# borglab/gtsfm

Measured on NVIDIA H100. Metric: image_pairs_per_sec, higher is better.
Workload: dtype f32

## Files before the change

gtsfm_b200/_lib.py:

```python
from __future__ import annotations

import ctypes as C
from pathlib import Path
from typing import Optional

import numpy as np

LIB_PATH = Path(__file__).resolve().parent / "libgtsfm_b200.so"

_lib: Optional[C.CDLL] = None


class B200Error(RuntimeError):
    pass


class LightGlueParams(C.Structure):
    _fields_ = [("depth_confidence", C.c_double), ("width_confidence", C.c_double), ("filter_threshold", C.c_double),
                ("prune_min_kpts", C.c_int), ("fp16_attention", C.c_int)]


class LightGluePair(C.Structure):
    _fields_ = [("kp0", C.c_void_p), ("desc0", C.c_void_p), ("n0", C.c_int), ("kp1", C.c_void_p), ("desc1", C.c_void_p), ("n1", C.c_int),
                ("out_matches", C.c_void_p), ("out_scores", C.c_void_p), ("out_k", C.c_int), ("out_stop_layer", C.c_int)]


class MnnPair(C.Structure):
    _fields_ = [("desc0", C.c_void_p), ("n0", C.c_int), ("desc1", C.c_void_p), ("n1", C.c_int), ("out_matches", C.c_void_p),
                ("out_dist", C.c_void_p), ("out_k", C.c_int)]


MNN_ERR_RATIO = -4


class SiftKeypoint(C.Structure):
    _fields_ = [("x", C.c_float), ("y", C.c_float), ("size", C.c_float), ("angle", C.c_float), ("response", C.c_float),
                ("octave", C.c_int32)]


SIFT_KEYPOINT_DTYPE = np.dtype([("x", np.float32), ("y", np.float32), ("size", np.float32), ("angle", np.float32),
                                ("response", np.float32), ("octave", np.int32)])


class SiftImage(C.Structure):
    _fields_ = [("image", C.c_void_p), ("mask", C.c_void_p), ("max_keypoints", C.c_int), ("out_keypoints", C.c_void_p),
                ("out_desc", C.c_void_p), ("out_n", C.c_int), ("out_total", C.c_int)]


class D2NetImage(C.Structure):
    _fields_ = [("image", C.c_void_p), ("max_keypoints", C.c_int), ("out_xy", C.c_void_p), ("out_scores", C.c_void_p),
                ("out_desc", C.c_void_p), ("out_n", C.c_int), ("out_total", C.c_int)]


SIFT_CAPACITY = -5


class RansacParams(C.Structure):
    _fields_ = [("threshold", C.c_double), ("confidence", C.c_double), ("max_iters", C.c_int), ("seed", C.c_uint64)]


_vp, _i, _f, _sz = C.c_void_p, C.c_int, C.c_float, C.c_size_t
_ip = C.POINTER(C.c_int)

SIGNATURES = {
    "b2_version": (_i, []),
    "b2_create": (_i, [_i, C.POINTER(_vp)]),
    "b2_destroy": (None, [_vp]),
    "b2_last_error": (C.c_char_p, [_vp]),
    "b2_launch_count": (C.c_uint64, [_vp]),
    "b2_h2d_bytes": (C.c_uint64, [_vp]),
    "b2_set_option": (C.c_int, [_vp, C.c_char_p, C.c_int64]),
    "b2_profile_start": (_i, [_vp, C.c_char_p]),
    "b2_profile_stop": (_i, [_vp, C.POINTER(C.c_double), C.POINTER(C.c_uint64), C.POINTER(C.c_double)]),
    "b2_debug_fetch": (C.c_int64, [_vp, C.c_char_p, _vp, C.c_int64]),
    "b2_debug_gemm_host": (_i, [_vp, _i, _vp, _vp, _vp, _vp, _i, _i, _i]),
    "b2_debug_attention_host": (_i, [_vp, _i, _ip, _ip, _i, _f, _i, _vp, _vp, _vp, _vp]),
    "b2_superpoint_set_weights": (_i, [_vp, _vp, _sz]),
    "b2_superpoint_detect_dev": (_i, [_vp, _vp, _i, _i, _i, _sz, _f, _i, _i, _vp, _vp, _i, _ip, C.POINTER(C.c_uint64), _vp]),
    "b2_superpoint_describe_dev": (_i, [_vp, C.c_uint64, _vp, _i, _vp, _vp]),
    "b2_superpoint_extract_dev": (_i, [_vp, _vp, _i, _i, _i, _sz, _f, _i, _i, _i, _vp, _vp, _vp, _ip, _vp]),
    "b2_superpoint_extract_async_dev": (_i, [_vp, _vp, _i, _i, _i, _sz, _f, _i, _i, _i, _vp, _vp, _vp, _vp, _vp]),
    "b2_superpoint_finish_dev": (_i, [_vp, _vp]),
    "b2_topk_indices_dev": (_i, [_vp, _vp, _i, _i, _vp, _ip, _vp]),
    "b2_superpoint_detect_host": (_i, [_vp, _vp, _i, _i, _i, _f, _i, _i, _vp, _vp, _i, _ip, C.POINTER(C.c_uint64)]),
    "b2_superpoint_describe_host": (_i, [_vp, C.c_uint64, _vp, _i, _vp]),
    "b2_image_resize_dev": (_i, [_vp, _vp, _i, _i, _i, _sz, _vp, _i, _i, _vp]),
    "b2_lightglue_set_weights": (_i, [_vp, _vp, _sz]),
    "b2_lightglue_match_dev": (_i, [_vp, _vp, _vp, _i, _vp, _vp, _i, C.POINTER(LightGlueParams), _vp, _vp, _ip, _ip, _vp]),
    "b2_lightglue_match_host": (_i, [_vp, _vp, _vp, _i, _vp, _vp, _i, C.POINTER(LightGlueParams), _vp, _vp, _ip, _ip]),
    "b2_lightglue_match_batched_dev": (_i, [_vp, C.POINTER(LightGluePair), _i, C.POINTER(LightGlueParams), _vp]),
    "b2_superglue_set_weights": (_i, [_vp, _vp, _sz]),
    "b2_superglue_match_dev": (_i, [_vp, _vp, _vp, _vp, _i, _i, _i, _vp, _vp, _vp, _i, _i, _i, _i, _f, _vp, _vp, _ip, _vp]),
    "b2_superglue_match_host": (_i, [_vp, _vp, _vp, _vp, _i, _i, _i, _vp, _vp, _vp, _i, _i, _i, _i, _f, _vp, _vp, _ip]),
    "b2_netvlad_blob_floats": (_sz, []),
    "b2_netvlad_set_weights": (_i, [_vp, _vp, _sz]),
    "b2_netvlad_describe_dev": (_i, [_vp, _vp, _i, _i, _i, _vp, _vp]),
    "b2_netvlad_describe_host": (_i, [_vp, _vp, _i, _i, _i, _vp]),
    "b2_megaloc_blob_floats": (_sz, []),
    "b2_megaloc_set_weights": (_i, [_vp, _vp, _sz]),
    "b2_megaloc_describe_dev": (_i, [_vp, _vp, _i, _i, _i, _vp, _vp]),
    "b2_megaloc_describe_host": (_i, [_vp, _vp, _i, _i, _i, _vp]),
    "b2_megaloc_describe_u8_dev": (_i, [_vp, _vp, _i, _i, _i, _sz, _vp, _vp]),
    "b2_megaloc_resize_u8_dev": (_i, [_vp, _vp, _i, _i, _i, _sz, _vp, _vp]),
    "b2_similarity_pairs_host": (_i, [_vp, _vp, _i, _i, _i, _f, _vp, _vp]),
    "b2_ransac_essential_host": (_i, [_vp, _vp, _vp, _i, C.POINTER(RansacParams), _vp, _vp, _ip, _vp, _vp]),
    "b2_ransac_fundamental_host": (_i, [_vp, _vp, _vp, _i, C.POINTER(RansacParams), _vp, _vp, _ip]),
    "b2_ransac_essential_dev": (_i, [_vp, _vp, _vp, _vp, _i, _vp, _vp, C.POINTER(RansacParams), _vp, _vp, _ip, _vp, _vp, _vp]),
    "b2_recover_pose_host": (_i, [_vp, _vp, _vp, _vp, _i, _vp, _vp, _ip]),
    "b2_mnn_match_batched_dev": (_i, [_vp, C.POINTER(MnnPair), _i, _i, _i, C.c_double, _vp]),
    "b2_mnn_match_host": (_i, [_vp, _vp, _i, _vp, _i, _i, _i, C.c_double, _vp, _vp, _ip]),
    "b2_sift_detect_batched_dev": (_i, [_vp, C.POINTER(SiftImage), _i, _i, _i, _i, _sz, _vp]),
    "b2_sift_detect_host": (_i, [_vp, _vp, _i, _i, _i, _vp, _vp, _vp, _i, _ip]),
    "b2_d2net_blob_floats": (_sz, []),
    "b2_d2net_norm_table": (_i, [_vp]),
    "b2_d2net_set_weights": (_i, [_vp, _vp, _sz]),
    "b2_d2net_detect_batched_dev": (_i, [_vp, C.POINTER(D2NetImage), _i, _i, _i, _i, _sz, _vp]),
    "b2_d2net_detect_host": (_i, [_vp, _vp, _i, _i, _i, _i, _vp, _vp, _vp, _ip, _ip]),
    "b2_debug_conv_ps_host": (_i, [_vp, _i, _vp, _i, _i, _i, _i, _vp, _vp, _i, _vp]),
    "b2_debug_d2net_avgpool_host": (_i, [_vp, _vp, _i, _i, _vp]),
    "b2_debug_d2net_rank_host": (_i, [_vp, _vp, _vp, _i, _i, _vp]),
}


def load() -> C.CDLL:
    global _lib
    if _lib is not None:
        return _lib
    if not LIB_PATH.exists():
        raise B200Error(f"{LIB_PATH} is missing: run `python -m gtsfm_b200.build` (there is no CPU fallback)")
    lib = C.CDLL(str(LIB_PATH))
    for name, (res, args) in SIGNATURES.items():
        fn = getattr(lib, name)
        fn.restype = res
        fn.argtypes = args
    _lib = lib
    return lib


def ptr(a) -> C.c_void_p:
    if a is None:
        return C.c_void_p(0)
    if isinstance(a, np.ndarray):
        assert a.flags["C_CONTIGUOUS"], "array must be C-contiguous"
        return C.c_void_p(a.ctypes.data)
    if hasattr(a, "data_ptr"):
        assert a.is_contiguous(), "tensor must be contiguous"
        return C.c_void_p(a.data_ptr())
    return C.c_void_p(int(a))


class Context:

    def __init__(self, device: int = 0):
        self._lib = load()
        h = C.c_void_p()
        rc = self._lib.b2_create(int(device), C.byref(h))
        if rc != 0 or not h:
            raise B200Error(
                f"b2_create(device={device}) failed with {rc}: an sm_90 (H100) GPU is required; there is no CPU fallback")
        self.handle = h
        self.device = device

    def check(self, rc: int, what: str) -> None:
        if rc < 0:
            raise B200Error(f"{what} failed ({rc}): {self._lib.b2_last_error(self.handle).decode()}")

    @property
    def lib(self) -> C.CDLL:
        return self._lib

    def launch_count(self) -> int:
        return int(self._lib.b2_launch_count(self.handle))

    def set_option(self, name: str, value: int) -> None:
        self.check(self._lib.b2_set_option(self.handle, name.encode(), int(value)), f"set_option({name})")

    def h2d_bytes(self) -> int:
        return int(self._lib.b2_h2d_bytes(self.handle))

    def profile_start(self, kernel_prefix: str) -> None:
        self.check(self._lib.b2_profile_start(self.handle, kernel_prefix.encode()), "profile_start")

    def profile_stop(self):
        ms, n, w = C.c_double(0), C.c_uint64(0), C.c_double(0)
        self.check(self._lib.b2_profile_stop(self.handle, C.byref(ms), C.byref(n), C.byref(w)), "profile_stop")
        return ms.value, int(n.value), w.value

    def debug_fetch(self, name: str, max_floats: int) -> np.ndarray:
        out = np.empty(max_floats, np.float32)
        n = self._lib.b2_debug_fetch(self.handle, name.encode(), ptr(out), max_floats)
        self.check(int(n), f"debug_fetch({name})")
        return out[:n]

    def close(self) -> None:
        if getattr(self, "handle", None):
            self._lib.b2_destroy(self.handle)
            self.handle = None

    def __del__(self):
        try:
            self.close()
        except Exception:
            pass
```

gtsfm_b200/csrc/attn_ps.cuh:

```cuda
#pragma once
#include "tma.cuh"

constexpr int AW_Q = 128, AW_KV = 64, AW_D = 64;
constexpr int AW_KV_BYTES = AW_KV * AW_D * 2;
constexpr int AS_NS = 4;
constexpr int AS_HALF = 2 * AW_KV_BYTES;
constexpr int AS_STAGE = 2 * AS_HALF;
constexpr int AS_TILE_BYTES = AS_NS * AS_STAGE;
constexpr int AS_Q_PLANE = AW_Q * AW_D * 2;
constexpr int AS_Q_BYTES = 2 * 2 * AS_Q_PLANE;
constexpr size_t AS_SMEM = AS_TILE_BYTES + AS_Q_BYTES + 1024 + 512;
constexpr int AS_THREADS = 256 + 128;
constexpr float AS_RESCALE = 8.0f;
constexpr int AP_MAXP = 16;

struct AttnPsMaps {
  CUtensorMap kh[AP_MAXP], kl[AP_MAXP], vh[AP_MAXP], vl[AP_MAXP];
};

struct AttnPsProblem {
  const __half *Qh, *Ql;
  __half *Oh, *Ol;
  int Nq, Nk;
  int ldo;
  int qt, tiles;
  int w_end;
  int item0;
};
struct AttnPsArgs {
  AttnPsProblem p[AP_MAXP];
  int nprob;
  float* Opart;
  float* ml;
  int* arrivals;
  int W;
  int quota;
  int max_splits;
  float scale;
  int* err_flag;
};

struct AttnPsSeg {
  int z, item, h, q0, tile0, T, split, nsplits, itemg;
};
__device__ __forceinline__ AttnPsSeg attn_ps_decode(const AttnPsArgs& a, int w, int w_end) {
  AttnPsSeg s;
  s.z = 0;
  while (s.z + 1 < a.nprob && w >= a.p[s.z].w_end) ++s.z;
  const AttnPsProblem& p = a.p[s.z];
  const int base = s.z ? a.p[s.z - 1].w_end : 0;
  const int wl = w - base;
  s.item = wl / p.tiles;
  s.tile0 = wl - s.item * p.tiles;
  s.T = min(p.tiles - s.tile0, w_end - w);
  s.h = s.item / p.qt;
  s.q0 = (s.item - s.h * p.qt) * (2 * AW_Q);
  const int wi0 = base + s.item * p.tiles, wi1 = wi0 + p.tiles;
  const int c_first = wi0 / a.quota;
  s.split = w / a.quota - c_first;
  s.nsplits = (wi1 - 1) / a.quota - c_first + 1;
  s.itemg = p.item0 + s.item;
  return s;
}

template <bool SINGLE>
static __global__ void __launch_bounds__(AS_THREADS, 1) k_flash_ps(const __grid_constant__ AttnPsMaps maps, const __grid_constant__ AttnPsArgs args) {
  extern __shared__ unsigned char ap_raw[];
  const uint32_t raw = tc::smem_u32(ap_raw);
  const uint32_t smem0 = (raw + 1023u) & ~1023u;
  unsigned char* sm = ap_raw + (smem0 - raw);
  uint64_t* bars = reinterpret_cast<uint64_t*>(sm + AS_TILE_BYTES + AS_Q_BYTES);
  uint64_t* kv_full = bars;
  uint64_t* kv_empty = kv_full + AS_NS;
  volatile int* last_flag = reinterpret_cast<volatile int*>(kv_empty + AS_NS);

  const int t = threadIdx.x, warp = t >> 5, lane = t & 31;
  const int w_begin = blockIdx.x * args.quota;
  const int w_end = min(args.W, w_begin + args.quota);

  if (t == 0) {
    for (int i = 0; i < AS_NS; ++i) tc::mbar_init(&kv_full[i], 1), tc::mbar_init(&kv_empty[i], 8);
    tc::fence_mbar_init();
  }
  __syncthreads();
  bool ok = true;

  if (warp >= 8) {
    asm volatile("setmaxnreg.dec.sync.aligned.u32 24;\n" ::: "memory");
    if (warp == 8 && lane == 0) {
      int ge = 0;
      for (int w = w_begin; w < w_end;) {
        const AttnPsSeg sg = attn_ps_decode(args, w, w_end);
        const int Nk = args.p[sg.z].Nk;
        for (int e = 0; e < sg.T + 2; ++e) {
          const int g = ge + e, s = g % AS_NS;
          if (g >= AS_NS) ok = tc::mbar_wait(&kv_empty[s], ((g / AS_NS) - 1) & 1) && ok;
          const bool hk = e < sg.T, hv = e >= 2;
          constexpr int PART = SINGLE ? AW_KV_BYTES : AS_HALF;
          tc::mbar_expect_tx(&kv_full[s], (hk ? PART : 0) + (hv ? PART : 0));
          const uint32_t dst = smem0 + s * AS_STAGE;
          if (hk) {
            const int row = sg.h * Nk + (sg.tile0 + e) * AW_KV;
            tc::tma_load_2d(dst, &maps.kh[sg.z], &kv_full[s], 0, row);
            if (!SINGLE) tc::tma_load_2d(dst + AW_KV_BYTES, &maps.kl[sg.z], &kv_full[s], 0, row);
          }
          if (hv) {
            const int row = sg.h * Nk + (sg.tile0 + e - 2) * AW_KV;
            tc::tma_load_2d(dst + AS_HALF, &maps.vh[sg.z], &kv_full[s], 0, row);
            if (!SINGLE) tc::tma_load_2d(dst + AS_HALF + AW_KV_BYTES, &maps.vl[sg.z], &kv_full[s], 0, row);
          }
        }
        ge += sg.T + 2;
        w += sg.T;
      }
    }
  } else {
    asm volatile("setmaxnreg.inc.sync.aligned.u32 240;\n" ::: "memory");
    const int q = warp >> 2;
    const int r = t & 127;
    const int rq = (warp & 3) * 16 + (lane >> 2);
    const int c2 = (lane & 3) * 2;
    const uint32_t sQ = smem0 + AS_TILE_BYTES + q * 2 * AS_Q_PLANE;
    const float c2s = args.scale * 1.4426950408889634f;
    auto wg_bar = [&]() { asm volatile("bar.sync %0, 128;" ::"r"(1 + q) : "memory"); };
    auto release = [&](int g) { if (lane == 0) tc::mbar_arrive(&kv_empty[g % AS_NS]); };

    int ge = 0;
    for (int w = w_begin; w < w_end;) {
      const AttnPsSeg sg = attn_ps_decode(args, w, w_end);
      const AttnPsProblem& pr = args.p[sg.z];
      const int T = sg.T, Nk = pr.Nk;
      {
        const int qrow = sg.q0 + q * AW_Q + r;
        wg_bar();
#pragma unroll
        for (int pl = 0; pl < (SINGLE ? 1 : 2); ++pl) {
          const __half* src = (pl ? pr.Ql : pr.Qh) + ((size_t)sg.h * pr.Nq + qrow) * 64;
          unsigned char* dst = sm + AS_TILE_BYTES + q * 2 * AS_Q_PLANE + pl * AS_Q_PLANE + r * 128;
#pragma unroll
          for (int c = 0; c < 8; ++c) {
            uint4 v = make_uint4(0u, 0u, 0u, 0u);
            if (qrow < pr.Nq) v = __ldg(reinterpret_cast<const uint4*>(src) + c);
            *reinterpret_cast<uint4*>(dst + ((c ^ (r & 7)) << 4)) = v;
          }
        }
        tc::fence_proxy_async();
        wg_bar();
      }
      uint32_t qf[2][16];
#pragma unroll
      for (int sl = 0; sl < 2; ++sl)
#pragma unroll
        for (int h = 0; h < 2; ++h) {
          const int qrow = sg.q0 + q * AW_Q + sl * 64 + rq + 8 * h;
          const uint32_t* src = reinterpret_cast<const uint32_t*>(pr.Qh + ((size_t)sg.h * pr.Nq + qrow) * 64 + c2);
#pragma unroll
          for (int j = 0; j < 8; ++j) qf[sl][4 * (j >> 1) + 2 * (j & 1) + h] = qrow < pr.Nq ? __ldg(src + 4 * j) : 0u;
        }
      float o[2][32];
      float m_ref[2][2], l_i[2][2];
#pragma unroll
      for (int sl = 0; sl < 2; ++sl)
#pragma unroll
        for (int h = 0; h < 2; ++h) m_ref[sl][h] = -INFINITY, l_i[sl][h] = 0.f;
      float s[2][32];
      uint32_t ph[2][16], pl[2][16];
      auto qk = [&](int i, int sl) {
        const uint32_t sK = smem0 + ((ge + i) % AS_NS) * AS_STAGE;
        const uint64_t dKh = tc::wg_desc_sw128(sK), dKl = tc::wg_desc_sw128(sK + AW_KV_BYTES);
        const uint64_t dQl = tc::wg_desc_sw128(sQ + AS_Q_PLANE + sl * (64 * 128));
        tc::wg_fence();
#pragma unroll
        for (int ks = 0; ks < 4; ++ks) {
          const uint64_t adv = (uint64_t)(ks * 2);
          tc::wg_rs_n64(s[sl], qf[sl] + 4 * ks, dKh + adv, ks ? 1u : 0u);
          if (!SINGLE) {
            tc::wg_rs_n64(s[sl], qf[sl] + 4 * ks, dKl + adv, 1u);
            tc::wg_ss_n64(s[sl], dQl + adv, dKh + adv, 1u);
          }
        }
        tc::wg_commit();
      };
      auto softmax = [&](int i, int sl) {
        float* a = s[sl];
        const int k0 = (sg.tile0 + i) * AW_KV;
        if (k0 + AW_KV > Nk) {
#pragma unroll
          for (int jj = 0; jj < 32; ++jj)
            if (k0 + 8 * (jj >> 2) + c2 + (jj & 1) >= Nk) a[jj] = -INFINITY;
        }
#pragma unroll
        for (int h = 0; h < 2; ++h) {
          float mx = a[2 * h];
#pragma unroll
          for (int j = 0; j < 8; ++j) mx = fmaxf(mx, fmaxf(a[4 * j + 2 * h], a[4 * j + 2 * h + 1]));
          mx = fmaxf(mx, __shfl_xor_sync(0xffffffffu, mx, 1));
          mx = fmaxf(mx, __shfl_xor_sync(0xffffffffu, mx, 2));
          const float m_new = fmaxf(m_ref[sl][h], mx * c2s);
          if (m_new - m_ref[sl][h] > AS_RESCALE) {
            const float corr = tc::ex2(m_ref[sl][h] - m_new);
            l_i[sl][h] *= corr;
            if (i > 0) {
#pragma unroll
              for (int j = 0; j < 8; ++j) o[sl][4 * j + 2 * h] *= corr, o[sl][4 * j + 2 * h + 1] *= corr;
            }
            m_ref[sl][h] = m_new;
          }
          float rs = 0.f;
#pragma unroll
          for (int j = 0; j < 8; ++j) {
            const float p0 = tc::ex2(fmaf(a[4 * j + 2 * h], c2s, -m_ref[sl][h]));
            const float p1 = tc::ex2(fmaf(a[4 * j + 2 * h + 1], c2s, -m_ref[sl][h]));
            rs += p0 + p1;
            const __half2 hh = __floats2half2_rn(p0, p1);
            const int ri = 4 * (j >> 1) + 2 * (j & 1) + h;
            ph[sl][ri] = *reinterpret_cast<const uint32_t*>(&hh);
            if (!SINGLE) {
              const float2 hf = __half22float2(hh);
              const __half2 ll = __floats2half2_rn(p0 - hf.x, p1 - hf.y);
              pl[sl][ri] = *reinterpret_cast<const uint32_t*>(&ll);
            }
          }
          l_i[sl][h] += rs;
        }
      };
      auto pv = [&](int i, int sl) {
        const uint32_t sV = smem0 + ((ge + i + 2) % AS_NS) * AS_STAGE + AS_HALF;
        const uint64_t dVh = tc::wg_desc_sw128(sV), dVl = tc::wg_desc_sw128(sV + AW_KV_BYTES);
        tc::wg_fence();
#pragma unroll
        for (int ks = 0; ks < 4; ++ks) {
          const uint64_t advV = (uint64_t)(ks * 128);
          tc::wg_rs_n64_bt(o[sl], ph[sl] + 4 * ks, dVh + advV, (i | ks) ? 1u : 0u);
          if (!SINGLE) {
            tc::wg_rs_n64_bt(o[sl], ph[sl] + 4 * ks, dVl + advV, 1u);
            tc::wg_rs_n64_bt(o[sl], pl[sl] + 4 * ks, dVh + advV, 1u);
          }
        }
        tc::wg_commit();
      };

      for (int j = 0; j < 2; ++j) ok = tc::mbar_wait(&kv_full[(ge + j) % AS_NS], ((ge + j) / AS_NS) & 1) && ok;
      if (T == 1) release(ge + 1);
      for (int i = 0; i < T; ++i) {
        qk(i, 0);
        qk(i, 1);
        tc::wg_wait<1>();
        tc::fence_regs(s[0]);
        softmax(i, 0);
        const int gv = ge + i + 2;
        ok = tc::mbar_wait(&kv_full[gv % AS_NS], (gv / AS_NS) & 1) && ok;
        pv(i, 0);
        tc::wg_wait<1>();
        tc::fence_regs(s[1]);
        release(ge + i);
        softmax(i, 1);
        pv(i, 1);
        tc::wg_wait<0>();
        tc::fence_regs(o[0]), tc::fence_regs(o[1]);
        if (i + 2 >= T) release(gv);
      }
      ge += T + 2;
      w += T;
#pragma unroll
      for (int sl = 0; sl < 2; ++sl)
#pragma unroll
        for (int h = 0; h < 2; ++h) {
          l_i[sl][h] += __shfl_xor_sync(0xffffffffu, l_i[sl][h], 1);
          l_i[sl][h] += __shfl_xor_sync(0xffffffffu, l_i[sl][h], 2);
        }
      auto write_row = [&](const float* v, float inv, int qrow) {
        uint32_t* dh = reinterpret_cast<uint32_t*>(pr.Oh + (size_t)qrow * pr.ldo + sg.h * 64 + c2);
        uint32_t* dl = reinterpret_cast<uint32_t*>(pr.Ol + (size_t)qrow * pr.ldo + sg.h * 64 + c2);
#pragma unroll
        for (int j = 0; j < 8; ++j) {
          uint32_t hi, lo;
          if (SINGLE) {
            const __half2 hh = __floats2half2_rn(tc::clamp_h(v[4 * j] * inv), tc::clamp_h(v[4 * j + 1] * inv));
            hi = *reinterpret_cast<const uint32_t*>(&hh), lo = 0u;
          } else {
            tc::split2(v[4 * j] * inv, v[4 * j + 1] * inv, hi, lo);
          }
          dh[4 * j] = hi;
          dl[4 * j] = lo;
        }
      };
      if (sg.nsplits == 1) {
#pragma unroll
        for (int sl = 0; sl < 2; ++sl)
#pragma unroll
          for (int h = 0; h < 2; ++h) {
            const int qrow = sg.q0 + q * AW_Q + sl * 64 + rq + 8 * h;
            if (qrow >= pr.Nq) continue;
            float v[32];
#pragma unroll
            for (int j = 0; j < 8; ++j) v[4 * j] = o[sl][4 * j + 2 * h], v[4 * j + 1] = o[sl][4 * j + 2 * h + 1];
            write_row(v, 1.0f / l_i[sl][h], qrow);
          }
      } else {
        const size_t slot0 = (size_t)sg.itemg * args.max_splits;
#pragma unroll
        for (int sl = 0; sl < 2; ++sl)
#pragma unroll
          for (int h = 0; h < 2; ++h) {
            const int rl = q * AW_Q + sl * 64 + rq + 8 * h;
            if (sg.q0 + rl >= pr.Nq) continue;
            const size_t rowi = (slot0 + sg.split) * 256 + rl;
            float* dst = args.Opart + rowi * 64 + c2;
#pragma unroll
            for (int j = 0; j < 8; ++j) *reinterpret_cast<float2*>(dst + 8 * j) = make_float2(o[sl][4 * j + 2 * h], o[sl][4 * j + 2 * h + 1]);
            if (c2 == 0) *reinterpret_cast<float2*>(args.ml + rowi * 2) = make_float2(m_ref[sl][h], l_i[sl][h]);
          }
        __threadfence();
        wg_bar();
        if (r == 0) {
          int* cnt = args.arrivals + sg.itemg * 2 + q;
          const int old = atomicAdd(cnt, 1);
          const int last = old == sg.nsplits - 1;
          if (last) atomicExch(cnt, 0);
          last_flag[q] = last;
        }
        wg_bar();
        if (last_flag[q]) {
          __threadfence();
#pragma unroll 1
          for (int sl = 0; sl < 2; ++sl)
#pragma unroll 1
            for (int h = 0; h < 2; ++h) {
              const int rl = q * AW_Q + sl * 64 + rq + 8 * h;
              const int qrow = sg.q0 + rl;
              if (qrow >= pr.Nq) continue;
              float m = -INFINITY;
              for (int sp = 0; sp < sg.nsplits; ++sp) m = fmaxf(m, __ldcg(args.ml + ((slot0 + sp) * 256 + rl) * 2));
              float l = 0.f, v[32];
#pragma unroll
              for (int j = 0; j < 32; ++j) v[j] = 0.f;
              for (int sp = 0; sp < sg.nsplits; ++sp) {
                const size_t ri = (slot0 + sp) * 256 + rl;
                const float2 mlv = __ldcg(reinterpret_cast<const float2*>(args.ml + ri * 2));
                const float wgt = tc::ex2(mlv.x - m);
                l = fmaf(mlv.y, wgt, l);
                const float* src = args.Opart + ri * 64 + c2;
#pragma unroll
                for (int j = 0; j < 8; ++j) {
                  const float2 x = __ldcg(reinterpret_cast<const float2*>(src + 8 * j));
                  v[4 * j] = fmaf(x.x, wgt, v[4 * j]), v[4 * j + 1] = fmaf(x.y, wgt, v[4 * j + 1]);
                }
              }
              write_row(v, 1.0f / l, qrow);
            }
        }
      }
    }
  }
  if (!ok && args.err_flag) *args.err_flag = 1;
}
```

gtsfm_b200/csrc/common.cuh:

```cuda
#pragma once
#include <cuda_runtime.h>
#include <stdint.h>
#include <stdio.h>
#include <stdlib.h>
#include <string.h>

#include <map>
#include <mutex>
#include <string>
#include <vector>

#include "../../include/gtsfm_b200.h"

#define B2_OK 0
#define B2_ERR_CUDA -1
#define B2_ERR_ARG -2
#define B2_ERR_STATE -3
#define B2_ERR_MNN_RATIO -4
#define B2_SIFT_CAPACITY -5

struct DevBuf {
  void* p = nullptr;
  size_t cap = 0;
  DevBuf() = default;
  DevBuf(const DevBuf&) = delete;
  DevBuf& operator=(const DevBuf&) = delete;
  ~DevBuf() { release(); }
  cudaError_t ensure(size_t bytes) {
    if (bytes <= cap) return cudaSuccess;
    if (p) cudaFree(p);
    p = nullptr;
    cap = 0;
    size_t want = bytes + bytes / 8 + 256;
    cudaError_t e = cudaMalloc(&p, want);
    if (e == cudaSuccess) cap = want;
    return e;
  }
  template <typename T>
  T* as() const { return reinterpret_cast<T*>(p); }
  void release() {
    if (p) cudaFree(p);
    p = nullptr;
    cap = 0;
  }
};

struct HostBuf {
  void* p = nullptr;
  size_t cap = 0;
  HostBuf() = default;
  HostBuf(const HostBuf&) = delete;
  HostBuf& operator=(const HostBuf&) = delete;
  ~HostBuf() { release(); }
  cudaError_t ensure(size_t bytes) {
    if (bytes <= cap) return cudaSuccess;
    if (p) cudaFreeHost(p);
    p = nullptr;
    cap = 0;
    size_t want = bytes + bytes / 8 + 256;
    cudaError_t e = cudaMallocHost(&p, want);
    if (e == cudaSuccess) cap = want;
    return e;
  }
  template <typename T>
  T* as() const { return reinterpret_cast<T*>(p); }
  void release() {
    if (p) cudaFreeHost(p);
    p = nullptr;
    cap = 0;
  }
};

struct DebugView {
  const float* p;
  int64_t n;
};

struct ProfState {
  bool on = false;
  std::string name;
  std::vector<cudaEvent_t> ev;
  size_t used = 0;
  double work = 0.0;
  bool match(const char* kernel) const { return on && strncmp(kernel, name.c_str(), name.size()) == 0; }
};

struct SuperPointState;
struct LightGlueState;
struct SuperGlueState;
struct RansacState;
struct RetrievalState;
struct NetVladState;
struct MnnState;
struct SiftState;
struct MegaLocState;
struct D2NetState;

struct FeatCacheEntry {
  const void* host = nullptr;
  size_t bytes = 0;
  uint64_t sig = 0;
  uint64_t stamp = 0;
  DevBuf buf;
};
constexpr int B2_FEAT_CACHE_SLOTS = 96;

struct b2_context {
  int device = 0;
  int sm_count = 132;
  int reserve_sms = 0;
  int lg_batch = 0;
  int sp_graph = -1;
  int force_simt = -1;
  std::string err;
  std::mutex mu;
  uint64_t launches = 0;
  ProfState prof;
  cudaStream_t stream = nullptr;
  std::map<std::string, DebugView> debug;
  SuperPointState* sp = nullptr;
  LightGlueState* lg = nullptr;
  SuperGlueState* sg = nullptr;
  RansacState* rs = nullptr;
  RetrievalState* rt = nullptr;
  NetVladState* nv = nullptr;
  MnnState* mn = nullptr;
  SiftState* sf = nullptr;
  MegaLocState* ml = nullptr;
  D2NetState* d2 = nullptr;
  DevBuf stage_d[8];
  HostBuf stage_h[4];
  FeatCacheEntry fcache[B2_FEAT_CACHE_SLOTS];
  DevBuf resize_taps;
  uint64_t fstamp = 0;
  int fcache_on = -1;
  uint64_t h2d_bytes = 0;
};

inline bool b2_force_simt(const b2_context* ctx) {
  if (ctx->force_simt >= 0) return ctx->force_simt != 0;
  const char* e = getenv("B2_FORCE_SIMT");
  return e && e[0] == '1';
}

inline int b2_fail(b2_context* ctx, int code, const std::string& msg) {
  if (ctx) ctx->err = msg;
  return code;
}

#define B2_CUDA(ctx, expr)                                                                        \
  do {                                                                                            \
    cudaError_t _e = (expr);                                                                      \
    if (_e != cudaSuccess) {                                                                      \
      return b2_fail(ctx, B2_ERR_CUDA, std::string(#expr) + ": " + cudaGetErrorString(_e) +       \
                                           " (" + __FILE__ + ":" + std::to_string(__LINE__) + ")"); \
    }                                                                                             \
  } while (0)

inline void b2_prof_mark(b2_context* ctx, cudaStream_t st) {
  ProfState& p = ctx->prof;
  if (p.used == p.ev.size()) {
    cudaEvent_t e;
    cudaEventCreate(&e);
    p.ev.push_back(e);
  }
  cudaEventRecord(p.ev[p.used++], st);
}
inline void b2_prof_work(b2_context* ctx, const char* kernel, double work) {
  if (ctx->prof.match(kernel)) ctx->prof.work += work;
}

#define B2_LAUNCH(ctx, kernel, grid, block, smem, stream, ...)  \
  do {                                                          \
    const bool _prof = (ctx)->prof.match(#kernel);              \
    if (_prof) b2_prof_mark((ctx), (stream));                   \
    kernel<<<(grid), (block), (smem), (stream)>>>(__VA_ARGS__); \
    if (_prof) b2_prof_mark((ctx), (stream));                   \
    (ctx)->launches++;                                          \
  } while (0)

#define B2_CHECK_LAUNCH(ctx) B2_CUDA(ctx, cudaGetLastError())

static inline int cdiv(int a, int b) { return (a + b - 1) / b; }

void sp_destroy(b2_context* ctx);
void lg_destroy(b2_context* ctx);
void sg_destroy(b2_context* ctx);
void rs_destroy(b2_context* ctx);
void rt_destroy(b2_context* ctx);
void nv_destroy(b2_context* ctx);
void mn_destroy(b2_context* ctx);
void sf_destroy(b2_context* ctx);
void ml_destroy(b2_context* ctx);
void d2_destroy(b2_context* ctx);

__device__ __forceinline__ float warp_sum(float v) {
#pragma unroll
  for (int o = 16; o > 0; o >>= 1) v += __shfl_xor_sync(0xffffffffu, v, o);
  return v;
}
__device__ __forceinline__ float warp_max(float v) {
#pragma unroll
  for (int o = 16; o > 0; o >>= 1) v = fmaxf(v, __shfl_xor_sync(0xffffffffu, v, o));
  return v;
}
```

gtsfm_b200/csrc/debug.cu:

```cuda
#include <stdlib.h>

#include <vector>

#include "common.cuh"
#include "linear.cuh"

static __global__ void k_split_unscaled_f32(const float* __restrict__ x, size_t n, __half* __restrict__ hi, __half* __restrict__ lo) {
  const size_t i = (size_t)blockIdx.x * blockDim.x + threadIdx.x;
  if (i < n) tc::split_h_unscaled(x[i], hi[i], lo[i]);
}

extern "C" int b2_debug_gemm_host(b2_context* ctx, int mode, const float* A, const float* B, const float* bias, float* C,
                                  int M, int N, int K) {
  if (!ctx || !A || !B || !C || M <= 0 || N <= 0 || K <= 0 || (K % 64)) return B2_ERR_ARG;
  std::lock_guard<std::mutex> lk(ctx->mu);
  cudaSetDevice(ctx->device);
  cudaStream_t st = ctx->stream;
  DevBuf dA, dB, dC, dBias, dErr;
  B2_CUDA(ctx, dA.ensure((size_t)M * K * 4));
  B2_CUDA(ctx, dB.ensure((size_t)N * K * 4));
  B2_CUDA(ctx, dC.ensure((size_t)M * N * 4));
  B2_CUDA(ctx, dBias.ensure((size_t)N * 4));
  B2_CUDA(ctx, dErr.ensure(16));
  B2_CUDA(ctx, cudaMemcpyAsync(dA.p, A, (size_t)M * K * 4, cudaMemcpyHostToDevice, st));
  B2_CUDA(ctx, cudaMemcpyAsync(dB.p, B, (size_t)N * K * 4, cudaMemcpyHostToDevice, st));
  if (bias) B2_CUDA(ctx, cudaMemcpyAsync(dBias.p, bias, (size_t)N * 4, cudaMemcpyHostToDevice, st));
  B2_CUDA(ctx, cudaMemsetAsync(dErr.p, 0, 16, st));
  if (mode == 0) {
    const int rc = launch_gemm(ctx, st, gemm_linear(dA.as<float>(), K, K, dB.as<float>(), bias ? dBias.as<float>() : nullptr, dC.as<float>(), N, M, N));
    if (rc != B2_OK) return rc;
  } else {
    DevBuf dAh, dAl, dBh, dBl;
    B2_CUDA(ctx, dAh.ensure((size_t)M * K * 2));
    B2_CUDA(ctx, dAl.ensure((size_t)M * K * 2));
    B2_CUDA(ctx, dBh.ensure((size_t)N * K * 2));
    B2_CUDA(ctx, dBl.ensure((size_t)N * K * 2));
    B2_LAUNCH(ctx, k_split_f32, (unsigned)(((size_t)M * K + 255) / 256), 256, 0, st, dA.as<float>(), (size_t)M * K, dAh.as<__half>(), dAl.as<__half>());
    B2_LAUNCH(ctx, k_split_f32, (unsigned)(((size_t)N * K + 255) / 256), 256, 0, st, dB.as<float>(), (size_t)N * K, dBh.as<__half>(), dBl.as<__half>());
    B2_CUDA(ctx, cudaFuncSetAttribute(k_gemm_ws, cudaFuncAttributeMaxDynamicSharedMemorySize, (int)GW_SMEM));
    TcWeights tw{nullptr, nullptr, nullptr, dErr.as<int>(), true};
    tw.sm_count = ctx->sm_count;
    LinArgs a;
    a.a1p = {dAh.as<__half>(), dAl.as<__half>()}, a.lda1 = K, a.K1 = K, a.bp = {dBh.as<__half>(), dBl.as<__half>()}, a.ldb = K;
    a.bias = bias ? dBias.as<float>() : nullptr, a.cf = dC.as<float>(), a.ldc = N, a.tc_want_f32 = true, a.M = M, a.N = N;
    const int rc = run_linear(ctx, st, tw, &a, 1);
    if (rc != B2_OK) return rc;
    B2_CUDA(ctx, cudaStreamSynchronize(st));
  }
  int err = 0;
  B2_CUDA(ctx, cudaMemcpyAsync(C, dC.p, (size_t)M * N * 4, cudaMemcpyDeviceToHost, st));
  B2_CUDA(ctx, cudaMemcpyAsync(&err, dErr.p, 4, cudaMemcpyDeviceToHost, st));
  B2_CUDA(ctx, cudaStreamSynchronize(st));
  if (err) return b2_fail(ctx, B2_ERR_STATE, "wgmma pipeline timed out on an mbarrier (kernel bug)");
  return B2_OK;
}

extern "C" int b2_debug_attention_host(b2_context* ctx, int np, const int* nq, const int* nk, int heads, float scale, int single,
                                       const float* q, const float* k, const float* v, float* o) {
  if (!ctx || !nq || !nk || !q || !k || !v || !o || np <= 0 || np > AP_MAXP || heads <= 0) return B2_ERR_ARG;
  size_t eq = 0, ek = 0;
  for (int z = 0; z < np; ++z) {
    if (nq[z] <= 0 || nk[z] <= 0) return B2_ERR_ARG;
    eq += (size_t)nq[z] * heads * 64, ek += (size_t)nk[z] * heads * 64;
  }
  std::lock_guard<std::mutex> lk(ctx->mu);
  cudaSetDevice(ctx->device);
  cudaStream_t st = ctx->stream;
  const size_t n = eq + 2 * ek;
  DevBuf dIn, dPl, dO, dErr, part, ml, cnt;
  B2_CUDA(ctx, dIn.ensure(n * 4));
  B2_CUDA(ctx, dPl.ensure(n * 2 * 2));
  B2_CUDA(ctx, dO.ensure(eq * 2 * 2));
  B2_CUDA(ctx, dErr.ensure(16));
  float* in = dIn.as<float>();
  B2_CUDA(ctx, cudaMemcpyAsync(in, q, eq * 4, cudaMemcpyHostToDevice, st));
  B2_CUDA(ctx, cudaMemcpyAsync(in + eq, k, ek * 4, cudaMemcpyHostToDevice, st));
  B2_CUDA(ctx, cudaMemcpyAsync(in + eq + ek, v, ek * 4, cudaMemcpyHostToDevice, st));
  B2_CUDA(ctx, cudaMemsetAsync(dErr.p, 0, 16, st));
  __half *hi = dPl.as<__half>(), *lo = hi + n, *oh = dO.as<__half>(), *ol = oh + eq;
  B2_LAUNCH(ctx, k_split_unscaled_f32, (unsigned)((n + 255) / 256), 256, 0, st, in, n, hi, lo);
  B2_CUDA(ctx, cudaFuncSetAttribute(k_flash_ps<false>, cudaFuncAttributeMaxDynamicSharedMemorySize, (int)AS_SMEM));
  B2_CUDA(ctx, cudaFuncSetAttribute(k_flash_ps<true>, cudaFuncAttributeMaxDynamicSharedMemorySize, (int)AS_SMEM));
  FlashPlanes fp[AP_MAXP];
  size_t qo = 0, ko = eq;
  for (int z = 0; z < np; ++z) {
    const size_t vo = ko + ek;
    fp[z] = {{hi + qo, lo + qo}, {hi + ko, lo + ko}, {hi + vo, lo + vo}, {oh + qo, ol + qo}, nq[z], nk[z], heads, 64 * heads};
    qo += (size_t)nq[z] * heads * 64, ko += (size_t)nk[z] * heads * 64;
  }
  TcWeights tw{nullptr, nullptr, nullptr, dErr.as<int>(), true};
  tw.attn_part = &part, tw.attn_ml = &ml, tw.attn_cnt = &cnt, tw.sm_count = ctx->sm_count;
  const int rc = run_flash_planes(ctx, st, tw, fp, np, scale, single != 0);
  if (rc != B2_OK) return rc;
  std::vector<__half> ho(2 * eq);
  int err = 0;
  B2_CUDA(ctx, cudaMemcpyAsync(ho.data(), oh, eq * 2 * 2, cudaMemcpyDeviceToHost, st));
  B2_CUDA(ctx, cudaMemcpyAsync(&err, dErr.p, 4, cudaMemcpyDeviceToHost, st));
  B2_CUDA(ctx, cudaStreamSynchronize(st));
  for (size_t i = 0; i < eq; ++i) o[i] = __half2float(ho[i]) + __half2float(ho[eq + i]) * tc::LO_INV;
  if (err) return b2_fail(ctx, B2_ERR_STATE, "wgmma attention timed out on an mbarrier (kernel bug)");
  return B2_OK;
}
```

gtsfm_b200/csrc/gemm_ws.cuh:

```cuda
#pragma once
#include "tma.cuh"

constexpr int GW_MAXP = 16;
constexpr int GW_M = 128, GW_N = 128, GW_K = 64;
constexpr int GW_A_BYTES = GW_M * GW_K * 2;
constexpr int GW_B_BYTES = GW_N * GW_K * 2;
constexpr int GW_STAGE_BYTES = 2 * GW_A_BYTES + 2 * GW_B_BYTES;
constexpr int GW_STAGES = 2;
constexpr int GW_PITCH = GW_N + 8;
constexpr int GW_STG_BYTES = GW_M * GW_PITCH * 4;
constexpr int GW_RB = 8;
constexpr int GW_EW = 4;
constexpr int GW_THREADS = 512;
constexpr size_t GW_SMEM = GW_STAGES * GW_STAGE_BYTES + GW_STG_BYTES + 1024  + 256 ;

struct GemmProblem {
  const float* resid;
  float* C;
  __half *Ch, *Cl;
  int M, N, ldc;
  int vec4;
  int tiles_n;
  int tile_end;
};
struct GemmWsMaps {
  CUtensorMap a1h[GW_MAXP], a1l[GW_MAXP];
  CUtensorMap a2h[GW_MAXP], a2l[GW_MAXP];
  CUtensorMap bh[GW_MAXP], bl[GW_MAXP];
};
struct GemmWsArgs {
  GemmProblem p[GW_MAXP];
  int nprob, tiles;
  int K1, K2;
  int b_per_problem;
  const float* bias;
  int ldr;
  float scale;
  int ldch;
  int head_major;
  int relu;
  int gelu;
  int lo_unscaled;
  int* err_flag;
};

static __global__ void __launch_bounds__(GW_THREADS, 1) k_gemm_ws(const __grid_constant__ GemmWsMaps maps, const __grid_constant__ GemmWsArgs g) {
  extern __shared__ unsigned char gw_raw[];
  const uint32_t raw = tc::smem_u32(gw_raw);
  const uint32_t smem0 = (raw + 1023u) & ~1023u;
  unsigned char* sm = gw_raw + (smem0 - raw);
  float* stg = reinterpret_cast<float*>(sm + GW_STAGES * GW_STAGE_BYTES);
  uint64_t* full = reinterpret_cast<uint64_t*>(sm + GW_STAGES * GW_STAGE_BYTES + GW_STG_BYTES);
  uint64_t* empty = full + GW_STAGES;
  uint64_t* sfull = empty + GW_STAGES;
  uint64_t* sempty = sfull + 1;

  const int t = threadIdx.x, warp = t >> 5, lane = t & 31;
  const int nk = (g.K1 + g.K2) / GW_K;

  if (t == 0) {
    for (int s = 0; s < GW_STAGES; ++s) tc::mbar_init(&full[s], 1), tc::mbar_init(&empty[s], 8);
    tc::mbar_init(sfull, 256);
    tc::mbar_init(sempty, 32 * GW_EW);
    tc::fence_mbar_init();
    tc::tma_prefetch_desc(&maps.bh[0]);
    tc::tma_prefetch_desc(&maps.bl[0]);
  }
  __syncthreads();
  bool ok = true;

  auto decode = [&](int tile, int& z, int& m0, int& n0) {
    z = 0;
    while (z + 1 < g.nprob && tile >= g.p[z].tile_end) ++z;
    const int local = tile - (z ? g.p[z - 1].tile_end : 0);
    const int mt = local / g.p[z].tiles_n;
    n0 = (local - mt * g.p[z].tiles_n) * GW_N;
    m0 = mt * GW_M;
  };

  if (warp >= 12) {
    asm volatile("setmaxnreg.dec.sync.aligned.u32 40;\n" ::: "memory");
    if (warp == 12 && lane == 0) {
      int gk = 0;
      for (int tile = blockIdx.x; tile < g.tiles; tile += gridDim.x) {
        int z, m0, n0;
        decode(tile, z, m0, n0);
        const int zb = g.b_per_problem ? z : 0;
        for (int kc = 0; kc < nk; ++kc, ++gk) {
          const int s = gk % GW_STAGES;
          if (gk >= GW_STAGES) ok = tc::mbar_wait(&empty[s], ((gk / GW_STAGES) - 1) & 1) && ok;
          const int k0 = kc * GW_K;
          const bool seg2 = k0 >= g.K1;
          const CUtensorMap* ah = seg2 ? &maps.a2h[z] : &maps.a1h[z];
          const CUtensorMap* al = seg2 ? &maps.a2l[z] : &maps.a1l[z];
          const int ka = seg2 ? k0 - g.K1 : k0;
          const uint32_t sA = smem0 + s * GW_STAGE_BYTES, sB = sA + 2 * GW_A_BYTES;
          tc::mbar_expect_tx(&full[s], GW_STAGE_BYTES);
          tc::tma_load_2d(sA, ah, &full[s], ka, m0);
          tc::tma_load_2d(sA + GW_A_BYTES, al, &full[s], ka, m0);
          tc::tma_load_2d(sB, &maps.bh[zb], &full[s], k0, n0);
          tc::tma_load_2d(sB + GW_B_BYTES, &maps.bl[zb], &full[s], k0, n0);
        }
      }
    }
  } else if (warp < 8) {
    asm volatile("setmaxnreg.inc.sync.aligned.u32 184;\n" ::: "memory");
    const int wg = warp >> 2;
    const int r0 = wg * 64 + (warp & 3) * 16 + (lane >> 2);
    const int c2 = (lane & 3) * 2;
    int gk = 0, it = 0;
    for (int tile = blockIdx.x; tile < g.tiles; tile += gridDim.x, ++it) {
      float acc0[64], acc1[64];
      for (int kc = 0; kc < nk; ++kc, ++gk) {
        const int s = gk % GW_STAGES;
        ok = tc::mbar_wait(&full[s], (gk / GW_STAGES) & 1) && ok;
        const uint32_t aH = smem0 + s * GW_STAGE_BYTES + wg * (64 * 128), aL = aH + GW_A_BYTES;
        const uint32_t bH = smem0 + s * GW_STAGE_BYTES + 2 * GW_A_BYTES, bL = bH + GW_B_BYTES;
        const uint64_t dAh = tc::wg_desc_sw128(aH), dAl = tc::wg_desc_sw128(aL), dBh = tc::wg_desc_sw128(bH), dBl = tc::wg_desc_sw128(bL);
        tc::wg_fence();
#pragma unroll
        for (int ks = 0; ks < GW_K / 16; ++ks) {
          const uint64_t adv = (uint64_t)(ks * 2);
          const uint32_t first = (kc == 0 && ks == 0) ? 0u : 1u;
          tc::wg_ss_n128(acc0, dAh + adv, dBh + adv, first);
          tc::wg_ss_n128(acc1, dAh + adv, dBl + adv, first);
          tc::wg_ss_n128(acc1, dAl + adv, dBh + adv, 1u);
        }
        tc::wg_commit();
        if (kc > 0) {
          tc::wg_wait<1>();
          if (lane == 0) tc::mbar_arrive(&empty[(gk - 1) % GW_STAGES]);
        }
      }
      tc::wg_wait<0>();
      if (lane == 0) tc::mbar_arrive(&empty[(gk - 1) % GW_STAGES]);

      if (it > 0) ok = tc::mbar_wait(sempty, (it - 1) & 1) && ok;
#pragma unroll
      for (int j = 0; j < 16; ++j)
#pragma unroll
        for (int h = 0; h < 2; ++h) {
          const int i = 4 * j + 2 * h;
          *reinterpret_cast<float2*>(stg + (r0 + 8 * h) * GW_PITCH + 8 * j + c2) =
              make_float2(fmaf(acc1[i], tc::LO_INV, acc0[i]), fmaf(acc1[i + 1], tc::LO_INV, acc0[i + 1]));
        }
      tc::mbar_arrive(sfull);
    }
  } else {
    asm volatile("setmaxnreg.dec.sync.aligned.u32 104;\n" ::: "memory");
    const int ew = warp - 8;
    const int c = 4 * lane;
    const float scale = g.scale;
    const int relu = g.relu, gelu = g.gelu, hm = g.head_major, lo_unscaled = g.lo_unscaled, ldr = g.ldr, ldch = g.ldch;
    int it = 0;
    for (int tile = blockIdx.x; tile < g.tiles; tile += gridDim.x, ++it) {
      int z, m0, n0;
      decode(tile, z, m0, n0);
      const GemmProblem& pb = g.p[z];
      const float* resid = pb.resid;
      float* C = pb.C;
      __half *Ch = pb.Ch, *Cl = pb.Cl;
      const int M = pb.M, ldc = pb.ldc;
      const int n = n0 + c;
      const int ncols = min(4, pb.N - n);
      const bool vec = pb.vec4 && ncols == 4;
      const int rows = min(GW_M, M - m0);
      float b4[4] = {0.f, 0.f, 0.f, 0.f};
      if (g.bias)
#pragma unroll
        for (int e = 0; e < 4; ++e)
          if (e < ncols) b4[e] = __ldg(g.bias + n + e);
      const size_t hm_col = (size_t)(n >> 6) * M * 64 + (n & 63);
      const bool vres = resid && vec;
      float4 rr[GW_RB];
      auto load_resid = [&](int rb) {
#pragma unroll
        for (int i = 0; i < GW_RB; ++i)
          if (rb + GW_EW * i < rows) rr[i] = *reinterpret_cast<const float4*>(resid + (size_t)(m0 + rb + GW_EW * i) * ldr + n);
      };
      if (vres) load_resid(ew);
      ok = tc::mbar_wait(sfull, it & 1) && ok;
      if (ncols > 0) {
        for (int rb = ew; rb < rows; rb += GW_EW * GW_RB) {
          if (vres && rb != ew) load_resid(rb);
#pragma unroll
          for (int i = 0; i < GW_RB; ++i) {
            const int r = rb + GW_EW * i;
            if (r >= rows) break;
            const int row = m0 + r;
            const float4 a = *reinterpret_cast<const float4*>(stg + r * GW_PITCH + c);
            float v[4] = {a.x, a.y, a.z, a.w};
#pragma unroll
            for (int e = 0; e < 4; ++e) {
              v[e] = (v[e] + b4[e]) * scale;
              if (relu) v[e] = fmaxf(v[e], 0.f);
              if (gelu) v[e] = 0.5f * v[e] * (1.0f + erff(v[e] * 0.70710678118654752440f));
            }
            const size_t off_c = hm ? hm_col + (size_t)row * 64 : (size_t)row * ldc + n;
            const size_t off_s = hm ? hm_col + (size_t)row * 64 : (size_t)row * ldch + n;
            if (vec) {
              if (resid) v[0] += rr[i].x, v[1] += rr[i].y, v[2] += rr[i].z, v[3] += rr[i].w;
              if (C) *reinterpret_cast<float4*>(C + off_c) = make_float4(v[0], v[1], v[2], v[3]);
              if (Ch) {
                uint32_t h01, l01, h23, l23;
                if (lo_unscaled) {
                  tc::split2_unscaled_clamped(v[0], v[1], h01, l01);
                  tc::split2_unscaled_clamped(v[2], v[3], h23, l23);
                } else {
                  tc::split2(v[0], v[1], h01, l01);
                  tc::split2(v[2], v[3], h23, l23);
                }
                *reinterpret_cast<uint2*>(Ch + off_s) = make_uint2(h01, h23);
                *reinterpret_cast<uint2*>(Cl + off_s) = make_uint2(l01, l23);
              }
            } else {
#pragma unroll
              for (int e = 0; e < 4; ++e) {
                if (e >= ncols) break;
                if (resid) v[e] += resid[(size_t)row * ldr + n + e];
                if (C) C[off_c + e] = v[e];
                if (Ch) {
                  __half hh, ll;
                  if (lo_unscaled) tc::split_h_unscaled(v[e], hh, ll);
                  else tc::split_h(v[e], hh, ll);
                  Ch[off_s + e] = hh;
                  Cl[off_s + e] = ll;
                }
              }
            }
          }
        }
      }
      tc::mbar_arrive(sempty);
    }
  }
  if (!ok && g.err_flag) *g.err_flag = 1;
}
```

gtsfm_b200/csrc/lightglue.cu:

```cuda
#include <stdlib.h>

#include "common.cuh"
#include "linear.cuh"
#include "assign_ps.cuh"

namespace {
constexpr int LG_LAYERS = 9;
constexpr size_t LG_NFLOATS = 11851601;
constexpr int D = 256;

struct SelfW {
  float *wqkv, *bqkv, *wout, *bout, *w0, *b0, *lng, *lnb, *w3, *b3;
};
struct CrossW {
  float *wqk, *bqk, *wv, *bv, *wout, *bout, *w0, *b0, *lng, *lnb, *w3, *b3;
};
struct AssignW {
  float *wm, *bm, *wf, *bf;
};
struct ConfW {
  float *w, *b;
};
}

constexpr int LG_MAX_PAIRS = 8;
constexpr int LG_MAX_SIDES = 2 * LG_MAX_PAIRS;
static_assert(LG_MAX_SIDES <= GW_MAXP && LG_MAX_SIDES <= AP_MAXP, "batch does not fit one launch");

struct LgSide {
  DevBuf x[2], xs[2], qkv, q, k, v, ctx, msg, h, hs, cs[2], sn[2], ind[2], conf, mat, src, md, rmax, rlog, ls, lsg, amax, aidx;
  int cur = 0;
  int n = 0;
  int cap = 0;
};

struct LgPair {
  bool active = false;
  int n0 = 0, n1 = 0;
  int stop = 0;
  long long* out_matches = nullptr;
  float* out_scores = nullptr;
};

struct LightGlueState {
  bool loaded = false;
  int persist_ctas = 132;
  DevBuf wblob, wblob_h, wblob_l, errflag;
  bool use_tc = true;
  float* wr = nullptr;
  SelfW sw[LG_LAYERS];
  CrossW cw[LG_LAYERS];
  AssignW aw[LG_LAYERS];
  ConfW tw[LG_LAYERS - 1];
  float thr[LG_LAYERS];
  LgSide side[LG_MAX_SIDES];
  LgPair pair[LG_MAX_PAIRS];
  DevBuf sim[LG_MAX_PAIRS], counters, attn_part, attn_ml, attn_cnt, as_part, as_bar;
  HostBuf hread;
};

template <typename J>
struct JobList {
  J j[LG_MAX_SIDES];
};

void lg_destroy(b2_context* ctx) {
  delete ctx->lg;
  ctx->lg = nullptr;
}


struct PosJob {
  const float* kp;
  int n;
  float *cs, *sn;
  int* ind;
};
__global__ void __launch_bounds__(1024) k_lg_posenc(const __grid_constant__ JobList<PosJob> jobs, const float* __restrict__ wr ) {
  const PosJob& jb = jobs.j[blockIdx.y];
  const float* __restrict__ kp = jb.kp;
  const int n = jb.n;
  float* __restrict__ cs = jb.cs;
  float* __restrict__ sn = jb.sn;
  int* __restrict__ ind = jb.ind;
  if (n <= 0 || blockIdx.x * 1024 >= n * 32) return;
  __shared__ float red[4][32];
  __shared__ float bb[4];
  float mnx = INFINITY, mny = INFINITY, mxx = -INFINITY, mxy = -INFINITY;
  for (int i = threadIdx.x; i < n; i += blockDim.x) {
    float x = kp[2 * i], y = kp[2 * i + 1];
    mnx = fminf(mnx, x), mny = fminf(mny, y), mxx = fmaxf(mxx, x), mxy = fmaxf(mxy, y);
  }
  mnx = -warp_max(-mnx), mny = -warp_max(-mny), mxx = warp_max(mxx), mxy = warp_max(mxy);
  int lane = threadIdx.x & 31, warp = threadIdx.x >> 5;
  if (lane == 0) red[0][warp] = mnx, red[1][warp] = mny, red[2][warp] = mxx, red[3][warp] = mxy;
  __syncthreads();
  if (warp == 0) {
    float a = -warp_max(-red[0][lane]), b = -warp_max(-red[1][lane]), c = warp_max(red[2][lane]), d = warp_max(red[3][lane]);
    if (lane == 0) bb[0] = a, bb[1] = b, bb[2] = c, bb[3] = d;
  }
  __syncthreads();
  const float sx = 1.0f + bb[2] - bb[0], sy = 1.0f + bb[3] - bb[1];
  const float shx = sx / 2.0f, shy = sy / 2.0f, sc = fmaxf(sx, sy) / 2.0f;
  const int gtid = blockIdx.x * blockDim.x + threadIdx.x, gsz = gridDim.x * blockDim.x;
  for (int i = gtid; i < n * 32; i += gsz) {
    int p = i >> 5, f = i & 31;
    float x = (kp[2 * p] - shx) / sc, y = (kp[2 * p + 1] - shy) / sc;
    float pr = x * wr[2 * f] + y * wr[2 * f + 1];
    cs[i] = cosf(pr);
    sn[i] = sinf(pr);
  }
  for (int i = gtid; i < n; i += gsz) ind[i] = i;
}

struct LoadJob {
  const float* desc;
  int n;
  float* x;
  __half *hi, *lo;
};
__global__ void __launch_bounds__(256) k_lg_load_desc(const __grid_constant__ JobList<LoadJob> jobs) {
  const LoadJob& jb = jobs.j[blockIdx.y];
  const size_t i = ((size_t)blockIdx.x * blockDim.x + threadIdx.x) * 4;
  if (i >= (size_t)jb.n * 256) return;
  const float4 v = *reinterpret_cast<const float4*>(jb.desc + i);
  *reinterpret_cast<float4*>(jb.x + i) = v;
  if (jb.hi) {
    uint32_t h01, l01, h23, l23;
    tc::split2(v.x, v.y, h01, l01);
    tc::split2(v.z, v.w, h23, l23);
    *reinterpret_cast<uint2*>(jb.hi + i) = make_uint2(h01, h23);
    *reinterpret_cast<uint2*>(jb.lo + i) = make_uint2(l01, l23);
  }
}

struct RotJob {
  const float *qkv, *cs, *sn;
  int n;
  size_t plane;
  void *qo, *ko, *vo;
};
template <bool SPLIT>
__global__ void __launch_bounds__(256) k_lg_split_rotary(const __grid_constant__ JobList<RotJob> jobs, int qk_unscaled) {
  const RotJob& jb = jobs.j[blockIdx.y];
  const float* __restrict__ qkv = jb.qkv;
  const float* __restrict__ cs = jb.cs;
  const float* __restrict__ sn = jb.sn;
  const int n = jb.n;
  const size_t plane = jb.plane;
  void* __restrict__ qo = jb.qo;
  void* __restrict__ ko = jb.ko;
  void* __restrict__ vo = jb.vo;
  int i = blockIdx.x * blockDim.x + threadIdx.x;
  if (i >= n * 128) return;
  int p = i & 31, h = (i >> 5) & 3, r = i >> 7;
  const float* src = qkv + (size_t)r * 768 + (h * 64 + 2 * p) * 3;
  float q0 = src[0], k0 = src[1], v0 = src[2], q1 = src[3], k1 = src[4], v1 = src[5];
  float c = cs[r * 32 + p], s = sn[r * 32 + p];
  size_t o = ((size_t)h * n + r) * 64 + 2 * p;
  const float qa = __fadd_rn(__fmul_rn(q0, c), __fmul_rn(-q1, s)), qb = __fadd_rn(__fmul_rn(q1, c), __fmul_rn(q0, s));
  const float ka = __fadd_rn(__fmul_rn(k0, c), __fmul_rn(-k1, s)), kb = __fadd_rn(__fmul_rn(k1, c), __fmul_rn(k0, s));
  if (SPLIT) {
    __half* outs[3] = {static_cast<__half*>(qo), static_cast<__half*>(ko), static_cast<__half*>(vo)};
    const float va[3] = {qa, ka, v0}, vb[3] = {qb, kb, v1};
#pragma unroll
    for (int j = 0; j < 3; ++j) {
      __half ha, la, hb, lb;
      if ((qk_unscaled >> (j < 2 ? 0 : 1)) & 1) {
        tc::split_h_unscaled(va[j], ha, la);
        tc::split_h_unscaled(vb[j], hb, lb);
      } else {
        tc::split_h(va[j], ha, la);
        tc::split_h(vb[j], hb, lb);
      }
      *reinterpret_cast<__half2*>(outs[j] + o) = __halves2half2(ha, hb);
      *reinterpret_cast<__half2*>(outs[j] + plane + o) = __halves2half2(la, lb);
    }
  } else {
    float *q = static_cast<float*>(qo), *k = static_cast<float*>(ko), *v = static_cast<float*>(vo);
    q[o] = qa, q[o + 1] = qb, k[o] = ka, k[o + 1] = kb, v[o] = v0, v[o + 1] = v1;
  }
}

struct LnJob {
  float* h;
  int n;
  __half *hi, *lo;
};
__global__ void __launch_bounds__(256) k_lg_ln_gelu(const __grid_constant__ JobList<LnJob> jobs, const float* __restrict__ g, const float* __restrict__ b) {
  const LnJob& jb = jobs.j[blockIdx.y];
  float* __restrict__ h = jb.h;
  __half* __restrict__ hi = jb.hi;
  __half* __restrict__ lo = jb.lo;
  const int n = jb.n;
  int r = blockIdx.x * 8 + (threadIdx.x >> 5), lane = threadIdx.x & 31;
  if (r >= n) return;
  float4* row = reinterpret_cast<float4*>(h + (size_t)r * 512);
  float4 v[4];
  float s = 0.f;
#pragma unroll
  for (int i = 0; i < 4; ++i) {
    v[i] = row[lane + 32 * i];
    s += v[i].x + v[i].y + v[i].z + v[i].w;
  }
  float mean = warp_sum(s) / 512.0f;
  float q = 0.f;
#pragma unroll
  for (int i = 0; i < 4; ++i) {
    float a = v[i].x - mean, bq = v[i].y - mean, c = v[i].z - mean, d = v[i].w - mean;
    q += a * a + bq * bq + c * c + d * d;
  }
  float rstd = 1.0f / sqrtf(warp_sum(q) / 512.0f + 1e-5f);
#pragma unroll
  for (int i = 0; i < 4; ++i) {
    int c0 = (lane + 32 * i) * 4;
    float4 gg = *reinterpret_cast<const float4*>(g + c0), bb = *reinterpret_cast<const float4*>(b + c0);
    float e[4] = {(v[i].x - mean) * rstd * gg.x + bb.x, (v[i].y - mean) * rstd * gg.y + bb.y,
                  (v[i].z - mean) * rstd * gg.z + bb.z, (v[i].w - mean) * rstd * gg.w + bb.w};
#pragma unroll
    for (int j = 0; j < 4; ++j) e[j] = 0.5f * e[j] * (1.0f + erff(e[j] * 0.70710678118654752440f));
    if (hi) {
      uint32_t h01, l01, h23, l23;
      tc::split2(e[0], e[1], h01, l01);
      tc::split2(e[2], e[3], h23, l23);
      *reinterpret_cast<uint2*>(hi + (size_t)r * 512 + c0) = make_uint2(h01, h23);
      *reinterpret_cast<uint2*>(lo + (size_t)r * 512 + c0) = make_uint2(l01, l23);
    } else {
      row[lane + 32 * i] = make_float4(e[0], e[1], e[2], e[3]);
    }
  }
}

struct HeadJob {
  const float* x;
  int n;
  const float *w2, *b2;
  float *o1, *o2, *zraw;
};
__global__ void __launch_bounds__(256) k_lg_rowheads(const __grid_constant__ JobList<HeadJob> jobs, const float* __restrict__ w1,
                                                      const float* __restrict__ b1) {
  const HeadJob& jb = jobs.j[blockIdx.y];
  const float* __restrict__ x = jb.x;
  const float* __restrict__ w2 = jb.w2;
  const float* __restrict__ b2 = jb.b2;
  float* __restrict__ o1 = jb.o1;
  float* __restrict__ o2 = jb.o2;
  float* __restrict__ zraw = jb.zraw;
  const int n = jb.n;
  int r = blockIdx.x * 8 + (threadIdx.x >> 5), lane = threadIdx.x & 31;
  if (r >= n) return;
  const float4* row = reinterpret_cast<const float4*>(x + (size_t)r * 256);
  float4 a = row[lane], b = row[lane + 32];
  float s1 = 0.f, s2 = 0.f;
  if (w1) {
    float4 wa = reinterpret_cast<const float4*>(w1)[lane], wb = reinterpret_cast<const float4*>(w1)[lane + 32];
    s1 = a.x * wa.x + a.y * wa.y + a.z * wa.z + a.w * wa.w + b.x * wb.x + b.y * wb.y + b.z * wb.z + b.w * wb.w;
  }
  if (w2) {
    float4 wa = reinterpret_cast<const float4*>(w2)[lane], wb = reinterpret_cast<const float4*>(w2)[lane + 32];
    s2 = a.x * wa.x + a.y * wa.y + a.z * wa.z + a.w * wa.w + b.x * wb.x + b.y * wb.y + b.z * wb.z + b.w * wb.w;
  }
  s1 = warp_sum(s1);
  s2 = warp_sum(s2);
  if (lane == 0) {
    if (w1) o1[r] = 1.0f / (1.0f + expf(-(s1 + b1[0])));
    if (w2) {
      float z = s2 + b2[0];
      if (o2) o2[r] = 1.0f / (1.0f + expf(-z));
      if (zraw) zraw[r] = z;
    }
  }
}

struct PruneJob {
  const float *conf, *mat;
  int n;
  int* src;
  int* counters;
  int side;
};
__global__ void __launch_bounds__(1024) k_lg_prune_plan(const __grid_constant__ JobList<PruneJob> jobs, float thr, float keep_thr) {
  const PruneJob& jb = jobs.j[blockIdx.y];
  const int side = jb.side;
  int* __restrict__ counters = jb.counters;
  if (jb.n <= 0) return;
  const float* __restrict__ conf = jb.conf;
  const float* __restrict__ mat = jb.mat;
  int* __restrict__ src = jb.src;
  const int n = jb.n;
  __shared__ int wtot[32];
  __shared__ int carry, unconf;
  if (threadIdx.x == 0) carry = 0, unconf = 0;
  __syncthreads();
  const int lane = threadIdx.x & 31, warp = threadIdx.x >> 5;
  for (int base = 0; base < n; base += 1024) {
    int i = base + threadIdx.x;
    bool keep = false, unc = false;
    if (i < n) {
      float c = conf[i];
      unc = c < thr;
      keep = (mat[i] > keep_thr) || (c <= thr);
    }
    unsigned km = __ballot_sync(0xffffffffu, keep), um = __ballot_sync(0xffffffffu, unc);
    if (lane == 0) wtot[warp] = __popc(km);
    if (lane == 0 && um) atomicAdd(&unconf, __popc(um));
    __syncthreads();
    if (warp == 0) {
      int w = wtot[lane], ws = w;
#pragma unroll
      for (int o = 1; o < 32; o <<= 1) {
        int u = __shfl_up_sync(0xffffffffu, ws, o);
        if (lane >= o) ws += u;
      }
      wtot[lane] = ws - w;
    }
    __syncthreads();
    int pos = carry + wtot[warp] + __popc(km & ((1u << lane) - 1));
    if (keep) src[pos] = i;
    __syncthreads();
    if (threadIdx.x == 1023) carry = pos + (keep ? 1 : 0);
    __syncthreads();
  }
  if (threadIdx.x == 0) {
    counters[side] = unconf;
    counters[2 + side] = carry;
  }
}

struct GatherJob {
  const int *src, *cnt;
  int n;
  const float *x, *cs, *sn;
  const int* ind;
  float *x2, *cs2, *sn2;
  int* ind2;
  const __half* ph;
  size_t pstride;
  __half* ph2;
  size_t pstride2;
};
__global__ void __launch_bounds__(256) k_lg_gather(const __grid_constant__ JobList<GatherJob> jobs) {
  const GatherJob& jb = jobs.j[blockIdx.y];
  int r = blockIdx.x * 8 + (threadIdx.x >> 5), lane = threadIdx.x & 31;
  if (jb.n <= 0 || r >= *jb.cnt) return;
  int s = jb.src[r];
  const float4* a = reinterpret_cast<const float4*>(jb.x + (size_t)s * 256);
  float4* o = reinterpret_cast<float4*>(jb.x2 + (size_t)r * 256);
  o[lane] = a[lane];
  o[lane + 32] = a[lane + 32];
  jb.cs2[r * 32 + lane] = jb.cs[s * 32 + lane];
  jb.sn2[r * 32 + lane] = jb.sn[s * 32 + lane];
  if (lane == 0) jb.ind2[r] = jb.ind[s];
  if (jb.ph) {
    reinterpret_cast<uint4*>(jb.ph2 + (size_t)r * 256)[lane] = reinterpret_cast<const uint4*>(jb.ph + (size_t)s * 256)[lane];
    reinterpret_cast<uint4*>(jb.ph2 + jb.pstride2 + (size_t)r * 256)[lane] = reinterpret_cast<const uint4*>(jb.ph + jb.pstride + (size_t)s * 256)[lane];
  }
}

__device__ __forceinline__ float logsigmoid(float z) {
  return fminf(z, 0.f) - log1pf(expf(-fabsf(z)));
}

__global__ void __launch_bounds__(256) k_lg_row_stats(const float* __restrict__ sim, int m, int n, float* __restrict__ rmax,
                                                       float* __restrict__ rlog, const float* __restrict__ z,
                                                       float* __restrict__ lsg) {
  int r = blockIdx.x * 8 + (threadIdx.x >> 5), lane = threadIdx.x & 31;
  if (r >= m) return;
  const float* row = sim + (size_t)r * n;
  float mx = -INFINITY;
  for (int j = lane; j < n; j += 32) mx = fmaxf(mx, row[j]);
  mx = warp_max(mx);
  float s = 0.f;
  for (int j = lane; j < n; j += 32) s += expf(row[j] - mx);
  s = warp_sum(s);
  if (lane == 0) rmax[r] = mx, rlog[r] = logf(s), lsg[r] = logsigmoid(z[r]);
}
constexpr int LG_COL_WARPS = 32, LG_COL_UNROLL = 4;
__global__ void __launch_bounds__(1024) k_lg_col_stats(const float* __restrict__ sim, int m, int n, float* __restrict__ cmax,
                                                        float* __restrict__ clog, const float* __restrict__ z,
                                                        float* __restrict__ lsg) {
  __shared__ float sm[LG_COL_WARPS][32], ss[LG_COL_WARPS][32];
  const int lane = threadIdx.x & 31, warp = threadIdx.x >> 5;
  const int j = blockIdx.x * 32 + lane;
  float mx = -INFINITY, s = 0.f;
  if (j < n) {
    for (int i0 = warp; i0 < m; i0 += LG_COL_WARPS * LG_COL_UNROLL) {
      float x[LG_COL_UNROLL];
#pragma unroll
      for (int u = 0; u < LG_COL_UNROLL; ++u) {
        const int i = i0 + u * LG_COL_WARPS;
        x[u] = i < m ? sim[(size_t)i * n + j] : -INFINITY;
      }
#pragma unroll
      for (int u = 0; u < LG_COL_UNROLL; ++u) {
        if (x[u] > mx) {
          s = s * expf(mx - x[u]) + 1.0f;
          mx = x[u];
        } else if (x[u] > -INFINITY) {
          s += expf(x[u] - mx);
        }
      }
    }
  }
  sm[warp][lane] = mx, ss[warp][lane] = s;
  __syncthreads();
  if (warp == 0 && j < n) {
    float M = sm[0][lane];
    for (int w = 1; w < LG_COL_WARPS; ++w) M = fmaxf(M, sm[w][lane]);
    float S = 0.f;
    for (int w = 0; w < LG_COL_WARPS; ++w)
      if (ss[w][lane] > 0.f) S += ss[w][lane] * expf(sm[w][lane] - M);
    cmax[j] = M, clog[j] = logf(S), lsg[j] = logsigmoid(z[j]);
  }
}

__global__ void __launch_bounds__(256) k_lg_row_argmax(const float* __restrict__ sim, int m, int n,
                                                        const float* __restrict__ rmax, const float* __restrict__ rlog,
                                                        const float* __restrict__ cmax, const float* __restrict__ clog,
                                                        const float* __restrict__ l0g, const float* __restrict__ l1g,
                                                        float* __restrict__ best, int* __restrict__ arg) {
  int r = blockIdx.x * 8 + (threadIdx.x >> 5), lane = threadIdx.x & 31;
  if (r >= m) return;
  const float* row = sim + (size_t)r * n;
  const float rm = rmax[r], rl = rlog[r], l0 = l0g[r];
  float bv = -INFINITY;
  int bi = 0x7fffffff;
  for (int j = lane; j < n; j += 32) {
    float x = row[j];
    float sc = (((x - rm) - rl) + ((x - cmax[j]) - clog[j])) + (l0 + l1g[j]);
    if (sc > bv) bv = sc, bi = j;
  }
#pragma unroll
  for (int o = 16; o > 0; o >>= 1) {
    float ov = __shfl_xor_sync(0xffffffffu, bv, o);
    int oi = __shfl_xor_sync(0xffffffffu, bi, o);
    if (ov > bv || (ov == bv && oi < bi)) bv = ov, bi = oi;
  }
  if (lane == 0) best[r] = bv, arg[r] = bi;
}
__global__ void __launch_bounds__(1024) k_lg_col_argmax(const float* __restrict__ sim, int m, int n,
                                                         const float* __restrict__ rmax, const float* __restrict__ rlog,
                                                         const float* __restrict__ cmax, const float* __restrict__ clog,
                                                         const float* __restrict__ l0g, const float* __restrict__ l1g,
                                                         int* __restrict__ arg) {
  __shared__ float sv[LG_COL_WARPS][32];
  __shared__ int si[LG_COL_WARPS][32];
  const int lane = threadIdx.x & 31, warp = threadIdx.x >> 5;
  const int j = blockIdx.x * 32 + lane;
  float bv = -INFINITY;
  int bi = 0x7fffffff;
  if (j < n) {
    const float cm = cmax[j], cl = clog[j], l1 = l1g[j];
    for (int i0 = warp; i0 < m; i0 += LG_COL_WARPS * LG_COL_UNROLL) {
      float x[LG_COL_UNROLL], rm[LG_COL_UNROLL], rl[LG_COL_UNROLL], l0[LG_COL_UNROLL];
#pragma unroll
      for (int u = 0; u < LG_COL_UNROLL; ++u) {
        const int i = i0 + u * LG_COL_WARPS;
        const bool in = i < m;
        x[u] = in ? sim[(size_t)i * n + j] : 0.f;
        rm[u] = in ? rmax[i] : 0.f, rl[u] = in ? rlog[i] : 0.f, l0[u] = in ? l0g[i] : 0.f;
      }
#pragma unroll
      for (int u = 0; u < LG_COL_UNROLL; ++u) {
        const int i = i0 + u * LG_COL_WARPS;
        if (i < m) {
          const float sc = (((x[u] - rm[u]) - rl[u]) + ((x[u] - cm) - cl)) + (l0[u] + l1);
          if (sc > bv) bv = sc, bi = i;
        }
      }
    }
  }
  sv[warp][lane] = bv, si[warp][lane] = bi;
  __syncthreads();
  if (warp == 0 && j < n) {
    for (int w = 1; w < LG_COL_WARPS; ++w) {
      float ov = sv[w][lane];
      int oi = si[w][lane];
      if (ov > bv || (ov == bv && oi < bi)) bv = ov, bi = oi;
    }
    arg[j] = bi == 0x7fffffff ? 0 : bi;
  }
}

__global__ void __launch_bounds__(1024) k_lg_filter(const float* __restrict__ best0, const int* __restrict__ a0,
                                                     const int* __restrict__ a1, int m, float th, const int* __restrict__ ind0,
                                                     const int* __restrict__ ind1, long long* __restrict__ out,
                                                     float* __restrict__ outs, int* __restrict__ count) {
  __shared__ int wtot[32];
  __shared__ int carry;
  if (threadIdx.x == 0) carry = 0;
  __syncthreads();
  const int lane = threadIdx.x & 31, warp = threadIdx.x >> 5;
  for (int base = 0; base < m; base += 1024) {
    int i = base + threadIdx.x;
    bool valid = false;
    float ms = 0.f;
    int j = 0;
    if (i < m) {
      j = a0[i];
      bool mutual = a1[j] == i;
      ms = mutual ? expf(best0[i]) : 0.f;
      valid = mutual && ms > th;
    }
    unsigned vm = __ballot_sync(0xffffffffu, valid);
    if (lane == 0) wtot[warp] = __popc(vm);
    __syncthreads();
    if (warp == 0) {
      int w = wtot[lane], ws = w;
#pragma unroll
      for (int o = 1; o < 32; o <<= 1) {
        int u = __shfl_up_sync(0xffffffffu, ws, o);
        if (lane >= o) ws += u;
      }
      wtot[lane] = ws - w;
    }
    __syncthreads();
    int pos = carry + wtot[warp] + __popc(vm & ((1u << lane) - 1));
    if (valid) {
      out[2 * (size_t)pos] = ind0[i];
      out[2 * (size_t)pos + 1] = ind1[j];
      if (outs) outs[pos] = ms;
    }
    __syncthreads();
    if (threadIdx.x == 1023) carry = pos + (valid ? 1 : 0);
    __syncthreads();
  }
  if (threadIdx.x == 0) *count = carry;
}


extern "C" int b2_lightglue_set_weights(b2_context* ctx, const float* blob, size_t n_floats) {
  if (!ctx || !blob) return B2_ERR_ARG;
  std::lock_guard<std::mutex> lk(ctx->mu);
  if (n_floats != LG_NFLOATS)
    return b2_fail(ctx, B2_ERR_ARG, "lightglue blob must hold 11851601 floats, got " + std::to_string(n_floats));
  cudaSetDevice(ctx->device);
  if (!ctx->lg) ctx->lg = new LightGlueState();
  LightGlueState* s = ctx->lg;
  std::vector<size_t> sizes;
  sizes.push_back(64);
  for (int i = 0; i < LG_LAYERS; ++i) {
    const size_t self_sz[] = {768 * 256, 768, 256 * 256, 256, 512 * 512, 512, 512, 512, 256 * 512, 256};
    const size_t cross_sz[] = {256 * 256, 256, 256 * 256, 256, 256 * 256, 256, 512 * 512, 512, 512, 512, 256 * 512, 256};
    for (size_t z : self_sz) sizes.push_back(z);
    for (size_t z : cross_sz) sizes.push_back(z);
  }
  for (int i = 0; i < LG_LAYERS; ++i) {
    const size_t asz[] = {256, 1, 256 * 256, 256};
    for (size_t z : asz) sizes.push_back(z);
  }
  for (int i = 0; i < LG_LAYERS - 1; ++i) sizes.push_back(256), sizes.push_back(1);
  size_t total = 0, src_total = 0;
  std::vector<size_t> doff;
  for (size_t z : sizes) {
    doff.push_back(total);
    total += (z + 63) / 64 * 64;
    src_total += z;
  }
  if (src_total != LG_NFLOATS) return b2_fail(ctx, B2_ERR_STATE, "internal lightglue layout mismatch");
  std::vector<float> host(total, 0.f);
  size_t so = 0;
  for (size_t i = 0; i < sizes.size(); ++i) {
    memcpy(host.data() + doff[i], blob + so, sizes[i] * sizeof(float));
    so += sizes[i];
  }
  B2_CUDA(ctx, s->wblob.ensure(total * sizeof(float)));
  B2_CUDA(ctx, cudaMemcpy(s->wblob.p, host.data(), total * sizeof(float), cudaMemcpyHostToDevice));
  float* base = s->wblob.as<float>();
  size_t ti = 0;
  auto next = [&]() { return base + doff[ti++]; };
  s->wr = next();
  for (int i = 0; i < LG_LAYERS; ++i) {
    SelfW& a = s->sw[i];
    a.wqkv = next(), a.bqkv = next(), a.wout = next(), a.bout = next(), a.w0 = next(), a.b0 = next(), a.lng = next(),
    a.lnb = next(), a.w3 = next(), a.b3 = next();
    CrossW& c = s->cw[i];
    c.wqk = next(), c.bqk = next(), c.wv = next(), c.bv = next(), c.wout = next(), c.bout = next(), c.w0 = next(),
    c.b0 = next(), c.lng = next(), c.lnb = next(), c.w3 = next(), c.b3 = next();
  }
  for (int i = 0; i < LG_LAYERS; ++i) {
    AssignW& a = s->aw[i];
    a.wm = next(), a.bm = next(), a.wf = next(), a.bf = next();
  }
  for (int i = 0; i < LG_LAYERS - 1; ++i) s->tw[i].w = next(), s->tw[i].b = next();
  for (int i = 0; i < LG_LAYERS; ++i) {
    double t = 0.8 + 0.1 * exp(-4.0 * i / LG_LAYERS);
    t = t < 0 ? 0 : (t > 1 ? 1 : t);
    s->thr[i] = (float)t;
  }
  B2_CUDA(ctx, s->wblob_h.ensure(total * sizeof(__half)));
  B2_CUDA(ctx, s->wblob_l.ensure(total * sizeof(__half)));
  B2_CUDA(ctx, s->errflag.ensure(16));
  B2_CUDA(ctx, cudaMemset(s->errflag.p, 0, 16));
  B2_LAUNCH(ctx, k_split_f32, (unsigned)((total + 255) / 256), 256, 0, (cudaStream_t)0, s->wblob.as<float>(), total,
            s->wblob_h.as<__half>(), s->wblob_l.as<__half>());
  B2_CHECK_LAUNCH(ctx);
  B2_CUDA(ctx, cudaDeviceSynchronize());
  B2_CUDA(ctx, cudaFuncSetAttribute(k_gemm_ws, cudaFuncAttributeMaxDynamicSharedMemorySize, (int)GW_SMEM));
  B2_CUDA(ctx, cudaFuncSetAttribute(k_flash_ps<false>, cudaFuncAttributeMaxDynamicSharedMemorySize, (int)AS_SMEM));
  B2_CUDA(ctx, cudaFuncSetAttribute(k_flash_ps<true>, cudaFuncAttributeMaxDynamicSharedMemorySize, (int)AS_SMEM));
  s->use_tc = !b2_force_simt(ctx);
  B2_CUDA(ctx, cudaFuncSetAttribute(k_flash_attn, cudaFuncAttributeMaxDynamicSharedMemorySize, (int)FA_SMEM));
  B2_CUDA(ctx, s->hread.ensure(8 * LG_MAX_PAIRS * sizeof(int)));
  B2_CUDA(ctx, s->counters.ensure(8 * LG_MAX_PAIRS * sizeof(int)));
  B2_CUDA(ctx, cudaMemset(s->counters.p, 0, 8 * LG_MAX_PAIRS * sizeof(int)));
  s->loaded = true;
  return B2_OK;
}

static inline TcWeights lg_tw(LightGlueState* s) {
  TcWeights t{s->wblob.as<float>(), s->wblob_h.as<__half>(), s->wblob_l.as<__half>(), s->errflag.as<int>(), s->use_tc};
  t.attn_part = &s->attn_part, t.attn_ml = &s->attn_ml, t.attn_cnt = &s->attn_cnt, t.sm_count = s->persist_ctas;
  return t;
}

static int lg_side_alloc(b2_context* ctx, LgSide& sd, int n) {
  const size_t N = (size_t)(n > 0 ? n : 1);
  for (int i = 0; i < 2; ++i) {
    B2_CUDA(ctx, sd.x[i].ensure(N * 256 * 4));
    B2_CUDA(ctx, sd.xs[i].ensure(N * 256 * 4));
    B2_CUDA(ctx, sd.cs[i].ensure(N * 32 * 4));
    B2_CUDA(ctx, sd.sn[i].ensure(N * 32 * 4));
    B2_CUDA(ctx, sd.ind[i].ensure(N * 4));
  }
  B2_CUDA(ctx, sd.qkv.ensure(N * 768 * 4));
  B2_CUDA(ctx, sd.q.ensure(N * 256 * 4));
  B2_CUDA(ctx, sd.k.ensure(N * 256 * 4));
  B2_CUDA(ctx, sd.v.ensure(N * 256 * 4));
  B2_CUDA(ctx, sd.ctx.ensure(N * 256 * 4));
  B2_CUDA(ctx, sd.msg.ensure(N * 256 * 4));
  B2_CUDA(ctx, sd.h.ensure(N * 512 * 4));
  B2_CUDA(ctx, sd.hs.ensure(N * 512 * 4));
  B2_CUDA(ctx, sd.md.ensure(N * 256 * 4));
  DevBuf* small[] = {&sd.conf, &sd.mat, &sd.src, &sd.rmax, &sd.rlog, &sd.ls, &sd.lsg, &sd.amax, &sd.aidx};
  for (DevBuf* b : small) B2_CUDA(ctx, b->ensure(N * 4));
  sd.cur = 0;
  sd.n = n;
  sd.cap = n;
  return B2_OK;
}

struct LgActive {
  int side[LG_MAX_SIDES];
  int n = 0;
};
static LgActive lg_active_sides(const LightGlueState* s, int np) {
  LgActive a;
  for (int p = 0; p < np; ++p)
    if (s->pair[p].active) a.side[a.n++] = 2 * p, a.side[a.n++] = 2 * p + 1;
  return a;
}
static int lg_max_n(const LightGlueState* s, const LgActive& act) {
  int mx = 0;
  for (int i = 0; i < act.n; ++i) mx = s->side[act.side[i]].n > mx ? s->side[act.side[i]].n : mx;
  return mx;
}

static int lg_out_and_ffn(b2_context* ctx, cudaStream_t st, LightGlueState* s, const LgActive& act, const float* wout, const float* bout,
                          const float* w0, const float* b0, const float* lng, const float* lnb, const float* w3, const float* b3) {
  int rc;
  const TcWeights tw = lg_tw(s);
  LinArgs o[LG_MAX_SIDES], f0[LG_MAX_SIDES], f3[LG_MAX_SIDES];
  for (int i = 0; i < act.n; ++i) {
    LgSide& sd = s->side[act.side[i]];
    const size_t e = (size_t)sd.cap * 256;
    float* x = sd.x[sd.cur].as<float>();
    LinArgs& a = o[i];
    a.a1f = sd.ctx.as<float>(), a.a1p = planes_of(sd.ctx, e), a.lda1 = 256, a.K1 = 256, a.w = wout, a.ldb = 256, a.bias = bout;
    a.cf = sd.msg.as<float>(), a.ldc = 256, a.cp = planes_of(sd.msg, e), a.ldch = 256, a.M = sd.n, a.N = 256;
    LinArgs& f = f0[i];
    f.a1f = x, f.a1p = planes_of(sd.xs[sd.cur], e), f.lda1 = 256, f.K1 = 256;
    f.a2f = sd.msg.as<float>(), f.a2p = planes_of(sd.msg, e), f.lda2 = 256, f.K2 = 256;
    f.w = w0, f.ldb = 512, f.bias = b0, f.cf = sd.h.as<float>(), f.ldc = 512, f.tc_want_f32 = true, f.M = sd.n, f.N = 512;
    LinArgs& c = f3[i];
    c.a1f = sd.h.as<float>(), c.a1p = planes_of(sd.hs, (size_t)sd.cap * 512), c.lda1 = 512, c.K1 = 512, c.w = w3, c.ldb = 512, c.bias = b3;
    c.resid = x, c.ldr = 256;
    c.cf = x, c.ldc = 256, c.tc_want_f32 = true, c.cp = planes_of(sd.xs[sd.cur], e), c.ldch = 256, c.M = sd.n, c.N = 256;
  }
  if ((rc = run_linear(ctx, st, tw, o, act.n))) return rc;
  if ((rc = run_linear(ctx, st, tw, f0, act.n))) return rc;
  {
    JobList<LnJob> lj{};
    for (int i = 0; i < act.n; ++i) {
      LgSide& sd = s->side[act.side[i]];
      const Pl hs = planes_of(sd.hs, (size_t)sd.cap * 512);
      lj.j[i] = {sd.h.as<float>(), sd.n, s->use_tc ? hs.hi : (__half*)nullptr, s->use_tc ? hs.lo : (__half*)nullptr};
    }
    const int mx = lg_max_n(s, act);
    if (mx > 0) {
      B2_LAUNCH(ctx, k_lg_ln_gelu, dim3(cdiv(mx, 8), act.n), 256, 0, st, lj, lng, lnb);
      B2_CHECK_LAUNCH(ctx);
    }
  }
  return run_linear(ctx, st, tw, f3, act.n);
}

static int lg_self_layer(b2_context* ctx, cudaStream_t st, LightGlueState* s, const LgActive& act, int layer, bool fp16_attn) {
  const SelfW& w = s->sw[layer];
  const TcWeights tw = lg_tw(s);
  int rc;
  LinArgs q[LG_MAX_SIDES];
  for (int i = 0; i < act.n; ++i) {
    LgSide& sd = s->side[act.side[i]];
    LinArgs& a = q[i];
    a.a1f = sd.x[sd.cur].as<float>(), a.a1p = planes_of(sd.xs[sd.cur], (size_t)sd.cap * 256), a.lda1 = 256, a.K1 = 256;
    a.w = w.wqkv, a.ldb = 256, a.bias = w.bqkv, a.cf = sd.qkv.as<float>(), a.ldc = 768, a.tc_want_f32 = true, a.M = sd.n, a.N = 768;
  }
  if ((rc = run_linear(ctx, st, tw, q, act.n))) return rc;
  {
    JobList<RotJob> rj{};
    for (int i = 0; i < act.n; ++i) {
      LgSide& sd = s->side[act.side[i]];
      rj.j[i] = {sd.qkv.as<float>(), sd.cs[sd.cur].as<float>(), sd.sn[sd.cur].as<float>(), sd.n, (size_t)sd.cap * 256, sd.q.p, sd.k.p, sd.v.p};
    }
    const int mx = lg_max_n(s, act);
    if (mx > 0) {
      if (s->use_tc)
        B2_LAUNCH(ctx, k_lg_split_rotary<true>, dim3(cdiv(mx * 128, 256), act.n), 256, 0, st, rj, 3);
      else
        B2_LAUNCH(ctx, k_lg_split_rotary<false>, dim3(cdiv(mx * 128, 256), act.n), 256, 0, st, rj, 0);
      B2_CHECK_LAUNCH(ctx);
    }
  }
  FlashJob fj[LG_MAX_SIDES];
  for (int i = 0; i < act.n; ++i) {
    LgSide& a = s->side[act.side[i]];
    fj[i] = {&a.q, &a.k, &a.v, &a.ctx, a.n, a.n, a.cap, a.cap};
  }
  if ((rc = run_flash(ctx, st, tw, fj, act.n, 0.125f, fp16_attn))) return rc;
  return lg_out_and_ffn(ctx, st, s, act, w.wout, w.bout, w.w0, w.b0, w.lng, w.lnb, w.w3, w.b3);
}

static int lg_cross_block(b2_context* ctx, cudaStream_t st, LightGlueState* s, const LgActive& act, int layer, bool fp16_attn) {
  const CrossW& w = s->cw[layer];
  const TcWeights tw = lg_tw(s);
  int rc;
  for (int which = 0; which < 2; ++which) {
    LinArgs p[LG_MAX_SIDES];
    for (int i = 0; i < act.n; ++i) {
      LgSide& sd = s->side[act.side[i]];
      const size_t e = (size_t)sd.cap * 256;
      LinArgs& a = p[i];
      a.a1f = sd.x[sd.cur].as<float>(), a.a1p = planes_of(sd.xs[sd.cur], e), a.lda1 = 256, a.K1 = 256;
      a.w = which ? w.wv : w.wqk, a.ldb = 256, a.bias = which ? w.bv : w.bqk;
      DevBuf& dst = which ? sd.v : sd.q;
      a.cf = dst.as<float>(), a.cp = planes_of(dst, e), a.head_major = 1, a.M = sd.n, a.N = 256;
      a.lo_unscaled = s->use_tc ? 1 : 0;
    }
    if ((rc = run_linear(ctx, st, tw, p, act.n))) return rc;
  }
  FlashJob fj[LG_MAX_SIDES];
  for (int i = 0; i < act.n; ++i) {
    LgSide &a = s->side[act.side[i]], &b = s->side[act.side[i] ^ 1];
    fj[i] = {&a.q, &b.q, &b.v, &a.ctx, a.n, b.n, a.cap, b.cap};
  }
  if ((rc = run_flash(ctx, st, tw, fj, act.n, 0.125f, fp16_attn))) return rc;
  return lg_out_and_ffn(ctx, st, s, act, w.wout, w.bout, w.w0, w.b0, w.lng, w.lnb, w.w3, w.b3);
}

static int lg_match_batch(b2_context* ctx, b2_lightglue_pair* pairs, int np, const b2_lightglue_params* prm, cudaStream_t st) {
  LightGlueState* s = ctx->lg;
  int rc;
  for (int p = 0; p < np; ++p) {
    b2_lightglue_pair& pr = pairs[p];
    pr.out_k = 0, pr.out_stop_layer = 1;
    LgPair& lp = s->pair[p];
    lp.n0 = pr.n0, lp.n1 = pr.n1, lp.stop = 0, lp.out_matches = (long long*)pr.out_matches, lp.out_scores = pr.out_scores;
    lp.active = pr.n0 > 0 && pr.n1 > 0;
    if (!lp.active) {
      s->side[2 * p].n = s->side[2 * p + 1].n = 0;
      continue;
    }
    if ((rc = lg_side_alloc(ctx, s->side[2 * p], pr.n0))) return rc;
    if ((rc = lg_side_alloc(ctx, s->side[2 * p + 1], pr.n1))) return rc;
  }
  LgActive act = lg_active_sides(s, np);
  if (act.n == 0) return B2_OK;
  {
    JobList<LoadJob> lj{};
    JobList<PosJob> pj{};
    for (int i = 0; i < act.n; ++i) {
      const int sdi = act.side[i];
      LgSide& sd = s->side[sdi];
      const b2_lightglue_pair& pr = pairs[sdi >> 1];
      const float* desc = (sdi & 1) ? pr.desc1 : pr.desc0;
      const float* kp = (sdi & 1) ? pr.kp1 : pr.kp0;
      const Pl xp = planes_of(sd.xs[0], (size_t)sd.cap * 256);
      lj.j[i] = {desc, sd.n, sd.x[0].as<float>(), s->use_tc ? xp.hi : (__half*)nullptr, s->use_tc ? xp.lo : (__half*)nullptr};
      pj.j[i] = {kp, sd.n, sd.cs[0].as<float>(), sd.sn[0].as<float>(), sd.ind[0].as<int>()};
    }
    const int mx = lg_max_n(s, act);
    B2_LAUNCH(ctx, k_lg_load_desc, dim3(cdiv(mx * 64, 256), act.n), 256, 0, st, lj);
    B2_CHECK_LAUNCH(ctx);
    const int pb = cdiv(mx * 32, 1024);
    B2_LAUNCH(ctx, k_lg_posenc, dim3(pb < 16 ? pb : 16, act.n), 1024, 0, st, pj, s->wr);
    B2_CHECK_LAUNCH(ctx);
  }
  const bool do_stop = prm->depth_confidence > 0.0, do_prune = prm->width_confidence > 0.0;
  const float keep_thr = (float)(1.0 - prm->width_confidence);
  int* counters = s->counters.as<int>();
  int* hread = s->hread.as<int>();
  for (int layer = 0; layer < LG_LAYERS && act.n > 0; ++layer) {
    const bool fp16_attn = prm->fp16_attention != 0 && s->use_tc;
    if ((rc = lg_self_layer(ctx, st, s, act, layer, fp16_attn))) return rc;
    if ((rc = lg_cross_block(ctx, st, s, act, layer, fp16_attn))) return rc;
    for (int p = 0; p < np; ++p)
      if (s->pair[p].active) s->pair[p].stop = layer;
    if (layer == LG_LAYERS - 1) break;
    if (!do_stop && !do_prune) continue;
    bool prune_side[LG_MAX_SIDES];
    JobList<HeadJob> hj{};
    JobList<PruneJob> pj{};
    for (int i = 0; i < act.n; ++i) {
      const int sdi = act.side[i];
      LgSide& sd = s->side[sdi];
      prune_side[i] = do_prune && sd.n > prm->prune_min_kpts;
      hj.j[i] = {sd.x[sd.cur].as<float>(), sd.n, prune_side[i] ? s->aw[layer].wm : nullptr, prune_side[i] ? s->aw[layer].bm : nullptr,
                 sd.conf.as<float>(), sd.mat.as<float>(), nullptr};
      pj.j[i] = {sd.conf.as<float>(), sd.mat.as<float>(), sd.n, sd.src.as<int>(), counters + 4 * (sdi >> 1), sdi & 1};
    }
    const int mxn = lg_max_n(s, act);
    B2_LAUNCH(ctx, k_lg_rowheads, dim3(cdiv(mxn, 8), act.n), 256, 0, st, hj, do_stop ? s->tw[layer].w : nullptr,
              do_stop ? s->tw[layer].b : nullptr);
    B2_CHECK_LAUNCH(ctx);
    for (int i = 0; i < act.n; ++i) {
      LgSide& sd = s->side[act.side[i]];
      if (!do_stop) B2_CUDA(ctx, cudaMemsetAsync(sd.conf.p, 0, (size_t)sd.n * 4, st));
      if (!prune_side[i]) B2_CUDA(ctx, cudaMemsetAsync(sd.mat.p, 0x7f, (size_t)sd.n * 4, st));
    }
    B2_LAUNCH(ctx, k_lg_prune_plan, dim3(1, act.n), 1024, 0, st, pj, do_stop ? s->thr[layer] : -1.0f, keep_thr);
    B2_CHECK_LAUNCH(ctx);
    B2_CUDA(ctx, cudaMemcpyAsync(hread, counters, 4 * LG_MAX_PAIRS * sizeof(int), cudaMemcpyDeviceToHost, st));
    B2_CUDA(ctx, cudaStreamSynchronize(st));
    JobList<GatherJob> gj{};
    int ng = 0, gmax = 0;
    for (int p = 0; p < np; ++p) {
      LgPair& lp = s->pair[p];
      if (!lp.active) continue;
      const int* hc = hread + 4 * p;
      if (do_stop) {
        const float ratio = 1.0f - (float)(hc[0] + hc[1]) / (float)(lp.n0 + lp.n1);
        if (ratio > (float)prm->depth_confidence) {
          lp.active = false;
          continue;
        }
      }
      for (int side = 0; side < 2; ++side) {
        LgSide& sd = s->side[2 * p + side];
        const bool pruned = do_prune && sd.n > prm->prune_min_kpts;
        if (!pruned || hc[2 + side] == sd.n) continue;
        const int nxt = sd.cur ^ 1;
        gj.j[ng++] = {sd.src.as<int>(), counters + 4 * p + 2 + side, sd.n, sd.x[sd.cur].as<float>(), sd.cs[sd.cur].as<float>(),
                      sd.sn[sd.cur].as<float>(), sd.ind[sd.cur].as<int>(), sd.x[nxt].as<float>(), sd.cs[nxt].as<float>(), sd.sn[nxt].as<float>(),
                      sd.ind[nxt].as<int>(), s->use_tc ? sd.xs[sd.cur].as<__half>() : (const __half*)nullptr, (size_t)sd.cap * 256,
                      sd.xs[nxt].as<__half>(), (size_t)sd.cap * 256};
        gmax = sd.n > gmax ? sd.n : gmax;
        sd.cur = nxt;
        sd.n = hc[2 + side];
      }
      if (s->side[2 * p].n == 0 || s->side[2 * p + 1].n == 0) lp.active = false;
    }
    if (ng > 0) {
      B2_LAUNCH(ctx, k_lg_gather, dim3(cdiv(gmax, 8), ng), 256, 0, st, gj);
      B2_CHECK_LAUNCH(ctx);
    }
    act = lg_active_sides(s, np);
  }
  const TcWeights tw = lg_tw(s);
  int live[LG_MAX_PAIRS], nlive = 0;
  for (int p = 0; p < np; ++p) {
    pairs[p].out_stop_layer = s->pair[p].stop + 1;
    if (s->pair[p].n0 > 0 && s->pair[p].n1 > 0 && s->side[2 * p].n > 0 && s->side[2 * p + 1].n > 0) live[nlive++] = p;
  }
  if (nlive == 0) return B2_OK;
  for (int layer = 0; layer < LG_LAYERS; ++layer) {
    LinArgs g[LG_MAX_SIDES];
    JobList<HeadJob> hj{};
    int ns = 0, mx = 0;
    for (int li = 0; li < nlive; ++li) {
      if (s->pair[live[li]].stop != layer) continue;
      for (int side = 0; side < 2; ++side) {
        LgSide& sd = s->side[2 * live[li] + side];
        const float* x = sd.x[sd.cur].as<float>();
        LinArgs& a = g[ns];
        a.a1f = x, a.a1p = planes_of(sd.xs[sd.cur], (size_t)sd.cap * 256), a.lda1 = 256, a.K1 = 256, a.w = s->aw[layer].wf, a.ldb = 256;
        a.bias = s->aw[layer].bf, a.scale = 0.25f;
        a.cf = sd.md.as<float>(), a.ldc = 256, a.cp = planes_of(sd.md, (size_t)sd.cap * 256), a.ldch = 256, a.M = sd.n, a.N = 256;
        hj.j[ns] = {x, sd.n, s->aw[layer].wm, s->aw[layer].bm, nullptr, nullptr, sd.ls.as<float>()};
        mx = sd.n > mx ? sd.n : mx;
        ++ns;
      }
    }
    if (ns == 0) continue;
    if ((rc = run_linear(ctx, st, tw, g, ns))) return rc;
    B2_LAUNCH(ctx, k_lg_rowheads, dim3(cdiv(mx, 8), ns), 256, 0, st, hj, (const float*)nullptr, (const float*)nullptr);
    B2_CHECK_LAUNCH(ctx);
  }
  {
    LinArgs gs[LG_MAX_PAIRS];
    for (int li = 0; li < nlive; ++li) {
      const int p = live[li];
      LgSide &a = s->side[2 * p], &b = s->side[2 * p + 1];
      B2_CUDA(ctx, s->sim[p].ensure((size_t)a.n * b.n * 4));
      LinArgs& g = gs[li];
      g.a1f = a.md.as<float>(), g.a1p = planes_of(a.md, (size_t)a.cap * 256), g.lda1 = 256, g.K1 = 256;
      g.bf = b.md.as<float>(), g.bp = planes_of(b.md, (size_t)b.cap * 256), g.ldb = 256;
      g.cf = s->sim[p].as<float>(), g.ldc = b.n, g.tc_want_f32 = true, g.M = a.n, g.N = b.n;
    }
    if ((rc = run_linear(ctx, st, tw, gs, nlive))) return rc;
  }
  for (int li = 0; li < nlive; ++li) {
    const int p = live[li];
    LgSide &a = s->side[2 * p], &b = s->side[2 * p + 1];
    const float* sim = s->sim[p].as<float>();
    if (assign_ps_fits(1, b.n)) {
      const int G = s->persist_ctas;
      B2_CUDA(ctx, s->as_part.ensure((size_t)G * 2 * b.n * sizeof(float)));
      B2_CUDA(ctx, s->as_bar.ensure(16));
      B2_CUDA(ctx, cudaMemsetAsync(s->as_bar.p, 0, 16, st));
      SinkArgs sa{};
      sa.Z = sim, sa.M = a.n, sa.N = b.n, sa.iters = 1, sa.u = a.rmax.as<float>(), sa.v = b.rmax.as<float>();
      sa.rlog = a.rlog.as<float>(), sa.clog = b.rlog.as<float>(), sa.z0 = a.ls.as<float>(), sa.z1 = b.ls.as<float>();
      sa.lsg0 = a.lsg.as<float>(), sa.lsg1 = b.lsg.as<float>(), sa.part = s->as_part.as<float>(), sa.bar = s->as_bar.as<unsigned>();
      sa.best0 = a.amax.as<float>(), sa.arg0 = a.aidx.as<int>(), sa.arg1 = b.aidx.as<int>(), sa.err_flag = s->errflag.as<int>();
      if ((rc = launch_assign_ps<1>(ctx, st, sa, G, "k_lg_assign"))) return rc;
    } else {
    B2_LAUNCH(ctx, k_lg_row_stats, cdiv(a.n, 8), 256, 0, st, sim, a.n, b.n, a.rmax.as<float>(), a.rlog.as<float>(), a.ls.as<float>(),
              a.lsg.as<float>());
    B2_CHECK_LAUNCH(ctx);
    B2_LAUNCH(ctx, k_lg_col_stats, cdiv(b.n, 32), 1024, 0, st, sim, a.n, b.n, b.rmax.as<float>(), b.rlog.as<float>(), b.ls.as<float>(),
              b.lsg.as<float>());
    B2_CHECK_LAUNCH(ctx);
    B2_LAUNCH(ctx, k_lg_row_argmax, cdiv(a.n, 8), 256, 0, st, sim, a.n, b.n, a.rmax.as<float>(), a.rlog.as<float>(),
              b.rmax.as<float>(), b.rlog.as<float>(), a.lsg.as<float>(), b.lsg.as<float>(), a.amax.as<float>(), a.aidx.as<int>());
    B2_CHECK_LAUNCH(ctx);
    B2_LAUNCH(ctx, k_lg_col_argmax, cdiv(b.n, 32), 1024, 0, st, sim, a.n, b.n, a.rmax.as<float>(), a.rlog.as<float>(),
              b.rmax.as<float>(), b.rlog.as<float>(), a.lsg.as<float>(), b.lsg.as<float>(), b.aidx.as<int>());
    B2_CHECK_LAUNCH(ctx);
    }
    B2_LAUNCH(ctx, k_lg_filter, 1, 1024, 0, st, a.amax.as<float>(), a.aidx.as<int>(), b.aidx.as<int>(), a.n,
              (float)prm->filter_threshold, a.ind[a.cur].as<int>(), b.ind[b.cur].as<int>(), s->pair[p].out_matches, s->pair[p].out_scores,
              counters + 4 * LG_MAX_PAIRS + p);
    B2_CHECK_LAUNCH(ctx);
  }
  B2_CUDA(ctx, cudaMemcpyAsync(hread + 4 * LG_MAX_PAIRS, counters + 4 * LG_MAX_PAIRS, LG_MAX_PAIRS * sizeof(int), cudaMemcpyDeviceToHost, st));
  B2_CUDA(ctx, cudaMemcpyAsync(hread + 5 * LG_MAX_PAIRS, s->errflag.p, sizeof(int), cudaMemcpyDeviceToHost, st));
  B2_CUDA(ctx, cudaStreamSynchronize(st));
  if (s->use_tc && hread[5 * LG_MAX_PAIRS]) return b2_fail(ctx, B2_ERR_STATE, "wgmma pipeline timed out on an mbarrier (kernel bug)");
  for (int li = 0; li < nlive; ++li) pairs[live[li]].out_k = hread[4 * LG_MAX_PAIRS + live[li]];
  ctx->debug["lg_desc0"] = {s->side[0].x[s->side[0].cur].as<float>(), (int64_t)s->side[0].n * 256};
  ctx->debug["lg_desc1"] = {s->side[1].x[s->side[1].cur].as<float>(), (int64_t)s->side[1].n * 256};
  return B2_OK;
}

static int lg_match_pairs(b2_context* ctx, b2_lightglue_pair* pairs, int n_pairs, const b2_lightglue_params* prm, cudaStream_t st) {
  LightGlueState* s = ctx->lg;
  if (!s || !s->loaded) return b2_fail(ctx, B2_ERR_STATE, "lightglue weights not set");
  s->persist_ctas = ctx->sm_count - ctx->reserve_sms > 0 ? ctx->sm_count - ctx->reserve_sms : 1;
  const int bmax = ctx->lg_batch > 0 && ctx->lg_batch < LG_MAX_PAIRS ? ctx->lg_batch : LG_MAX_PAIRS;
  for (int p0 = 0; p0 < n_pairs; p0 += bmax) {
    const int np = n_pairs - p0 < bmax ? n_pairs - p0 : bmax;
    int rc = lg_match_batch(ctx, pairs + p0, np, prm, st);
    if (rc) return rc;
  }
  return B2_OK;
}

extern "C" int b2_lightglue_match_batched_dev(b2_context* ctx, b2_lightglue_pair* pairs, int n_pairs, const b2_lightglue_params* params,
                                              void* stream) {
  if (!ctx || !params || n_pairs < 0 || (n_pairs > 0 && !pairs)) return B2_ERR_ARG;
  for (int p = 0; p < n_pairs; ++p) {
    const b2_lightglue_pair& pr = pairs[p];
    if (pr.n0 < 0 || pr.n1 < 0) return B2_ERR_ARG;
    if (pr.n0 > 0 && pr.n1 > 0 && (!pr.kp0 || !pr.desc0 || !pr.kp1 || !pr.desc1 || !pr.out_matches)) return B2_ERR_ARG;
  }
  std::lock_guard<std::mutex> lk(ctx->mu);
  cudaSetDevice(ctx->device);
  return lg_match_pairs(ctx, pairs, n_pairs, params, (cudaStream_t)stream);
}

extern "C" int b2_lightglue_match_dev(b2_context* ctx, const float* kp0, const float* desc0, int n0, const float* kp1,
                                      const float* desc1, int n1, const b2_lightglue_params* params, int64_t* out_matches,
                                      float* out_scores, int* out_k, int* out_stop_layer, void* stream) {
  if (!ctx || !params || !out_k || !out_stop_layer || n0 < 0 || n1 < 0) return B2_ERR_ARG;
  if (n0 > 0 && n1 > 0 && (!kp0 || !desc0 || !kp1 || !desc1 || !out_matches)) return B2_ERR_ARG;
  b2_lightglue_pair pr{kp0, desc0, n0, kp1, desc1, n1, out_matches, out_scores, 0, 1};
  std::lock_guard<std::mutex> lk(ctx->mu);
  cudaSetDevice(ctx->device);
  int rc = lg_match_pairs(ctx, &pr, 1, params, (cudaStream_t)stream);
  *out_k = pr.out_k, *out_stop_layer = pr.out_stop_layer;
  return rc;
}


static uint64_t b2_feat_signature(const void* host, size_t bytes) {
  const unsigned char* p = static_cast<const unsigned char*>(host);
  const uint64_t K0 = 0x9E3779B97F4A7C15ull, K1 = 0xC2B2AE3D27D4EB4Full;
  uint64_t h[4] = {K0 ^ bytes, K1 + bytes, K0 * 3 + bytes, K1 * 5 ^ bytes};
  size_t i = 0;
  for (; i + 32 <= bytes; i += 32) {
    uint64_t w[4];
    memcpy(w, p + i, 32);
#pragma unroll
    for (int l = 0; l < 4; ++l) {
      h[l] = (h[l] ^ w[l]) * K0;
      h[l] ^= h[l] >> 29;
    }
  }
  uint64_t tail = 0;
  for (int sh = 0; i < bytes; ++i, sh += 8) {
    tail ^= (uint64_t)p[i] << (sh & 63);
    if ((sh & 63) == 56) h[0] = (h[0] ^ tail) * K1, h[0] ^= h[0] >> 31, tail = 0;
  }
  h[1] = (h[1] ^ tail) * K1;
  uint64_t r = h[0];
  for (int l = 1; l < 4; ++l) r = (r ^ (h[l] + K0 + (r << 6) + (r >> 2))) * K1, r ^= r >> 32;
  return r;
}
static int b2_upload_cached(b2_context* ctx, const void* host, size_t bytes, DevBuf* fallback, cudaStream_t st, const void** dev) {
  if (ctx->fcache_on < 0) {
    const char* e = getenv("B2_FEATURE_CACHE");
    ctx->fcache_on = (e && e[0] == '1') ? 1 : 0;
  }
  if (!ctx->fcache_on || bytes < 4) {
    B2_CUDA(ctx, fallback->ensure(bytes));
    B2_CUDA(ctx, cudaMemcpyAsync(fallback->p, host, bytes, cudaMemcpyHostToDevice, st));
    ctx->h2d_bytes += bytes;
    *dev = fallback->p;
    return B2_OK;
  }
  const uint64_t sig = b2_feat_signature(host, bytes);
  FeatCacheEntry* lru = &ctx->fcache[0];
  for (FeatCacheEntry& e : ctx->fcache) {
    if (e.host == host && e.bytes == bytes && e.sig == sig) {
      e.stamp = ++ctx->fstamp;
      *dev = e.buf.p;
      return B2_OK;
    }
    if (e.stamp < lru->stamp) lru = &e;
  }
  B2_CUDA(ctx, lru->buf.ensure(bytes));
  B2_CUDA(ctx, cudaMemcpyAsync(lru->buf.p, host, bytes, cudaMemcpyHostToDevice, st));
  ctx->h2d_bytes += bytes;
  lru->host = host, lru->bytes = bytes, lru->sig = sig, lru->stamp = ++ctx->fstamp;
  *dev = lru->buf.p;
  return B2_OK;
}

extern "C" int b2_lightglue_match_host(b2_context* ctx, const float* kp0, const float* desc0, int n0, const float* kp1,
                                       const float* desc1, int n1, const b2_lightglue_params* params,
                                       int64_t* out_matches, float* out_scores, int* out_k, int* out_stop_layer) {
  if (!ctx || !params || !out_k || !out_stop_layer || n0 < 0 || n1 < 0) return B2_ERR_ARG;
  *out_k = 0;
  *out_stop_layer = 1;
  if (n0 == 0 || n1 == 0) return B2_OK;
  if (!kp0 || !desc0 || !kp1 || !desc1 || !out_matches) return B2_ERR_ARG;
  std::lock_guard<std::mutex> lk(ctx->mu);
  cudaSetDevice(ctx->device);
  cudaStream_t st = ctx->stream;
  const int mk = n0 < n1 ? n0 : n1;
  B2_CUDA(ctx, ctx->stage_d[5].ensure((size_t)mk * 2 * 8));
  B2_CUDA(ctx, ctx->stage_d[6].ensure((size_t)mk * 4));
  const float* dkp[2];
  const float* ddesc[2];
  {
    const float* hk[2] = {kp0, kp1};
    const float* hd[2] = {desc0, desc1};
    const int nn[2] = {n0, n1};
    for (int i = 0; i < 2; ++i) {
      const void *a = nullptr, *b = nullptr;
      int rc2;
      if ((rc2 = b2_upload_cached(ctx, hk[i], (size_t)nn[i] * 2 * 4, &ctx->stage_d[2 * i], st, &a))) return rc2;
      if ((rc2 = b2_upload_cached(ctx, hd[i], (size_t)nn[i] * 256 * 4, &ctx->stage_d[2 * i + 1], st, &b))) return rc2;
      dkp[i] = static_cast<const float*>(a), ddesc[i] = static_cast<const float*>(b);
    }
  }
  b2_lightglue_pair pr{dkp[0], ddesc[0], n0, dkp[1], ddesc[1], n1, ctx->stage_d[5].as<int64_t>(), ctx->stage_d[6].as<float>(), 0, 1};
  int rc = lg_match_pairs(ctx, &pr, 1, params, st);
  *out_k = pr.out_k, *out_stop_layer = pr.out_stop_layer;
  if (rc) return rc;
  if (*out_k > 0) {
    B2_CUDA(ctx, cudaMemcpyAsync(out_matches, ctx->stage_d[5].p, (size_t)*out_k * 2 * 8, cudaMemcpyDeviceToHost, st));
    if (out_scores) B2_CUDA(ctx, cudaMemcpyAsync(out_scores, ctx->stage_d[6].p, (size_t)*out_k * 4, cudaMemcpyDeviceToHost, st));
    B2_CUDA(ctx, cudaStreamSynchronize(st));
  }
  return B2_OK;
}
```

gtsfm_b200/csrc/linear.cuh:

```cuda
#pragma once
#include "attn_ps.cuh"
#include "common.cuh"
#include "gemm.cuh"
#include "gemm_ws.cuh"

struct TcWeights {
  const float* f;
  const __half* h;
  const __half* l;
  int* err;
  bool use_tc;
  DevBuf* attn_part = nullptr;
  DevBuf* attn_ml = nullptr;
  DevBuf* attn_cnt = nullptr;
  int sm_count = 132;
};

struct Pl {
  __half* hi;
  __half* lo;
};
static inline Pl planes_of(const DevBuf& b, size_t elems) { return {b.as<__half>(), b.as<__half>() + elems}; }

struct LinArgs {
  const float* a1f = nullptr;
  Pl a1p{nullptr, nullptr};
  int lda1 = 0, K1 = 0;
  const float* a2f = nullptr;
  Pl a2p{nullptr, nullptr};
  int lda2 = 0, K2 = 0;
  const float* w = nullptr;
  const float* bf = nullptr;
  Pl bp{nullptr, nullptr};
  int ldb = 0;
  const float* bias = nullptr;
  float scale = 1.f;
  const float* resid = nullptr;
  int ldr = 0;
  float* cf = nullptr;
  int ldc = 0;
  Pl cp{nullptr, nullptr};
  int ldch = 0;
  int head_major = 0;
  bool tc_want_f32 = false;
  int relu = 0;
  int gelu = 0;
  int lo_unscaled = 0;
  int M = 0, N = 0;
};

static int run_linear(b2_context* ctx, cudaStream_t st, const TcWeights& tw, const LinArgs* a, int np) {
  if (np <= 0) return B2_OK;
  if (np > GW_MAXP) return b2_fail(ctx, B2_ERR_ARG, "run_linear: too many problems in one launch");
  if (!tw.use_tc) {
    for (int i = 0; i < np; ++i) {
      const LinArgs& x = a[i];
      if (x.M <= 0 || x.N <= 0) continue;
      if (x.gelu) return b2_fail(ctx, B2_ERR_ARG, "run_linear: the GELU epilogue exists on the wgmma path only");
      GemmArgs g{};
      g.A1 = x.a1f, g.lda1 = x.lda1, g.K1 = x.K1, g.A2 = x.a2f, g.lda2 = x.lda2, g.K2 = x.K2;
      g.B = x.w ? x.w : x.bf, g.ldb = x.ldb, g.C = x.cf, g.ldc = x.ldc, g.M = x.M, g.N = x.N;
      g.bias = x.bias, g.resid = x.resid, g.ldr = x.ldr, g.scale = x.scale, g.head_major = x.head_major, g.relu = x.relu;
      int rc = launch_gemm(ctx, st, g);
      if (rc) return rc;
    }
    return B2_OK;
  }
  if (!tma_encoder()) return b2_fail(ctx, B2_ERR_CUDA, "cuTensorMapEncodeTiled is not available (driver too old?)");
  const LinArgs& a0 = a[0];
  const bool per_b = a0.w == nullptr;
  static thread_local GemmWsMaps maps;
  GemmWsArgs q{};
  double work = 0.0;
  bool ok = true;
  int nz = 0, tiles = 0;
  for (int i = 0; i < np; ++i) {
    const LinArgs& x = a[i];
    if (x.M <= 0 || x.N <= 0) continue;
    ok = ok && tma_map_2d(&maps.a1h[nz], x.a1p.hi, x.M, x.K1, x.lda1, GW_M) && tma_map_2d(&maps.a1l[nz], x.a1p.lo, x.M, x.K1, x.lda1, GW_M);
    if (x.K2 > 0)
      ok = ok && tma_map_2d(&maps.a2h[nz], x.a2p.hi, x.M, x.K2, x.lda2, GW_M) && tma_map_2d(&maps.a2l[nz], x.a2p.lo, x.M, x.K2, x.lda2, GW_M);
    if (per_b || nz == 0) {
      const __half *bh, *bl;
      if (x.w) {
        const size_t off = (size_t)(x.w - tw.f);
        bh = tw.h + off, bl = tw.l + off;
      } else {
        bh = x.bp.hi, bl = x.bp.lo;
      }
      ok = ok && tma_map_2d(&maps.bh[nz], bh, x.N, x.K1 + x.K2, x.ldb, GW_N) && tma_map_2d(&maps.bl[nz], bl, x.N, x.K1 + x.K2, x.ldb, GW_N);
    }
    GemmProblem& pr = q.p[nz];
    pr.resid = x.resid, pr.C = x.tc_want_f32 ? x.cf : nullptr, pr.Ch = x.cp.hi, pr.Cl = x.cp.lo, pr.M = x.M, pr.N = x.N, pr.ldc = x.ldc;
    {
      auto al16 = [](const void* q) { return (reinterpret_cast<uintptr_t>(q) & 15) == 0; };
      const bool hm = x.head_major != 0;
      bool v = al16(pr.resid) && (x.ldr % 4 == 0 || !pr.resid) && al16(pr.C) && (hm || x.ldc % 4 == 0 || !pr.C);
      v = v && (reinterpret_cast<uintptr_t>(pr.Ch) & 7) == 0 && (reinterpret_cast<uintptr_t>(pr.Cl) & 7) == 0 && (hm || x.ldch % 4 == 0 || !pr.Ch);
      pr.vec4 = v ? 1 : 0;
    }
    pr.tiles_n = cdiv(x.N, GW_N);
    tiles += cdiv(x.M, GW_M) * pr.tiles_n;
    pr.tile_end = tiles;
    work += 2.0 * x.M * x.N * (x.K1 + x.K2);
    ++nz;
  }
  if (nz == 0) return B2_OK;
  if (!ok) return b2_fail(ctx, B2_ERR_CUDA, "cuTensorMapEncodeTiled failed");
  q.nprob = nz, q.tiles = tiles, q.K1 = a0.K1, q.K2 = a0.K2, q.b_per_problem = per_b ? 1 : 0;
  q.bias = a0.bias, q.ldr = a0.ldr, q.scale = a0.scale, q.ldch = a0.ldch;
  q.head_major = a0.head_major, q.relu = a0.relu, q.gelu = a0.gelu, q.lo_unscaled = a0.lo_unscaled, q.err_flag = tw.err;
  b2_prof_work(ctx, "k_gemm_ws", work);
  B2_LAUNCH(ctx, k_gemm_ws, tiles < tw.sm_count ? tiles : tw.sm_count, GW_THREADS, GW_SMEM, st, maps, q);
  B2_CHECK_LAUNCH(ctx);
  return B2_OK;
}

struct FlashPlanes {
  Pl q, k, v, o;
  int nq, nk;
  int heads, ldo;
};
static int run_flash_planes(b2_context* ctx, cudaStream_t st, const TcWeights& tw, const FlashPlanes* jobs, int np, float scale,
                            bool fp16_single = false) {
  if (np <= 0) return B2_OK;
  if (np > AP_MAXP) return b2_fail(ctx, B2_ERR_ARG, "run_flash: too many problems in one launch");
  if (!tma_encoder() || !tw.attn_part) return b2_fail(ctx, B2_ERR_CUDA, "wgmma attention needs cuTensorMapEncodeTiled and its scratch buffers");
  static thread_local AttnPsMaps tmaps;
  AttnPsArgs pa{};
  bool okm = true;
  int items = 0, nz = 0, W = 0, tmax = 0;
  double work = 0.0;
  for (int i = 0; i < np; ++i) {
    const FlashPlanes& j = jobs[i];
    if (j.nq <= 0 || j.nk <= 0) continue;
    AttnPsProblem& p = pa.p[nz];
    p.Qh = j.q.hi, p.Ql = j.q.lo, p.Oh = j.o.hi, p.Ol = j.o.lo, p.Nq = j.nq, p.Nk = j.nk, p.ldo = j.ldo;
    p.qt = cdiv(j.nq, 2 * AW_Q), p.tiles = cdiv(j.nk, AW_KV);
    p.item0 = items;
    items += p.qt * j.heads;
    W += p.qt * j.heads * p.tiles;
    p.w_end = W;
    tmax = p.tiles > tmax ? p.tiles : tmax;
    const uint64_t rows = (uint64_t)j.heads * j.nk;
    okm = okm && tma_map_2d(&tmaps.kh[nz], j.k.hi, rows, 64, 64, AW_KV) && tma_map_2d(&tmaps.kl[nz], j.k.lo, rows, 64, 64, AW_KV);
    okm = okm && tma_map_2d(&tmaps.vh[nz], j.v.hi, rows, 64, 64, AW_KV) && tma_map_2d(&tmaps.vl[nz], j.v.lo, rows, 64, 64, AW_KV);
    work += j.heads * 2.0 * 2.0 * 64 * (double)j.nq * j.nk;
    ++nz;
  }
  if (nz == 0) return B2_OK;
  if (!okm) return b2_fail(ctx, B2_ERR_CUDA, "cuTensorMapEncodeTiled failed (attention)");
  pa.nprob = nz, pa.W = W;
  int ncta = W < tw.sm_count ? W : tw.sm_count;
  pa.quota = cdiv(W, ncta);
  ncta = cdiv(W, pa.quota);
  pa.max_splits = cdiv(tmax, pa.quota) + 1;
  B2_CUDA(ctx, tw.attn_part->ensure((size_t)items * pa.max_splits * 256 * 64 * 4));
  B2_CUDA(ctx, tw.attn_ml->ensure((size_t)items * pa.max_splits * 256 * 2 * 4));
  {
    DevBuf& cnt = *tw.attn_cnt;
    const size_t need = (size_t)items * 2 * sizeof(int);
    if (cnt.cap < need) {
      B2_CUDA(ctx, cnt.ensure(need * 4));
      B2_CUDA(ctx, cudaMemsetAsync(cnt.p, 0, cnt.cap, st));
    }
    pa.arrivals = cnt.as<int>();
  }
  pa.Opart = tw.attn_part->as<float>(), pa.ml = tw.attn_ml->as<float>();
  pa.scale = scale, pa.err_flag = tw.err;
  b2_prof_work(ctx, "k_flash_ps", work);
  if (fp16_single) B2_LAUNCH(ctx, k_flash_ps<true>, ncta, AS_THREADS, AS_SMEM, st, tmaps, pa);
  else B2_LAUNCH(ctx, k_flash_ps<false>, ncta, AS_THREADS, AS_SMEM, st, tmaps, pa);
  B2_CHECK_LAUNCH(ctx);
  return B2_OK;
}

struct FlashJob {
  const DevBuf *q, *k, *v, *o;
  int nq, nk;
  int capq, capk;
};
static int run_flash(b2_context* ctx, cudaStream_t st, const TcWeights& tw, const FlashJob* jobs, int np, float scale, bool fp16_single = false) {
  if (np <= 0) return B2_OK;
  if (np > AP_MAXP) return b2_fail(ctx, B2_ERR_ARG, "run_flash: too many problems in one launch");
  if (!tw.use_tc) {
    for (int i = 0; i < np; ++i) {
      const FlashJob& j = jobs[i];
      int rc = launch_flash(ctx, st, j.q->as<float>(), j.k->as<float>(), j.v->as<float>(), j.o->as<float>(), j.nq, j.nk, scale);
      if (rc) return rc;
    }
    return B2_OK;
  }
  FlashPlanes fp[AP_MAXP];
  for (int i = 0; i < np; ++i) {
    const FlashJob& j = jobs[i];
    fp[i] = {planes_of(*j.q, (size_t)j.capq * 256), planes_of(*j.k, (size_t)j.capk * 256), planes_of(*j.v, (size_t)j.capk * 256),
             planes_of(*j.o, (size_t)j.capq * 256), j.nq, j.nk, 4, 256};
  }
  return run_flash_planes(ctx, st, tw, fp, np, scale, fp16_single);
}
```

include/gtsfm_b200.h:

```cpp
#ifndef GTSFM_B200_H
#define GTSFM_B200_H

#include <stddef.h>
#include <stdint.h>

#ifdef __cplusplus
extern "C" {
#endif

typedef struct b2_context b2_context;

int b2_version(void);
int b2_create(int device, b2_context** out);
void b2_destroy(b2_context* ctx);
const char* b2_last_error(const b2_context* ctx);
uint64_t b2_launch_count(const b2_context* ctx);
uint64_t b2_h2d_bytes(const b2_context* ctx);
int b2_set_option(b2_context* ctx, const char* name, int64_t value);
int b2_profile_start(b2_context* ctx, const char* kernel_prefix);
int b2_profile_stop(b2_context* ctx, double* total_ms, uint64_t* launches, double* work);
int64_t b2_debug_fetch(b2_context* ctx, const char* name, float* host_out, int64_t max_floats);

int b2_debug_gemm_host(b2_context* ctx, int mode, const float* A, const float* B, const float* bias, float* C, int M, int N,
                       int K);
int b2_debug_attention_host(b2_context* ctx, int np, const int* nq, const int* nk, int heads, float scale, int single,
                            const float* q, const float* k, const float* v, float* o);

int b2_superpoint_set_weights(b2_context* ctx, const float* host_blob, size_t n_floats);

int b2_superpoint_detect_dev(b2_context* ctx, const uint8_t* image, int height, int width, int channels, size_t pitch,
                             float keypoint_threshold, int nms_radius, int border, float* out_xy, float* out_score,
                             int cap, int* out_n, uint64_t* out_map_token, void* stream);
int b2_superpoint_describe_dev(b2_context* ctx, uint64_t map_token, const float* xy, int n, float* out_desc, void* stream);
int b2_superpoint_extract_dev(b2_context* ctx, const uint8_t* image, int height, int width, int channels, size_t pitch,
                              float keypoint_threshold, int nms_radius, int border, int max_keypoints, float* out_xy,
                              float* out_score, float* out_desc, int* out_n, void* stream);
int b2_superpoint_extract_async_dev(b2_context* ctx, const uint8_t* image, int height, int width, int channels, size_t pitch,
                                    float threshold, int nms_radius, int border, int max_keypoints, float* out_xy,
                                    float* out_score, float* out_desc, int* out_n_pinned, void* stream);
int b2_superpoint_finish_dev(b2_context* ctx, void* stream);
int b2_topk_indices_dev(b2_context* ctx, const float* scores, int n, int k, int32_t* out_idx, int* out_k, void* stream);

int b2_superpoint_detect_host(b2_context* ctx, const uint8_t* image, int height, int width, int channels,
                              float keypoint_threshold, int nms_radius, int border, float* out_xy, float* out_score,
                              int cap, int* out_n, uint64_t* out_map_token);
int b2_superpoint_describe_host(b2_context* ctx, uint64_t map_token, const float* xy, int n, float* out_desc);

int b2_image_resize_dev(b2_context* ctx, const uint8_t* src, int height, int width, int channels, size_t pitch, uint8_t* dst,
                        int new_height, int new_width, void* stream);

int b2_lightglue_set_weights(b2_context* ctx, const float* host_blob, size_t n_floats);

typedef struct b2_lightglue_params {
  double depth_confidence;
  double width_confidence;
  double filter_threshold;
  int prune_min_kpts;
  int fp16_attention;
} b2_lightglue_params;

int b2_lightglue_match_dev(b2_context* ctx, const float* kp0, const float* desc0, int n0, const float* kp1,
                           const float* desc1, int n1, const b2_lightglue_params* params, int64_t* out_matches,
                           float* out_scores, int* out_k, int* out_stop_layer, void* stream);
int b2_lightglue_match_host(b2_context* ctx, const float* kp0, const float* desc0, int n0, const float* kp1,
                            const float* desc1, int n1, const b2_lightglue_params* params, int64_t* out_matches,
                            float* out_scores, int* out_k, int* out_stop_layer);

typedef struct b2_lightglue_pair {
  const float* kp0;
  const float* desc0;
  int n0;
  const float* kp1;
  const float* desc1;
  int n1;
  int64_t* out_matches;
  float* out_scores;
  int out_k;
  int out_stop_layer;
} b2_lightglue_pair;
int b2_lightglue_match_batched_dev(b2_context* ctx, b2_lightglue_pair* pairs, int n_pairs, const b2_lightglue_params* params,
                                   void* stream);

int b2_superglue_set_weights(b2_context* ctx, const float* host_blob, size_t n_floats);
int b2_superglue_match_dev(b2_context* ctx, const float* kp0, const float* score0, const float* desc0, int n0, int h0,
                           int w0, const float* kp1, const float* score1, const float* desc1, int n1, int h1, int w1,
                           int sinkhorn_iters, float match_threshold, uint32_t* out_matches, float* out_scores,
                           int* out_k, void* stream);
int b2_superglue_match_host(b2_context* ctx, const float* kp0, const float* score0, const float* desc0, int n0, int h0,
                            int w0, const float* kp1, const float* score1, const float* desc1, int n1, int h1, int w1,
                            int sinkhorn_iters, float match_threshold, uint32_t* out_matches, float* out_scores,
                            int* out_k);

typedef struct b2_ransac_params {
  double threshold;
  double confidence;
  int max_iters;
  uint64_t seed;
} b2_ransac_params;

int b2_ransac_essential_host(b2_context* ctx, const double* x1, const double* x2, int k, const b2_ransac_params* params,
                             double* out_model, uint8_t* out_mask, int* out_num_inliers, double* out_R, double* out_t);
int b2_ransac_fundamental_host(b2_context* ctx, const double* x1, const double* x2, int k,
                               const b2_ransac_params* params, double* out_model, uint8_t* out_mask,
                               int* out_num_inliers);
int b2_ransac_essential_dev(b2_context* ctx, const float* kp1, const float* kp2, const int64_t* matches, int k,
                            const double* cal1, const double* cal2, const b2_ransac_params* params, double* out_model,
                            uint8_t* out_mask_dev, int* out_num_inliers, double* out_R, double* out_t, void* stream);
int b2_recover_pose_host(b2_context* ctx, const double* E, const double* x1, const double* x2, int k, double* out_R,
                         double* out_t, int* out_num_good);

size_t b2_netvlad_blob_floats(void);
int b2_netvlad_set_weights(b2_context* ctx, const float* blob, size_t n_floats);
int b2_netvlad_describe_dev(b2_context* ctx, const float* images, int batch, int height, int width, float* out, void* stream);
int b2_netvlad_describe_host(b2_context* ctx, const float* images, int batch, int height, int width, float* out);

size_t b2_megaloc_blob_floats(void);
int b2_megaloc_set_weights(b2_context* ctx, const float* blob, size_t n_floats);
int b2_megaloc_describe_dev(b2_context* ctx, const float* images, int batch, int height, int width, float* out, void* stream);
int b2_megaloc_describe_host(b2_context* ctx, const float* images, int batch, int height, int width, float* out);
int b2_megaloc_describe_u8_dev(b2_context* ctx, const uint8_t* const* images, int n, int height, int width, size_t pitch, float* out,
                               void* stream);
int b2_megaloc_resize_u8_dev(b2_context* ctx, const uint8_t* const* images, int n, int height, int width, size_t pitch, uint8_t* out,
                             void* stream);

int b2_similarity_pairs_host(b2_context* ctx, const float* desc, int n, int dim, int num_matched, float min_score,
                             int32_t* out_partners, float* out_sim);

typedef struct b2_mnn_pair {
  const void* desc0;
  int n0;
  const void* desc1;
  int n1;
  int64_t* out_matches;
  float* out_dist;
  int out_k;
} b2_mnn_pair;
int b2_mnn_match_batched_dev(b2_context* ctx, b2_mnn_pair* pairs, int n_pairs, int dim, int dtype, double ratio, void* stream);
int b2_mnn_match_host(b2_context* ctx, const void* desc0, int n0, const void* desc1, int n1, int dim, int dtype, double ratio,
                      int64_t* out_matches, float* out_dist, int* out_k);

typedef struct b2_sift_keypoint {
  float x, y, size, angle, response;
  int32_t octave;
} b2_sift_keypoint;
typedef struct b2_sift_image {
  const uint8_t* image;
  const uint8_t* mask;
  int max_keypoints;
  b2_sift_keypoint* out_keypoints;
  uint8_t* out_desc;
  int out_n;
  int out_total;
} b2_sift_image;
int b2_sift_detect_batched_dev(b2_context* ctx, b2_sift_image* images, int n_images, int height, int width, int channels,
                               size_t pitch, void* stream);
int b2_sift_detect_host(b2_context* ctx, const uint8_t* image, int height, int width, int channels, const uint8_t* mask,
                        b2_sift_keypoint* out_keypoints, uint8_t* out_desc, int capacity, int* out_n);

size_t b2_d2net_blob_floats(void);
int b2_d2net_norm_table(float* out);
int b2_d2net_set_weights(b2_context* ctx, const float* blob, size_t n_floats);
typedef struct b2_d2net_image {
  const uint8_t* image;
  int max_keypoints;
  float* out_xy;
  float* out_scores;
  float* out_desc;
  int out_n;
  int out_total;
} b2_d2net_image;
int b2_d2net_detect_batched_dev(b2_context* ctx, b2_d2net_image* images, int n_images, int height, int width, int channels,
                                size_t pitch, void* stream);
int b2_d2net_detect_host(b2_context* ctx, const uint8_t* image, int height, int width, int channels, int max_keypoints,
                         float* out_xy, float* out_scores, float* out_desc, int* out_n, int* out_total);
int b2_debug_conv_ps_host(b2_context* ctx, int dilation, const float* in, int height, int width, int cin, int cout, const float* weight,
                          const float* bias, int relu, float* out);
int b2_debug_d2net_avgpool_host(b2_context* ctx, const float* in, int height, int width, float* out);
int b2_debug_d2net_rank_host(b2_context* ctx, const float* scores, const int* cij, int n, int max_k, int* order);

#ifdef __cplusplus
}
#endif
#endif
```

Baseline: 116.2.

## Fuse QKV projection with rotary and head-major segment split in GEMM epilogue

The GEMM epilogue can now write up to three separate output segments (Q, K, V) in head-major split-fp16 form and apply rotary position rotation using per-row cos/sin tables. This lets the LightGlue self-attention QKV projection skip the separate split/rotary kernel and its extra round trip through global memory. The attention kernel now stages only the low-half Q plane in shared memory, which shrinks its shared memory footprint and the Q load work. The change also adds per-call-site profiling names and a debug entry point, and moves GELU into a noinline helper, which may add call overhead in the epilogue.

After: 125.0, median of 6. 7.6% higher.

```diff
diff --git a/gtsfm_b200/_lib.py b/gtsfm_b200/_lib.py
--- a/gtsfm_b200/_lib.py
+++ b/gtsfm_b200/_lib.py
@@ -74,6 +74,7 @@
     "b2_profile_stop": (_i, [_vp, C.POINTER(C.c_double), C.POINTER(C.c_uint64), C.POINTER(C.c_double)]),
     "b2_debug_fetch": (C.c_int64, [_vp, C.c_char_p, _vp, C.c_int64]),
     "b2_debug_gemm_host": (_i, [_vp, _i, _vp, _vp, _vp, _vp, _i, _i, _i]),
+    "b2_debug_gemm_segments_host": (_i, [_vp, _vp, _vp, _vp, _i, _i, _i, _i, _vp, _vp, _i, _vp, _vp]),
     "b2_debug_attention_host": (_i, [_vp, _i, _ip, _ip, _i, _f, _i, _vp, _vp, _vp, _vp]),
     "b2_superpoint_set_weights": (_i, [_vp, _vp, _sz]),
     "b2_superpoint_detect_dev": (_i, [_vp, _vp, _i, _i, _i, _sz, _f, _i, _i, _vp, _vp, _i, _ip, C.POINTER(C.c_uint64), _vp]),
@@ -86,6 +87,7 @@
     "b2_superpoint_describe_host": (_i, [_vp, C.c_uint64, _vp, _i, _vp]),
     "b2_image_resize_dev": (_i, [_vp, _vp, _i, _i, _i, _sz, _vp, _i, _i, _vp]),
     "b2_lightglue_set_weights": (_i, [_vp, _vp, _sz]),
+    "b2_lightglue_qkv_rows": (_i, [_vp]),
     "b2_lightglue_match_dev": (_i, [_vp, _vp, _vp, _i, _vp, _vp, _i, C.POINTER(LightGlueParams), _vp, _vp, _ip, _ip, _vp]),
     "b2_lightglue_match_host": (_i, [_vp, _vp, _vp, _i, _vp, _vp, _i, C.POINTER(LightGlueParams), _vp, _vp, _ip, _ip]),
     "b2_lightglue_match_batched_dev": (_i, [_vp, C.POINTER(LightGluePair), _i, C.POINTER(LightGlueParams), _vp]),
diff --git a/gtsfm_b200/csrc/attn_ps.cuh b/gtsfm_b200/csrc/attn_ps.cuh
--- a/gtsfm_b200/csrc/attn_ps.cuh
+++ b/gtsfm_b200/csrc/attn_ps.cuh
@@ -8,7 +8,7 @@
 constexpr int AS_STAGE = 2 * AS_HALF;
 constexpr int AS_TILE_BYTES = AS_NS * AS_STAGE;
 constexpr int AS_Q_PLANE = AW_Q * AW_D * 2;
-constexpr int AS_Q_BYTES = 2 * 2 * AS_Q_PLANE;
+constexpr int AS_Q_BYTES = 2 * AS_Q_PLANE;
 constexpr size_t AS_SMEM = AS_TILE_BYTES + AS_Q_BYTES + 1024 + 512;
 constexpr int AS_THREADS = 256 + 128;
 constexpr float AS_RESCALE = 8.0f;
@@ -120,7 +120,7 @@
     const int r = t & 127;
     const int rq = (warp & 3) * 16 + (lane >> 2);
     const int c2 = (lane & 3) * 2;
-    const uint32_t sQ = smem0 + AS_TILE_BYTES + q * 2 * AS_Q_PLANE;
+    const uint32_t sQl = smem0 + AS_TILE_BYTES + q * AS_Q_PLANE;
     const float c2s = args.scale * 1.4426950408889634f;
     auto wg_bar = [&]() { asm volatile("bar.sync %0, 128;" ::"r"(1 + q) : "memory"); };
     auto release = [&](int g) { if (lane == 0) tc::mbar_arrive(&kv_empty[g % AS_NS]); };
@@ -130,19 +130,16 @@
       const AttnPsSeg sg = attn_ps_decode(args, w, w_end);
       const AttnPsProblem& pr = args.p[sg.z];
       const int T = sg.T, Nk = pr.Nk;
-      {
+      if (!SINGLE) {
         const int qrow = sg.q0 + q * AW_Q + r;
         wg_bar();
-#pragma unroll
-        for (int pl = 0; pl < (SINGLE ? 1 : 2); ++pl) {
-          const __half* src = (pl ? pr.Ql : pr.Qh) + ((size_t)sg.h * pr.Nq + qrow) * 64;
-          unsigned char* dst = sm + AS_TILE_BYTES + q * 2 * AS_Q_PLANE + pl * AS_Q_PLANE + r * 128;
-#pragma unroll
-          for (int c = 0; c < 8; ++c) {
-            uint4 v = make_uint4(0u, 0u, 0u, 0u);
-            if (qrow < pr.Nq) v = __ldg(reinterpret_cast<const uint4*>(src) + c);
-            *reinterpret_cast<uint4*>(dst + ((c ^ (r & 7)) << 4)) = v;
-          }
+        const __half* src = pr.Ql + ((size_t)sg.h * pr.Nq + qrow) * 64;
+        unsigned char* dst = sm + AS_TILE_BYTES + q * AS_Q_PLANE + r * 128;
+#pragma unroll
+        for (int c = 0; c < 8; ++c) {
+          uint4 v = make_uint4(0u, 0u, 0u, 0u);
+          if (qrow < pr.Nq) v = __ldg(reinterpret_cast<const uint4*>(src) + c);
+          *reinterpret_cast<uint4*>(dst + ((c ^ (r & 7)) << 4)) = v;
         }
         tc::fence_proxy_async();
         wg_bar();
@@ -168,7 +165,7 @@
       auto qk = [&](int i, int sl) {
         const uint32_t sK = smem0 + ((ge + i) % AS_NS) * AS_STAGE;
         const uint64_t dKh = tc::wg_desc_sw128(sK), dKl = tc::wg_desc_sw128(sK + AW_KV_BYTES);
-        const uint64_t dQl = tc::wg_desc_sw128(sQ + AS_Q_PLANE + sl * (64 * 128));
+        const uint64_t dQl = tc::wg_desc_sw128(sQl + sl * (64 * 128));
         tc::wg_fence();
 #pragma unroll
         for (int ks = 0; ks < 4; ++ks) {
diff --git a/gtsfm_b200/csrc/common.cuh b/gtsfm_b200/csrc/common.cuh
--- a/gtsfm_b200/csrc/common.cuh
+++ b/gtsfm_b200/csrc/common.cuh
@@ -170,14 +170,15 @@
   if (ctx->prof.match(kernel)) ctx->prof.work += work;
 }
 
-#define B2_LAUNCH(ctx, kernel, grid, block, smem, stream, ...)  \
-  do {                                                          \
-    const bool _prof = (ctx)->prof.match(#kernel);              \
-    if (_prof) b2_prof_mark((ctx), (stream));                   \
-    kernel<<<(grid), (block), (smem), (stream)>>>(__VA_ARGS__); \
-    if (_prof) b2_prof_mark((ctx), (stream));                   \
-    (ctx)->launches++;                                          \
+#define B2_LAUNCH_NAMED(ctx, name, kernel, grid, block, smem, stream, ...) \
+  do {                                                                     \
+    const bool _prof = (ctx)->prof.match(name);                            \
+    if (_prof) b2_prof_mark((ctx), (stream));                              \
+    kernel<<<(grid), (block), (smem), (stream)>>>(__VA_ARGS__);            \
+    if (_prof) b2_prof_mark((ctx), (stream));                              \
+    (ctx)->launches++;                                                     \
   } while (0)
+#define B2_LAUNCH(ctx, kernel, grid, block, smem, stream, ...) B2_LAUNCH_NAMED(ctx, #kernel, kernel, grid, block, smem, stream, __VA_ARGS__)
 
 #define B2_CHECK_LAUNCH(ctx) B2_CUDA(ctx, cudaGetLastError())
 
diff --git a/gtsfm_b200/csrc/debug.cu b/gtsfm_b200/csrc/debug.cu
--- a/gtsfm_b200/csrc/debug.cu
+++ b/gtsfm_b200/csrc/debug.cu
@@ -55,6 +55,66 @@
   return B2_OK;
 }
 
+extern "C" int b2_debug_gemm_segments_host(b2_context* ctx, const float* A, const float* B, const float* bias, int M, int K, int nseg,
+                                           int rot_mask, const float* cs, const float* sn, int separate, uint16_t* out_hi, uint16_t* out_lo) {
+  if (!ctx || !A || !B || !bias || !out_hi || !out_lo || M <= 0 || K <= 0 || (K % 64) || nseg < 1 || nseg > GW_SEGS ||
+      (rot_mask && (!cs || !sn || separate)))
+    return B2_ERR_ARG;
+  std::lock_guard<std::mutex> lk(ctx->mu);
+  cudaSetDevice(ctx->device);
+  cudaStream_t st = ctx->stream;
+  const int N = 256 * nseg;
+  const size_t ep = (size_t)M * 256;
+  DevBuf dA, dB, dBias, dCs, dSn, dErr, dAh, dAl, dBh, dBl, dH, dL;
+  B2_CUDA(ctx, dA.ensure((size_t)M * K * 4));
+  B2_CUDA(ctx, dB.ensure((size_t)N * K * 4));
+  B2_CUDA(ctx, dBias.ensure((size_t)N * 4));
+  B2_CUDA(ctx, dCs.ensure((size_t)M * 32 * 4));
+  B2_CUDA(ctx, dSn.ensure((size_t)M * 32 * 4));
+  B2_CUDA(ctx, dErr.ensure(16));
+  B2_CUDA(ctx, dAh.ensure((size_t)M * K * 2));
+  B2_CUDA(ctx, dAl.ensure((size_t)M * K * 2));
+  B2_CUDA(ctx, dBh.ensure((size_t)N * K * 2));
+  B2_CUDA(ctx, dBl.ensure((size_t)N * K * 2));
+  B2_CUDA(ctx, dH.ensure(nseg * ep * 2));
+  B2_CUDA(ctx, dL.ensure(nseg * ep * 2));
+  B2_CUDA(ctx, cudaMemcpyAsync(dA.p, A, (size_t)M * K * 4, cudaMemcpyHostToDevice, st));
+  B2_CUDA(ctx, cudaMemcpyAsync(dB.p, B, (size_t)N * K * 4, cudaMemcpyHostToDevice, st));
+  B2_CUDA(ctx, cudaMemcpyAsync(dBias.p, bias, (size_t)N * 4, cudaMemcpyHostToDevice, st));
+  if (rot_mask) {
+    B2_CUDA(ctx, cudaMemcpyAsync(dCs.p, cs, (size_t)M * 32 * 4, cudaMemcpyHostToDevice, st));
+    B2_CUDA(ctx, cudaMemcpyAsync(dSn.p, sn, (size_t)M * 32 * 4, cudaMemcpyHostToDevice, st));
+  }
+  B2_CUDA(ctx, cudaMemsetAsync(dErr.p, 0, 16, st));
+  B2_LAUNCH(ctx, k_split_f32, (unsigned)(((size_t)M * K + 255) / 256), 256, 0, st, dA.as<float>(), (size_t)M * K, dAh.as<__half>(), dAl.as<__half>());
+  B2_LAUNCH(ctx, k_split_f32, (unsigned)(((size_t)N * K + 255) / 256), 256, 0, st, dB.as<float>(), (size_t)N * K, dBh.as<__half>(), dBl.as<__half>());
+  B2_CUDA(ctx, cudaFuncSetAttribute(k_gemm_ws, cudaFuncAttributeMaxDynamicSharedMemorySize, (int)GW_SMEM));
+  TcWeights tw{nullptr, nullptr, nullptr, dErr.as<int>(), true};
+  tw.sm_count = ctx->sm_count;
+  __half *H = dH.as<__half>(), *L = dL.as<__half>(), *Bh = dBh.as<__half>(), *Bl = dBl.as<__half>();
+  LinArgs a;
+  a.a1p = {dAh.as<__half>(), dAl.as<__half>()}, a.lda1 = K, a.K1 = K, a.ldb = K, a.M = M, a.head_major = 1, a.lo_unscaled = 1;
+  for (int s = 0; s < (separate ? nseg : 1); ++s) {
+    if (separate) {
+      a.bp = {Bh + (size_t)s * 256 * K, Bl + (size_t)s * 256 * K}, a.bias = dBias.as<float>() + s * 256, a.N = 256;
+      a.cp = {H + s * ep, L + s * ep};
+    } else {
+      a.bp = {Bh, Bl}, a.bias = dBias.as<float>(), a.N = N, a.seg_n = 256;
+      for (int j = 0; j < nseg; ++j) a.seg_p[j] = {H + j * ep, L + j * ep};
+      a.rot_mask = rot_mask, a.cs = dCs.as<float>(), a.sn = dSn.as<float>();
+    }
+    const int rc = run_linear(ctx, st, tw, &a, 1);
+    if (rc != B2_OK) return rc;
+  }
+  int err = 0;
+  B2_CUDA(ctx, cudaMemcpyAsync(out_hi, H, nseg * ep * 2, cudaMemcpyDeviceToHost, st));
+  B2_CUDA(ctx, cudaMemcpyAsync(out_lo, L, nseg * ep * 2, cudaMemcpyDeviceToHost, st));
+  B2_CUDA(ctx, cudaMemcpyAsync(&err, dErr.p, 4, cudaMemcpyDeviceToHost, st));
+  B2_CUDA(ctx, cudaStreamSynchronize(st));
+  if (err) return b2_fail(ctx, B2_ERR_STATE, "wgmma pipeline timed out on an mbarrier (kernel bug)");
+  return B2_OK;
+}
+
 extern "C" int b2_debug_attention_host(b2_context* ctx, int np, const int* nq, const int* nk, int heads, float scale, int single,
                                        const float* q, const float* k, const float* v, float* o) {
   if (!ctx || !nq || !nk || !q || !k || !v || !o || np <= 0 || np > AP_MAXP || heads <= 0) return B2_ERR_ARG;
diff --git a/gtsfm_b200/csrc/gemm_ws.cuh b/gtsfm_b200/csrc/gemm_ws.cuh
--- a/gtsfm_b200/csrc/gemm_ws.cuh
+++ b/gtsfm_b200/csrc/gemm_ws.cuh
@@ -13,11 +13,13 @@
 constexpr int GW_EW = 4;
 constexpr int GW_THREADS = 512;
 constexpr size_t GW_SMEM = GW_STAGES * GW_STAGE_BYTES + GW_STG_BYTES + 1024  + 256 ;
+constexpr int GW_SEGS = 3;
 
 struct GemmProblem {
   const float* resid;
   float* C;
-  __half *Ch, *Cl;
+  __half *Ch[GW_SEGS], *Cl[GW_SEGS];
+  const float *cs, *sn;
   int M, N, ldc;
   int vec4;
   int tiles_n;
@@ -41,8 +43,12 @@
   int relu;
   int gelu;
   int lo_unscaled;
+  int seg_n;
+  int rot_mask;
   int* err_flag;
 };
+
+static __device__ __noinline__ float gelu_erf(float x) { return 0.5f * x * (1.0f + erff(x * 0.70710678118654752440f)); }
 
 static __global__ void __launch_bounds__(GW_THREADS, 1) k_gemm_ws(const __grid_constant__ GemmWsMaps maps, const __grid_constant__ GemmWsArgs g) {
   extern __shared__ unsigned char gw_raw[];
@@ -159,7 +165,9 @@
       const GemmProblem& pb = g.p[z];
       const float* resid = pb.resid;
       float* C = pb.C;
-      __half *Ch = pb.Ch, *Cl = pb.Cl;
+      const int sg = g.seg_n ? n0 / g.seg_n : 0;
+      __half *Ch = pb.Ch[sg], *Cl = pb.Cl[sg];
+      const bool rot = (g.rot_mask >> sg) & 1;
       const int M = pb.M, ldc = pb.ldc;
       const int n = n0 + c;
       const int ncols = min(4, pb.N - n);
@@ -170,63 +178,91 @@
 #pragma unroll
         for (int e = 0; e < 4; ++e)
           if (e < ncols) b4[e] = __ldg(g.bias + n + e);
-      const size_t hm_col = (size_t)(n >> 6) * M * 64 + (n & 63);
+      const int ns = n - sg * g.seg_n;
+      const size_t hm_col = (size_t)(ns >> 6) * M * 64 + (ns & 63);
       const bool vres = resid && vec;
+      const int rp = (ns & 63) >> 1;
       float4 rr[GW_RB];
-      auto load_resid = [&](int rb) {
-#pragma unroll
-        for (int i = 0; i < GW_RB; ++i)
-          if (rb + GW_EW * i < rows) rr[i] = *reinterpret_cast<const float4*>(resid + (size_t)(m0 + rb + GW_EW * i) * ldr + n);
+      auto load_rows = [&](int rb) {
+        if (rot) {
+#pragma unroll
+          for (int i = 0; i < GW_RB; ++i)
+            if (rb + GW_EW * i < rows) {
+              const size_t o = (size_t)(m0 + rb + GW_EW * i) * 32 + rp;
+              const float2 cc = __ldg(reinterpret_cast<const float2*>(pb.cs + o)), ss = __ldg(reinterpret_cast<const float2*>(pb.sn + o));
+              rr[i] = make_float4(cc.x, cc.y, ss.x, ss.y);
+            }
+        } else {
+#pragma unroll
+          for (int i = 0; i < GW_RB; ++i)
+            if (rb + GW_EW * i < rows) rr[i] = *reinterpret_cast<const float4*>(resid + (size_t)(m0 + rb + GW_EW * i) * ldr + n);
+        }
       };
-      if (vres) load_resid(ew);
+      if (vres || rot) load_rows(ew);
       ok = tc::mbar_wait(sfull, it & 1) && ok;
-      if (ncols > 0) {
+      auto pre = [&](int r, float* v) {
+        const float4 a = *reinterpret_cast<const float4*>(stg + r * GW_PITCH + c);
+        v[0] = a.x, v[1] = a.y, v[2] = a.z, v[3] = a.w;
+#pragma unroll
+        for (int e = 0; e < 4; ++e) {
+          v[e] = (v[e] + b4[e]) * scale;
+          if (relu) v[e] = fmaxf(v[e], 0.f);
+          if (gelu) v[e] = gelu_erf(v[e]);
+        }
+      };
+      if (ncols > 0 && vec) {
         for (int rb = ew; rb < rows; rb += GW_EW * GW_RB) {
-          if (vres && rb != ew) load_resid(rb);
+          if ((vres || rot) && rb != ew) load_rows(rb);
 #pragma unroll
           for (int i = 0; i < GW_RB; ++i) {
             const int r = rb + GW_EW * i;
             if (r >= rows) break;
             const int row = m0 + r;
-            const float4 a = *reinterpret_cast<const float4*>(stg + r * GW_PITCH + c);
-            float v[4] = {a.x, a.y, a.z, a.w};
-#pragma unroll
-            for (int e = 0; e < 4; ++e) {
-              v[e] = (v[e] + b4[e]) * scale;
-              if (relu) v[e] = fmaxf(v[e], 0.f);
-              if (gelu) v[e] = 0.5f * v[e] * (1.0f + erff(v[e] * 0.70710678118654752440f));
-            }
-            const size_t off_c = hm ? hm_col + (size_t)row * 64 : (size_t)row * ldc + n;
-            const size_t off_s = hm ? hm_col + (size_t)row * 64 : (size_t)row * ldch + n;
-            if (vec) {
-              if (resid) v[0] += rr[i].x, v[1] += rr[i].y, v[2] += rr[i].z, v[3] += rr[i].w;
-              if (C) *reinterpret_cast<float4*>(C + off_c) = make_float4(v[0], v[1], v[2], v[3]);
-              if (Ch) {
-                uint32_t h01, l01, h23, l23;
-                if (lo_unscaled) {
-                  tc::split2_unscaled_clamped(v[0], v[1], h01, l01);
-                  tc::split2_unscaled_clamped(v[2], v[3], h23, l23);
-                } else {
-                  tc::split2(v[0], v[1], h01, l01);
-                  tc::split2(v[2], v[3], h23, l23);
-                }
-                *reinterpret_cast<uint2*>(Ch + off_s) = make_uint2(h01, h23);
-                *reinterpret_cast<uint2*>(Cl + off_s) = make_uint2(l01, l23);
+            float v[4];
+            pre(r, v);
+            if (resid) v[0] += rr[i].x, v[1] += rr[i].y, v[2] += rr[i].z, v[3] += rr[i].w;
+            if (rot) {
+              const float c0 = rr[i].x, c1 = rr[i].y, s0 = rr[i].z, s1 = rr[i].w;
+              const float a0 = __fadd_rn(__fmul_rn(v[0], c0), __fmul_rn(-v[1], s0)), a1 = __fadd_rn(__fmul_rn(v[1], c0), __fmul_rn(v[0], s0));
+              const float a2 = __fadd_rn(__fmul_rn(v[2], c1), __fmul_rn(-v[3], s1)), a3 = __fadd_rn(__fmul_rn(v[3], c1), __fmul_rn(v[2], s1));
+              v[0] = a0, v[1] = a1, v[2] = a2, v[3] = a3;
+            }
+            const size_t off = hm ? hm_col + (size_t)row * 64 : (size_t)row * ldc + n;
+            if (C) *reinterpret_cast<float4*>(C + off) = make_float4(v[0], v[1], v[2], v[3]);
+            if (Ch) {
+              const size_t off_s = hm ? off : (size_t)row * ldch + n;
+              uint32_t h01, l01, h23, l23;
+              if (lo_unscaled) {
+                tc::split2_unscaled_clamped(v[0], v[1], h01, l01);
+                tc::split2_unscaled_clamped(v[2], v[3], h23, l23);
+              } else {
+                tc::split2(v[0], v[1], h01, l01);
+                tc::split2(v[2], v[3], h23, l23);
               }
-            } else {
-#pragma unroll
-              for (int e = 0; e < 4; ++e) {
-                if (e >= ncols) break;
-                if (resid) v[e] += resid[(size_t)row * ldr + n + e];
-                if (C) C[off_c + e] = v[e];
-                if (Ch) {
-                  __half hh, ll;
-                  if (lo_unscaled) tc::split_h_unscaled(v[e], hh, ll);
-                  else tc::split_h(v[e], hh, ll);
-                  Ch[off_s + e] = hh;
-                  Cl[off_s + e] = ll;
-                }
-              }
+              *reinterpret_cast<uint2*>(Ch + off_s) = make_uint2(h01, h23);
+              *reinterpret_cast<uint2*>(Cl + off_s) = make_uint2(l01, l23);
+            }
+          }
+        }
+      } else if (ncols > 0) {
+#pragma unroll 1
+        for (int r = ew; r < rows; r += GW_EW) {
+          const int row = m0 + r;
+          float v[4];
+          pre(r, v);
+          const size_t off_c = hm ? hm_col + (size_t)row * 64 : (size_t)row * ldc + n;
+          const size_t off_s = hm ? hm_col + (size_t)row * 64 : (size_t)row * ldch + n;
+#pragma unroll
+          for (int e = 0; e < 4; ++e) {
+            if (e >= ncols) break;
+            if (resid) v[e] += resid[(size_t)row * ldr + n + e];
+            if (C) C[off_c + e] = v[e];
+            if (Ch) {
+              __half hh, ll;
+              if (lo_unscaled) tc::split_h_unscaled(v[e], hh, ll);
+              else tc::split_h(v[e], hh, ll);
+              Ch[off_s + e] = hh;
+              Cl[off_s + e] = ll;
             }
           }
         }
diff --git a/gtsfm_b200/csrc/lightglue.cu b/gtsfm_b200/csrc/lightglue.cu
--- a/gtsfm_b200/csrc/lightglue.cu
+++ b/gtsfm_b200/csrc/lightglue.cu
@@ -13,7 +13,7 @@
   float *wqkv, *bqkv, *wout, *bout, *w0, *b0, *lng, *lnb, *w3, *b3;
 };
 struct CrossW {
-  float *wqk, *bqk, *wv, *bv, *wout, *bout, *w0, *b0, *lng, *lnb, *w3, *b3;
+  float *wqv, *bqv, *wout, *bout, *w0, *b0, *lng, *lnb, *w3, *b3;
 };
 struct AssignW {
   float *wm, *bm, *wf, *bf;
@@ -137,49 +137,27 @@
 struct RotJob {
   const float *qkv, *cs, *sn;
   int n;
-  size_t plane;
-  void *qo, *ko, *vo;
-};
-template <bool SPLIT>
-__global__ void __launch_bounds__(256) k_lg_split_rotary(const __grid_constant__ JobList<RotJob> jobs, int qk_unscaled) {
+  float *qo, *ko, *vo;
+};
+__global__ void __launch_bounds__(256) k_lg_split_rotary(const __grid_constant__ JobList<RotJob> jobs) {
   const RotJob& jb = jobs.j[blockIdx.y];
   const float* __restrict__ qkv = jb.qkv;
   const float* __restrict__ cs = jb.cs;
   const float* __restrict__ sn = jb.sn;
   const int n = jb.n;
-  const size_t plane = jb.plane;
-  void* __restrict__ qo = jb.qo;
-  void* __restrict__ ko = jb.ko;
-  void* __restrict__ vo = jb.vo;
+  float* __restrict__ q = jb.qo;
+  float* __restrict__ k = jb.ko;
+  float* __restrict__ v = jb.vo;
   int i = blockIdx.x * blockDim.x + threadIdx.x;
   if (i >= n * 128) return;
   int p = i & 31, h = (i >> 5) & 3, r = i >> 7;
-  const float* src = qkv + (size_t)r * 768 + (h * 64 + 2 * p) * 3;
-  float q0 = src[0], k0 = src[1], v0 = src[2], q1 = src[3], k1 = src[4], v1 = src[5];
+  const float* src = qkv + (size_t)r * 768 + h * 64 + 2 * p;
+  float q0 = src[0], q1 = src[1], k0 = src[256], k1 = src[257], v0 = src[512], v1 = src[513];
   float c = cs[r * 32 + p], s = sn[r * 32 + p];
   size_t o = ((size_t)h * n + r) * 64 + 2 * p;
   const float qa = __fadd_rn(__fmul_rn(q0, c), __fmul_rn(-q1, s)), qb = __fadd_rn(__fmul_rn(q1, c), __fmul_rn(q0, s));
   const float ka = __fadd_rn(__fmul_rn(k0, c), __fmul_rn(-k1, s)), kb = __fadd_rn(__fmul_rn(k1, c), __fmul_rn(k0, s));
-  if (SPLIT) {
-    __half* outs[3] = {static_cast<__half*>(qo), static_cast<__half*>(ko), static_cast<__half*>(vo)};
-    const float va[3] = {qa, ka, v0}, vb[3] = {qb, kb, v1};
-#pragma unroll
-    for (int j = 0; j < 3; ++j) {
-      __half ha, la, hb, lb;
-      if ((qk_unscaled >> (j < 2 ? 0 : 1)) & 1) {
-        tc::split_h_unscaled(va[j], ha, la);
-        tc::split_h_unscaled(vb[j], hb, lb);
-      } else {
-        tc::split_h(va[j], ha, la);
-        tc::split_h(vb[j], hb, lb);
-      }
-      *reinterpret_cast<__half2*>(outs[j] + o) = __halves2half2(ha, hb);
-      *reinterpret_cast<__half2*>(outs[j] + plane + o) = __halves2half2(la, lb);
-    }
-  } else {
-    float *q = static_cast<float*>(qo), *k = static_cast<float*>(ko), *v = static_cast<float*>(vo);
-    q[o] = qa, q[o + 1] = qb, k[o] = ka, k[o + 1] = kb, v[o] = v0, v[o + 1] = v1;
-  }
+  q[o] = qa, q[o + 1] = qb, k[o] = ka, k[o + 1] = kb, v[o] = v0, v[o + 1] = v1;
 }
 
 struct LnJob {
@@ -529,6 +507,12 @@
 }
 
 
+extern "C" int b2_lightglue_qkv_rows(int* out) {
+  if (!out) return B2_ERR_ARG;
+  for (int r = 0; r < 3 * D; ++r) out[r] = (r % D) * 3 + r / D;
+  return B2_OK;
+}
+
 extern "C" int b2_lightglue_set_weights(b2_context* ctx, const float* blob, size_t n_floats) {
   if (!ctx || !blob) return B2_ERR_ARG;
   std::lock_guard<std::mutex> lk(ctx->mu);
@@ -550,19 +534,28 @@
     for (size_t z : asz) sizes.push_back(z);
   }
   for (int i = 0; i < LG_LAYERS - 1; ++i) sizes.push_back(256), sizes.push_back(1);
+  constexpr int SELF_T = 10, LAYER_T = 22;
+  std::vector<size_t> order(sizes.size());
+  for (size_t i = 0; i < order.size(); ++i) order[i] = i;
+  for (int i = 0; i < LG_LAYERS; ++i) std::swap(order[1 + LAYER_T * i + SELF_T + 1], order[1 + LAYER_T * i + SELF_T + 2]);
   size_t total = 0, src_total = 0;
-  std::vector<size_t> doff;
-  for (size_t z : sizes) {
-    doff.push_back(total);
-    total += (z + 63) / 64 * 64;
-    src_total += z;
-  }
+  std::vector<size_t> doff(sizes.size()), soff(sizes.size());
+  for (size_t k : order) {
+    doff[k] = total;
+    total += (sizes[k] + 63) / 64 * 64;
+  }
+  for (size_t i = 0; i < sizes.size(); ++i) soff[i] = src_total, src_total += sizes[i];
   if (src_total != LG_NFLOATS) return b2_fail(ctx, B2_ERR_STATE, "internal lightglue layout mismatch");
   std::vector<float> host(total, 0.f);
-  size_t so = 0;
-  for (size_t i = 0; i < sizes.size(); ++i) {
-    memcpy(host.data() + doff[i], blob + so, sizes[i] * sizeof(float));
-    so += sizes[i];
+  for (size_t i = 0; i < sizes.size(); ++i) memcpy(host.data() + doff[i], blob + soff[i], sizes[i] * sizeof(float));
+  int qkv_rows[3 * D];
+  b2_lightglue_qkv_rows(qkv_rows);
+  for (int i = 0; i < LG_LAYERS; ++i) {
+    const size_t tw = 1 + LAYER_T * i, tb = tw + 1;
+    for (int r = 0; r < 3 * D; ++r) {
+      memcpy(host.data() + doff[tw] + (size_t)r * D, blob + soff[tw] + (size_t)qkv_rows[r] * D, D * sizeof(float));
+      host[doff[tb] + r] = blob[soff[tb] + qkv_rows[r]];
+    }
   }
   B2_CUDA(ctx, s->wblob.ensure(total * sizeof(float)));
   B2_CUDA(ctx, cudaMemcpy(s->wblob.p, host.data(), total * sizeof(float), cudaMemcpyHostToDevice));
@@ -575,8 +568,8 @@
     a.wqkv = next(), a.bqkv = next(), a.wout = next(), a.bout = next(), a.w0 = next(), a.b0 = next(), a.lng = next(),
     a.lnb = next(), a.w3 = next(), a.b3 = next();
     CrossW& c = s->cw[i];
-    c.wqk = next(), c.bqk = next(), c.wv = next(), c.bv = next(), c.wout = next(), c.bout = next(), c.w0 = next(),
-    c.b0 = next(), c.lng = next(), c.lnb = next(), c.w3 = next(), c.b3 = next();
+    c.wqv = next(), c.bqv = next(), next(), next();
+    c.wout = next(), c.bout = next(), c.w0 = next(), c.b0 = next(), c.lng = next(), c.lnb = next(), c.w3 = next(), c.b3 = next();
   }
   for (int i = 0; i < LG_LAYERS; ++i) {
     AssignW& a = s->aw[i];
@@ -614,7 +607,7 @@
   return t;
 }
 
-static int lg_side_alloc(b2_context* ctx, LgSide& sd, int n) {
+static int lg_side_alloc(b2_context* ctx, LgSide& sd, int n, bool use_tc) {
   const size_t N = (size_t)(n > 0 ? n : 1);
   for (int i = 0; i < 2; ++i) {
     B2_CUDA(ctx, sd.x[i].ensure(N * 256 * 4));
@@ -623,7 +616,7 @@
     B2_CUDA(ctx, sd.sn[i].ensure(N * 32 * 4));
     B2_CUDA(ctx, sd.ind[i].ensure(N * 4));
   }
-  B2_CUDA(ctx, sd.qkv.ensure(N * 768 * 4));
+  if (!use_tc) B2_CUDA(ctx, sd.qkv.ensure(N * 768 * 4));
   B2_CUDA(ctx, sd.q.ensure(N * 256 * 4));
   B2_CUDA(ctx, sd.k.ensure(N * 256 * 4));
   B2_CUDA(ctx, sd.v.ensure(N * 256 * 4));
@@ -656,8 +649,9 @@
   return mx;
 }
 
-static int lg_out_and_ffn(b2_context* ctx, cudaStream_t st, LightGlueState* s, const LgActive& act, const float* wout, const float* bout,
-                          const float* w0, const float* b0, const float* lng, const float* lnb, const float* w3, const float* b3) {
+static int lg_out_and_ffn(b2_context* ctx, cudaStream_t st, LightGlueState* s, const LgActive& act, const char* blk, const float* wout,
+                          const float* bout, const float* w0, const float* b0, const float* lng, const float* lnb, const float* w3,
+                          const float* b3) {
   int rc;
   const TcWeights tw = lg_tw(s);
   LinArgs o[LG_MAX_SIDES], f0[LG_MAX_SIDES], f3[LG_MAX_SIDES];
@@ -677,8 +671,9 @@
     c.resid = x, c.ldr = 256;
     c.cf = x, c.ldc = 256, c.tc_want_f32 = true, c.cp = planes_of(sd.xs[sd.cur], e), c.ldch = 256, c.M = sd.n, c.N = 256;
   }
-  if ((rc = run_linear(ctx, st, tw, o, act.n))) return rc;
-  if ((rc = run_linear(ctx, st, tw, f0, act.n))) return rc;
+  const std::string site(blk);
+  if ((rc = run_linear(ctx, st, tw, o, act.n, (site + "_out").c_str()))) return rc;
+  if ((rc = run_linear(ctx, st, tw, f0, act.n, (site + "_ffn0").c_str()))) return rc;
   {
     JobList<LnJob> lj{};
     for (int i = 0; i < act.n; ++i) {
@@ -692,7 +687,7 @@
       B2_CHECK_LAUNCH(ctx);
     }
   }
-  return run_linear(ctx, st, tw, f3, act.n);
+  return run_linear(ctx, st, tw, f3, act.n, (site + "_ffn3").c_str());
 }
 
 static int lg_self_layer(b2_context* ctx, cudaStream_t st, LightGlueState* s, const LgActive& act, int layer, bool fp16_attn) {
@@ -702,25 +697,28 @@
   LinArgs q[LG_MAX_SIDES];
   for (int i = 0; i < act.n; ++i) {
     LgSide& sd = s->side[act.side[i]];
+    const size_t e = (size_t)sd.cap * 256;
     LinArgs& a = q[i];
-    a.a1f = sd.x[sd.cur].as<float>(), a.a1p = planes_of(sd.xs[sd.cur], (size_t)sd.cap * 256), a.lda1 = 256, a.K1 = 256;
-    a.w = w.wqkv, a.ldb = 256, a.bias = w.bqkv, a.cf = sd.qkv.as<float>(), a.ldc = 768, a.tc_want_f32 = true, a.M = sd.n, a.N = 768;
-  }
-  if ((rc = run_linear(ctx, st, tw, q, act.n))) return rc;
-  {
+    a.a1f = sd.x[sd.cur].as<float>(), a.a1p = planes_of(sd.xs[sd.cur], e), a.lda1 = 256, a.K1 = 256;
+    a.w = w.wqkv, a.ldb = 256, a.bias = w.bqkv, a.M = sd.n, a.N = 768;
+    if (s->use_tc) {
+      a.seg_n = 256, a.seg_p[0] = planes_of(sd.q, e), a.seg_p[1] = planes_of(sd.k, e), a.seg_p[2] = planes_of(sd.v, e);
+      a.rot_mask = 3, a.cs = sd.cs[sd.cur].as<float>(), a.sn = sd.sn[sd.cur].as<float>();
+      a.head_major = 1, a.lo_unscaled = 1;
+    } else {
+      a.cf = sd.qkv.as<float>(), a.ldc = 768;
+    }
+  }
+  if ((rc = run_linear(ctx, st, tw, q, act.n, "lg_self_qkv"))) return rc;
+  const int mx = lg_max_n(s, act);
+  if (!s->use_tc && mx > 0) {
     JobList<RotJob> rj{};
     for (int i = 0; i < act.n; ++i) {
       LgSide& sd = s->side[act.side[i]];
-      rj.j[i] = {sd.qkv.as<float>(), sd.cs[sd.cur].as<float>(), sd.sn[sd.cur].as<float>(), sd.n, (size_t)sd.cap * 256, sd.q.p, sd.k.p, sd.v.p};
-    }
-    const int mx = lg_max_n(s, act);
-    if (mx > 0) {
-      if (s->use_tc)
-        B2_LAUNCH(ctx, k_lg_split_rotary<true>, dim3(cdiv(mx * 128, 256), act.n), 256, 0, st, rj, 3);
-      else
-        B2_LAUNCH(ctx, k_lg_split_rotary<false>, dim3(cdiv(mx * 128, 256), act.n), 256, 0, st, rj, 0);
-      B2_CHECK_LAUNCH(ctx);
-    }
+      rj.j[i] = {sd.qkv.as<float>(), sd.cs[sd.cur].as<float>(), sd.sn[sd.cur].as<float>(), sd.n, sd.q.as<float>(), sd.k.as<float>(), sd.v.as<float>()};
+    }
+    B2_LAUNCH(ctx, k_lg_split_rotary, dim3(cdiv(mx * 128, 256), act.n), 256, 0, st, rj);
+    B2_CHECK_LAUNCH(ctx);
   }
   FlashJob fj[LG_MAX_SIDES];
   for (int i = 0; i < act.n; ++i) {
@@ -728,34 +726,31 @@
     fj[i] = {&a.q, &a.k, &a.v, &a.ctx, a.n, a.n, a.cap, a.cap};
   }
   if ((rc = run_flash(ctx, st, tw, fj, act.n, 0.125f, fp16_attn))) return rc;
-  return lg_out_and_ffn(ctx, st, s, act, w.wout, w.bout, w.w0, w.b0, w.lng, w.lnb, w.w3, w.b3);
+  return lg_out_and_ffn(ctx, st, s, act, "lg_self", w.wout, w.bout, w.w0, w.b0, w.lng, w.lnb, w.w3, w.b3);
 }
 
 static int lg_cross_block(b2_context* ctx, cudaStream_t st, LightGlueState* s, const LgActive& act, int layer, bool fp16_attn) {
   const CrossW& w = s->cw[layer];
   const TcWeights tw = lg_tw(s);
   int rc;
-  for (int which = 0; which < 2; ++which) {
-    LinArgs p[LG_MAX_SIDES];
-    for (int i = 0; i < act.n; ++i) {
-      LgSide& sd = s->side[act.side[i]];
-      const size_t e = (size_t)sd.cap * 256;
-      LinArgs& a = p[i];
-      a.a1f = sd.x[sd.cur].as<float>(), a.a1p = planes_of(sd.xs[sd.cur], e), a.lda1 = 256, a.K1 = 256;
-      a.w = which ? w.wv : w.wqk, a.ldb = 256, a.bias = which ? w.bv : w.bqk;
-      DevBuf& dst = which ? sd.v : sd.q;
-      a.cf = dst.as<float>(), a.cp = planes_of(dst, e), a.head_major = 1, a.M = sd.n, a.N = 256;
-      a.lo_unscaled = s->use_tc ? 1 : 0;
-    }
-    if ((rc = run_linear(ctx, st, tw, p, act.n))) return rc;
-  }
+  LinArgs p[LG_MAX_SIDES];
+  for (int i = 0; i < act.n; ++i) {
+    LgSide& sd = s->side[act.side[i]];
+    const size_t e = (size_t)sd.cap * 256;
+    LinArgs& a = p[i];
+    a.a1f = sd.x[sd.cur].as<float>(), a.a1p = planes_of(sd.xs[sd.cur], e), a.lda1 = 256, a.K1 = 256;
+    a.w = w.wqv, a.ldb = 256, a.bias = w.bqv, a.head_major = 1, a.M = sd.n, a.N = 512;
+    a.seg_n = 256, a.seg_f[0] = sd.q.as<float>(), a.seg_f[1] = sd.v.as<float>(), a.seg_p[0] = planes_of(sd.q, e), a.seg_p[1] = planes_of(sd.v, e);
+    a.lo_unscaled = s->use_tc ? 1 : 0;
+  }
+  if ((rc = run_linear(ctx, st, tw, p, act.n, "lg_cross_qv"))) return rc;
   FlashJob fj[LG_MAX_SIDES];
   for (int i = 0; i < act.n; ++i) {
     LgSide &a = s->side[act.side[i]], &b = s->side[act.side[i] ^ 1];
     fj[i] = {&a.q, &b.q, &b.v, &a.ctx, a.n, b.n, a.cap, b.cap};
   }
   if ((rc = run_flash(ctx, st, tw, fj, act.n, 0.125f, fp16_attn))) return rc;
-  return lg_out_and_ffn(ctx, st, s, act, w.wout, w.bout, w.w0, w.b0, w.lng, w.lnb, w.w3, w.b3);
+  return lg_out_and_ffn(ctx, st, s, act, "lg_cross", w.wout, w.bout, w.w0, w.b0, w.lng, w.lnb, w.w3, w.b3);
 }
 
 static int lg_match_batch(b2_context* ctx, b2_lightglue_pair* pairs, int np, const b2_lightglue_params* prm, cudaStream_t st) {
@@ -771,8 +766,8 @@
       s->side[2 * p].n = s->side[2 * p + 1].n = 0;
       continue;
     }
-    if ((rc = lg_side_alloc(ctx, s->side[2 * p], pr.n0))) return rc;
-    if ((rc = lg_side_alloc(ctx, s->side[2 * p + 1], pr.n1))) return rc;
+    if ((rc = lg_side_alloc(ctx, s->side[2 * p], pr.n0, s->use_tc))) return rc;
+    if ((rc = lg_side_alloc(ctx, s->side[2 * p + 1], pr.n1, s->use_tc))) return rc;
   }
   LgActive act = lg_active_sides(s, np);
   if (act.n == 0) return B2_OK;
@@ -892,7 +887,7 @@
       }
     }
     if (ns == 0) continue;
-    if ((rc = run_linear(ctx, st, tw, g, ns))) return rc;
+    if ((rc = run_linear(ctx, st, tw, g, ns, "lg_assign_proj"))) return rc;
     B2_LAUNCH(ctx, k_lg_rowheads, dim3(cdiv(mx, 8), ns), 256, 0, st, hj, (const float*)nullptr, (const float*)nullptr);
     B2_CHECK_LAUNCH(ctx);
   }
@@ -907,7 +902,7 @@
       g.bf = b.md.as<float>(), g.bp = planes_of(b.md, (size_t)b.cap * 256), g.ldb = 256;
       g.cf = s->sim[p].as<float>(), g.ldc = b.n, g.tc_want_f32 = true, g.M = a.n, g.N = b.n;
     }
-    if ((rc = run_linear(ctx, st, tw, gs, nlive))) return rc;
+    if ((rc = run_linear(ctx, st, tw, gs, nlive, "lg_assign_sim"))) return rc;
   }
   for (int li = 0; li < nlive; ++li) {
     const int p = live[li];
diff --git a/gtsfm_b200/csrc/linear.cuh b/gtsfm_b200/csrc/linear.cuh
--- a/gtsfm_b200/csrc/linear.cuh
+++ b/gtsfm_b200/csrc/linear.cuh
@@ -47,27 +47,43 @@
   int gelu = 0;
   int lo_unscaled = 0;
   int M = 0, N = 0;
-};
-
-static int run_linear(b2_context* ctx, cudaStream_t st, const TcWeights& tw, const LinArgs* a, int np) {
+  int seg_n = 0;
+  float* seg_f[GW_SEGS] = {};
+  Pl seg_p[GW_SEGS] = {};
+  int rot_mask = 0;
+  const float *cs = nullptr, *sn = nullptr;
+};
+
+static int run_linear(b2_context* ctx, cudaStream_t st, const TcWeights& tw, const LinArgs* a, int np, const char* site = nullptr) {
   if (np <= 0) return B2_OK;
   if (np > GW_MAXP) return b2_fail(ctx, B2_ERR_ARG, "run_linear: too many problems in one launch");
+  const LinArgs& a0 = a[0];
+  const int nseg = a0.seg_n > 0 ? a0.N / a0.seg_n : 1;
+  if (a0.seg_n > 0 && (a0.seg_n % GW_N || a0.N != nseg * a0.seg_n || nseg > GW_SEGS || !a0.head_major || a0.resid || a0.tc_want_f32 ||
+                       (a0.rot_mask && (!a0.cs || !a0.sn))))
+    return b2_fail(ctx, B2_ERR_ARG, "run_linear: column segments need N = seg_n x (<= 3), seg_n % 128 == 0, head-major planes, "
+                                    "no residual or fp32 output, and a rotary table when rotary is on");
   if (!tw.use_tc) {
+    if (a0.rot_mask) return b2_fail(ctx, B2_ERR_ARG, "run_linear: the rotary epilogue exists on the wgmma path only");
     for (int i = 0; i < np; ++i) {
       const LinArgs& x = a[i];
       if (x.M <= 0 || x.N <= 0) continue;
       if (x.gelu) return b2_fail(ctx, B2_ERR_ARG, "run_linear: the GELU epilogue exists on the wgmma path only");
-      GemmArgs g{};
-      g.A1 = x.a1f, g.lda1 = x.lda1, g.K1 = x.K1, g.A2 = x.a2f, g.lda2 = x.lda2, g.K2 = x.K2;
-      g.B = x.w ? x.w : x.bf, g.ldb = x.ldb, g.C = x.cf, g.ldc = x.ldc, g.M = x.M, g.N = x.N;
-      g.bias = x.bias, g.resid = x.resid, g.ldr = x.ldr, g.scale = x.scale, g.head_major = x.head_major, g.relu = x.relu;
-      int rc = launch_gemm(ctx, st, g);
-      if (rc) return rc;
+      for (int s = 0; s < nseg; ++s) {
+        const int c0 = s * x.seg_n;
+        GemmArgs g{};
+        g.A1 = x.a1f, g.lda1 = x.lda1, g.K1 = x.K1, g.A2 = x.a2f, g.lda2 = x.lda2, g.K2 = x.K2;
+        g.B = (x.w ? x.w : x.bf) + (size_t)c0 * x.ldb, g.ldb = x.ldb, g.C = x.seg_n ? x.seg_f[s] : x.cf, g.ldc = x.ldc, g.M = x.M;
+        g.N = x.seg_n ? x.seg_n : x.N;
+        g.bias = x.bias ? x.bias + c0 : nullptr, g.resid = x.resid, g.ldr = x.ldr, g.scale = x.scale, g.head_major = x.head_major;
+        g.relu = x.relu;
+        int rc = launch_gemm(ctx, st, g);
+        if (rc) return rc;
+      }
     }
     return B2_OK;
   }
   if (!tma_encoder()) return b2_fail(ctx, B2_ERR_CUDA, "cuTensorMapEncodeTiled is not available (driver too old?)");
-  const LinArgs& a0 = a[0];
   const bool per_b = a0.w == nullptr;
   static thread_local GemmWsMaps maps;
   GemmWsArgs q{};
@@ -91,13 +107,22 @@
       ok = ok && tma_map_2d(&maps.bh[nz], bh, x.N, x.K1 + x.K2, x.ldb, GW_N) && tma_map_2d(&maps.bl[nz], bl, x.N, x.K1 + x.K2, x.ldb, GW_N);
     }
     GemmProblem& pr = q.p[nz];
-    pr.resid = x.resid, pr.C = x.tc_want_f32 ? x.cf : nullptr, pr.Ch = x.cp.hi, pr.Cl = x.cp.lo, pr.M = x.M, pr.N = x.N, pr.ldc = x.ldc;
+    pr.resid = x.resid, pr.C = x.tc_want_f32 ? x.cf : nullptr, pr.M = x.M, pr.N = x.N, pr.ldc = x.ldc;
+    for (int s = 0; s < GW_SEGS; ++s) {
+      const Pl p = x.seg_n ? (s < nseg ? x.seg_p[s] : Pl{nullptr, nullptr}) : (s == 0 ? x.cp : Pl{nullptr, nullptr});
+      pr.Ch[s] = p.hi, pr.Cl[s] = p.lo;
+    }
+    pr.cs = x.cs, pr.sn = x.sn;
     {
       auto al16 = [](const void* q) { return (reinterpret_cast<uintptr_t>(q) & 15) == 0; };
+      auto al8 = [](const void* q) { return (reinterpret_cast<uintptr_t>(q) & 7) == 0; };
       const bool hm = x.head_major != 0;
       bool v = al16(pr.resid) && (x.ldr % 4 == 0 || !pr.resid) && al16(pr.C) && (hm || x.ldc % 4 == 0 || !pr.C);
-      v = v && (reinterpret_cast<uintptr_t>(pr.Ch) & 7) == 0 && (reinterpret_cast<uintptr_t>(pr.Cl) & 7) == 0 && (hm || x.ldch % 4 == 0 || !pr.Ch);
+      v = v && (hm || x.ldch % 4 == 0 || !pr.Ch[0]);
+      for (int s = 0; s < GW_SEGS; ++s) v = v && al8(pr.Ch[s]) && al8(pr.Cl[s]);
+      v = v && al8(pr.cs) && al8(pr.sn);
       pr.vec4 = v ? 1 : 0;
+      if (x.seg_n && !v) return b2_fail(ctx, B2_ERR_ARG, "run_linear: column segments need 8-byte aligned planes and rotary tables");
     }
     pr.tiles_n = cdiv(x.N, GW_N);
     tiles += cdiv(x.M, GW_M) * pr.tiles_n;
@@ -110,8 +135,10 @@
   q.nprob = nz, q.tiles = tiles, q.K1 = a0.K1, q.K2 = a0.K2, q.b_per_problem = per_b ? 1 : 0;
   q.bias = a0.bias, q.ldr = a0.ldr, q.scale = a0.scale, q.ldch = a0.ldch;
   q.head_major = a0.head_major, q.relu = a0.relu, q.gelu = a0.gelu, q.lo_unscaled = a0.lo_unscaled, q.err_flag = tw.err;
-  b2_prof_work(ctx, "k_gemm_ws", work);
-  B2_LAUNCH(ctx, k_gemm_ws, tiles < tw.sm_count ? tiles : tw.sm_count, GW_THREADS, GW_SMEM, st, maps, q);
+  q.seg_n = a0.seg_n, q.rot_mask = a0.rot_mask;
+  const std::string name = site ? std::string("k_gemm_ws/") + site : std::string("k_gemm_ws");
+  b2_prof_work(ctx, name.c_str(), work);
+  B2_LAUNCH_NAMED(ctx, name.c_str(), k_gemm_ws, tiles < tw.sm_count ? tiles : tw.sm_count, GW_THREADS, GW_SMEM, st, maps, q);
   B2_CHECK_LAUNCH(ctx);
   return B2_OK;
 }
diff --git a/include/gtsfm_b200.h b/include/gtsfm_b200.h
--- a/include/gtsfm_b200.h
+++ b/include/gtsfm_b200.h
@@ -23,6 +23,9 @@
 
 int b2_debug_gemm_host(b2_context* ctx, int mode, const float* A, const float* B, const float* bias, float* C, int M, int N,
                        int K);
+int b2_debug_gemm_segments_host(b2_context* ctx, const float* A, const float* B, const float* bias, int M, int K, int nseg,
+                                int rot_mask, const float* cs, const float* sn, int separate, uint16_t* out_hi,
+                                uint16_t* out_lo);
 int b2_debug_attention_host(b2_context* ctx, int np, const int* nq, const int* nk, int heads, float scale, int single,
                             const float* q, const float* k, const float* v, float* o);
 
@@ -50,6 +53,7 @@
                         int new_height, int new_width, void* stream);
 
 int b2_lightglue_set_weights(b2_context* ctx, const float* host_blob, size_t n_floats);
+int b2_lightglue_qkv_rows(int* out);
 
 typedef struct b2_lightglue_params {
   double depth_confidence;
diff --git a/profiles/lightglue_call_sites.py b/profiles/lightglue_call_sites.py
--- /dev/null
+++ b/profiles/lightglue_call_sites.py
@@ -0,0 +1,159 @@
+#!/usr/bin/env python
+from __future__ import annotations
+
+import argparse
+import json
+import subprocess
+import sys
+from collections import deque
+from pathlib import Path
+
+import numpy as np
+
+ROOT = Path(__file__).resolve().parent.parent
+sys.path.insert(0, str(ROOT))
+
+PEAK_FLOPS = 989e12
+PEAK_BYTES = 3.35e12
+LOOKAHEAD, NEW_FRAMES, THR_PX = 20, 2, 4.0
+
+GEMM_SITES = ["lg_self_qkv", "lg_self_out", "lg_self_ffn0", "lg_self_ffn3", "lg_cross_qk", "lg_cross_v", "lg_cross_qv",
+              "lg_cross_out", "lg_cross_ffn0", "lg_cross_ffn3", "lg_assign_proj", "lg_assign_sim"]
+LG_KERNELS = ["k_lg_load_desc", "k_lg_posenc", "k_lg_split_rotary", "k_lg_ln_gelu", "k_lg_rowheads", "k_lg_prune_plan", "k_lg_gather",
+              "k_lg_assign", "k_lg_row_stats", "k_lg_col_stats", "k_lg_row_argmax", "k_lg_col_argmax", "k_lg_filter"]
+GEMM_SHAPE = {
+    "lg_self_qkv": (768, 256), "lg_self_out": (256, 256), "lg_self_ffn0": (512, 512), "lg_self_ffn3": (256, 512),
+    "lg_cross_qk": (256, 256), "lg_cross_v": (256, 256), "lg_cross_qv": (512, 256), "lg_cross_out": (256, 256),
+    "lg_cross_ffn0": (512, 512), "lg_cross_ffn3": (256, 512), "lg_assign_proj": (256, 256)}
+GEMM_ROW_BYTES = {
+    "lg_self_out": 256 * 4 + 256 * 4, "lg_self_ffn0": 512 * 4 + 512 * 4, "lg_self_ffn3": 512 * 4 + 256 * 4 * 3,
+    "lg_cross_qk": 256 * 4 + 256 * 4, "lg_cross_v": 256 * 4 + 256 * 4, "lg_cross_qv": 256 * 4 + 512 * 4,
+    "lg_cross_out": 256 * 4 + 256 * 4, "lg_cross_ffn0": 512 * 4 + 512 * 4, "lg_cross_ffn3": 512 * 4 + 256 * 4 * 3,
+    "lg_assign_proj": 256 * 4 + 256 * 4 * 2}
+
+
+def qkv_row_bytes(fused: bool) -> int:
+    return 256 * 4 + (768 * 4 + 2 * 64 * 4 if fused else 768 * 4)
+
+
+LG_ROW_BYTES = {
+    "k_lg_split_rotary": (768 * 4 + 64 * 4 + 768 * 4, 1.0),
+    "k_lg_ln_gelu": (512 * 4 + 512 * 4, 2.0),
+    "k_lg_rowheads": (256 * 4, 1.0 / 9 * 8),
+}
+
+
+def gpu_name() -> str:
+    try:
+        return subprocess.run(["nvidia-smi", "--query-gpu=name,power.limit,clocks.max.sm", "--format=csv,noheader"], capture_output=True,
+                              text=True, timeout=30).stdout.strip()
+    except Exception as e:
+        return f"unknown ({e!r})"
+
+
+def main():
+    ap = argparse.ArgumentParser()
+    ap.add_argument("--steps", type=int, default=2, help="steps per profiled row (their mean is reported)")
+    ap.add_argument("--warmup", type=int, default=3)
+    ap.add_argument("--out", default=None, help="also write the rows as JSON here")
+    args = ap.parse_args()
+
+    import torch
+
+    from gtsfm_b200 import synthetic as syn
+    from gtsfm_b200.pipeline import DeviceFrontEnd
+
+    dev = torch.device("cuda", 0)
+    fe = DeviceFrontEnd(syn.superpoint_state_dict(0), syn.lightglue_state_dict(2, "bench"), device=0, max_keypoints=5000)
+    n_frames = LOOKAHEAD + NEW_FRAMES * (args.warmup + args.steps * (len(GEMM_SITES) + len(LG_KERNELS) + 2) + 2)
+    frames, cal = syn.synthetic_sequence(n_frames, 480, 640, seed=77)
+    frames_dev = [torch.from_numpy(f).to(dev) for f in frames]
+    window = deque((fe.detect(frames_dev[i]) for i in range(LOOKAHEAD)), maxlen=LOOKAHEAD)
+    cursor = [LOOKAHEAD]
+
+    def step():
+        pending = []
+        for _ in range(NEW_FRAMES):
+            f = fe.detect(frames_dev[cursor[0]])
+            cursor[0] += 1
+            prevs = list(window)
+
+            def on_chunk(c0, res, prevs=prevs, f=f):
+                for prev, (m, _) in zip(prevs[c0:c0 + len(res)], res):
+                    pending.append(fe.verify_async(prev, f, m, cal, cal, THR_PX))
+
+            fe.match_many([(p, f) for p in prevs], on_chunk=on_chunk)
+            window.append(f)
+        for fut in pending:
+            fut.result()
+        torch.cuda.synchronize()
+
+    for _ in range(args.warmup):
+        step()
+    e0, e1 = torch.cuda.Event(enable_timing=True), torch.cuda.Event(enable_timing=True)
+    e0.record()
+    for _ in range(args.steps):
+        step()
+    e1.record()
+    torch.cuda.synchronize()
+    step_ms = e0.elapsed_time(e1) / args.steps
+
+    def profile(prefix):
+        fe.profile_start(prefix)
+        for _ in range(args.steps):
+            step()
+        ms, n, work = fe.profile_stop()
+        return ms / args.steps, n / args.steps, work / args.steps
+
+    rows = {}
+    for site in GEMM_SITES:
+        ms, n, work = profile(f"k_gemm_ws/{site}")
+        if n:
+            rows[site] = {"kernel": f"k_gemm_ws/{site}", "ms": ms, "launches": n, "work": work}
+    for k in LG_KERNELS:
+        ms, n, _ = profile(k)
+        if n:
+            rows[k] = {"kernel": k, "ms": ms, "launches": n, "work": 0.0}
+    fam = {f: profile(f) for f in ("k_gemm_ws", "k_lg_", "k_flash_ps")}
+
+    fused = "k_lg_split_rotary" not in rows
+    R = rows["lg_self_qkv"]["work"] / (2 * 768 * 256)
+    for name, r in rows.items():
+        flop, nbytes = 0.0, None
+        if name in GEMM_SHAPE:
+            N, K = GEMM_SHAPE[name]
+            M = r["work"] / (2 * N * K)
+            flop = 3 * r["work"]
+            nbytes = M * (qkv_row_bytes(fused) if name == "lg_self_qkv" else GEMM_ROW_BYTES[name])
+        elif name == "lg_assign_sim":
+            flop = 3 * r["work"]
+            nbytes = r["work"] / (2 * 256) * 4
+        elif name in LG_ROW_BYTES:
+            per_row, mult = LG_ROW_BYTES[name]
+            nbytes = per_row * mult * R
+        r["gflop"] = flop / 1e9
+        r["mb"] = None if nbytes is None else nbytes / 1e6
+        if nbytes is not None:
+            t_f, t_b = flop / PEAK_FLOPS * 1e3, nbytes / PEAK_BYTES * 1e3
+            r["bound_ms"] = max(t_f, t_b)
+            r["bound"] = "tensor" if t_f >= t_b else "HBM"
+            r["frac_of_bound"] = r["bound_ms"] / r["ms"] if r["ms"] else None
+    out = {"gpu": gpu_name(), "workload": "vga_lightglue (40 pairs per step, <= 5000 keypoints)", "steps_per_row": args.steps,
+           "step_ms": step_ms, "rows_per_block": R, "families": {f: {"ms": v[0], "launches": v[1]} for f, v in fam.items()},
+           "rows": rows}
+    print(f"# {out['gpu']}; step {step_ms:.1f} ms (unprofiled); {R:.0f} keypoint rows per attention block per step")
+    print(f"{'call site / kernel':<34}{'ms/step':>9}{'launch':>8}{'GFLOP':>9}{'MB':>9}{'bound ms':>10}  bound  of bound")
+    for name, r in rows.items():
+        mb = "-" if r["mb"] is None else f"{r['mb']:.0f}"
+        b = "-" if "bound_ms" not in r else f"{r['bound_ms']:.2f}"
+        frac = "-" if "bound_ms" not in r else f"{100 * r['frac_of_bound']:.0f}%"
+        print(f"{r['kernel']:<34}{r['ms']:>9.2f}{r['launches']:>8.0f}{r['gflop']:>9.0f}{mb:>9}{b:>10}  {r.get('bound', '-'):<6} {frac:>5}")
+    for f, (ms, n, _) in fam.items():
+        print(f"{f + ' (family)':<34}{ms:>9.2f}{n:>8.0f}")
+    if args.out:
+        Path(args.out).parent.mkdir(parents=True, exist_ok=True)
+        Path(args.out).write_text(json.dumps(out, indent=1))
+
+
+if __name__ == "__main__":
+    main()
```
